# ZPP-Robotics/OSQP-Solver

Hardware: AMD Instinct MI355X
Metric: QPs/sec on a 1024-QP batch of box-QPs (n=512, m=1024), OSQP defaults; ADMM iters/sec alongside (higher is better)
Workload: dtype f64

## Files before the change

include/mi_osqp.h:

```cpp
#ifndef MI_OSQP_H
#define MI_OSQP_H

#include <stdint.h>

#ifdef __cplusplus
extern "C" {
#endif

typedef enum {
  MI_OSQP_OK = 0,
  MI_OSQP_ERR_INVALID_DATA = 1,
  MI_OSQP_ERR_INVALID_SETTINGS = 2,
  MI_OSQP_ERR_PATTERN_CHANGED = 3,
  MI_OSQP_ERR_NONCONVEX = 4,
  MI_OSQP_ERR_DEVICE = 5,
  MI_OSQP_ERR_NULL = 6,
  MI_OSQP_ERR_ALLOC = 7
} mi_osqp_error;

typedef enum {
  MI_OSQP_EXIT_OPTIMAL = 0,
  MI_OSQP_EXIT_PRIMAL_INFEASIBLE = 1,
  MI_OSQP_EXIT_DUAL_INFEASIBLE = 2,
  MI_OSQP_EXIT_OPTIMAL_INACCURATE = 3,
// ... 132 lines not shown
int mi_osqp_batch_update_A_bounds_some(mi_osqp_batch *h, int64_t n_ids, const int64_t *ids,
                                       const double *A_val, const double *l, const double *u);
int mi_osqp_batch_warm_start_x_some(mi_osqp_batch *h, int64_t n_ids, const int64_t *ids, const double *x );
int mi_osqp_batch_update_q_some(mi_osqp_batch *h, int64_t n_ids, const int64_t *ids, const double *q );
int mi_osqp_batch_warm_start_y_some(mi_osqp_batch *h, int64_t n_ids, const int64_t *ids, const double *y );
int mi_osqp_batch_solve_begin_some(mi_osqp_batch *h, int64_t n_ids, const int64_t *ids);
int mi_osqp_batch_advance(mi_osqp_batch *h, int64_t n_segments);
int mi_osqp_batch_poll(mi_osqp_batch *h, int64_t wait, int64_t *n_finished, int64_t *ids_out, int64_t capacity);
int mi_osqp_batch_get_primal_some(mi_osqp_batch *h, int64_t n_ids, const int64_t *ids, double *x_out );
int mi_osqp_batch_get_dual_some(mi_osqp_batch *h, int64_t n_ids, const int64_t *ids, double *y_out );
int mi_osqp_batch_get_info_some(mi_osqp_batch *h, int64_t n_ids, const int64_t *ids, mi_osqp_info *info );
int64_t mi_osqp_batch_running(mi_osqp_batch *h);

typedef enum {
  MI_GOMP_MODEL_UR5E_FLANGE = 1,
  MI_GOMP_MODEL_UR5E_WRIST3 = 2,
  MI_GOMP_MODEL_UR5E_ELBOW = 3,
  MI_GOMP_MODEL_YAW_2LINK = 4,
  MI_GOMP_MODEL_TABLE = 5
} mi_gomp_model;
typedef struct { int32_t model; int32_t is_gripper; double radius; double param[12]; } mi_gomp_ball;
typedef struct { double dir[2]; double point[3]; int32_t below; int32_t reserved; } mi_gomp_line;
typedef struct mi_gomp_scene mi_gomp_scene;
int mi_gomp_scene_create(mi_gomp_scene **out, mi_osqp_batch *h, int64_t dims, int64_t waypoints,
                         int64_t n_balls, const mi_gomp_ball *balls, int64_t n_lines, const mi_gomp_line *lines,
                         const double *con_lo, const double *con_hi);
void mi_gomp_scene_free(mi_gomp_scene *sc);
int mi_gomp_scene_set_rows(mi_gomp_scene *sc, int64_t n_ids, const int64_t *ids, const double *A_val, const double *l, const double *u);
int mi_gomp_scene_get_rows(mi_gomp_scene *sc, int64_t id, double *A_val, double *l, double *u);
int mi_gomp_assemble_some(mi_gomp_scene *sc, int64_t n_ids, const int64_t *ids, const double *x, int32_t *ok_out);
int mi_gomp_relinearise_some(mi_gomp_scene *sc, int64_t n_ids, const int64_t *ids, const double *x, int32_t *ok_out);

typedef struct mi_osqp_multi mi_osqp_multi;
int mi_osqp_multi_batch_setup(mi_osqp_multi **out, int64_t n_devices, const int64_t *devices,
                              int64_t B, int64_t n, int64_t m,
                              const int64_t *P_colptr, const int64_t *P_rowidx, const double *P_val,
                              const double *q,
                              const int64_t *A_colptr, const int64_t *A_rowidx, const double *A_val,
                              const double *l, const double *u, const mi_osqp_settings *settings);
int mi_osqp_multi_batch_update_A(mi_osqp_multi *h, const int64_t *A_colptr, const int64_t *A_rowidx, const double *A_val);
int mi_osqp_multi_batch_update_bounds(mi_osqp_multi *h, const double *l, const double *u);
int mi_osqp_multi_batch_update_A_bounds(mi_osqp_multi *h, const int64_t *A_colptr, const int64_t *A_rowidx, const double *A_val,
                                        const double *l, const double *u);
int mi_osqp_multi_batch_warm_start_x(mi_osqp_multi *h, const double *x);
int mi_osqp_multi_batch_update_q(mi_osqp_multi *h, const double *q);
int mi_osqp_multi_batch_update_P(mi_osqp_multi *h, const int64_t *P_colptr, const int64_t *P_rowidx, const double *P_val);
int mi_osqp_multi_batch_update_P_A(mi_osqp_multi *h, const int64_t *P_colptr, const int64_t *P_rowidx, const double *P_val,
                                   const int64_t *A_colptr, const int64_t *A_rowidx, const double *A_val);
int mi_osqp_multi_batch_warm_start_y(mi_osqp_multi *h, const double *y);
int mi_osqp_multi_batch_solve(mi_osqp_multi *h);
int mi_osqp_multi_batch_solve_async(mi_osqp_multi *h);
int mi_osqp_multi_batch_wait(mi_osqp_multi *h);
int mi_osqp_multi_batch_get_primal(mi_osqp_multi *h, double *x_out );
int mi_osqp_multi_batch_get_dual(mi_osqp_multi *h, double *y_out );
int mi_osqp_multi_batch_get_info(mi_osqp_multi *h, mi_osqp_info *info );
int64_t mi_osqp_multi_batch_shards(mi_osqp_multi *h);
int mi_osqp_multi_batch_shard(mi_osqp_multi *h, int64_t k, int64_t *device, int64_t *begin, int64_t *end, mi_osqp_batch **handle);
void mi_osqp_multi_batch_free(mi_osqp_multi *h);

int mi_osqp_batch_spmv(mi_osqp_batch *h, const double *d_x, const double *d_y,
                       double *d_Px, double *d_Aty, double *d_Ax, void *stream);
int mi_osqp_batch_kkt_solve(mi_osqp_batch *h, const double *d_rhs, double *d_sol, void *stream);
int mi_osqp_batch_refactor_device(mi_osqp_batch *h);
int mi_osqp_batch_kernel_time(mi_osqp_batch *h, double *avg_ms, int64_t *launches);
int mi_osqp_batch_refactor_time(mi_osqp_batch *h, double *factor_ms, double *tail_ms, int64_t *launches, int64_t *qps);
int mi_osqp_batch_refactor_peak(mi_osqp_batch *h, int64_t *qps, double *factor_ms, double *tail_ms);

int mi_osqp_batch_get_scaling(mi_osqp_batch *h, double *D , double *E , double *c );

int mi_osqp_debug_host_kkt_solve(int64_t n, int64_t m,
                                 const int64_t *P_colptr, const int64_t *P_rowidx, const double *P_val,
                                 const int64_t *A_colptr, const int64_t *A_rowidx, const double *A_val,
                                 const double *l, const double *u, const mi_osqp_settings *settings,
                                 int64_t tile, const double *rhs ,
                                 double *sol_schedule , double *sol_direct ,
                                 mi_osqp_stats *st);

int mi_osqp_debug_host_block_factor(int64_t n, int64_t m,
                                    const int64_t *P_colptr, const int64_t *P_rowidx, const double *P_val,
                                    const int64_t *A_colptr, const int64_t *A_rowidx, const double *A_val,
                                    const double *l, const double *u, const mi_osqp_settings *settings,
                                    double *max_rel_diff_L, double *max_rel_diff_Dinv, int64_t *counts);

int mi_osqp_debug_refactor_chunks(int64_t n_flagged, const int64_t *flagged, int64_t n_active, const int64_t *active, int64_t tile,
                                  int64_t chunk_qps, int64_t max_chunks, int64_t *n_chunks, int64_t *work_begin, int64_t *tiles,
                                  int64_t *tile_begin);

int mi_osqp_debug_trace_kkt_solve(mi_osqp_batch *h, int32_t which, const double *d_rhs, double *d_sol,
                                  uint32_t *out, int64_t out_capacity_words, int64_t *dims);

#ifdef __cplusplus
}
#endif
#endif
```

osqp-solver_amd/__init__.py:

```python
import ctypes as C
import os

import numpy as np

try:
    import torch
except ImportError:
    torch = None

from . import build as _build

_HERE = os.path.dirname(os.path.abspath(__file__))
_LIB = None

EXIT_NAMES = ["kOptimal", "kPrimalInfeasible", "kDualInfeasible", "kOptimalInaccurate",
              "kPrimalInfeasibleInaccurate", "kDualInfeasibleInaccurate", "kMaxIterations",
              "kInterrupted", "kTimeLimitReached", "kNonConvex", "kUnknown"]
K_OPTIMAL = 0


class Settings(C.Structure):
    _fields_ = [("rho", C.c_double), ("sigma", C.c_double), ("scaling", C.c_int64),
                ("adaptive_rho", C.c_int64), ("adaptive_rho_interval", C.c_int64),
                ("adaptive_rho_tolerance", C.c_double), ("max_iter", C.c_int64),
# ... 58 lines not shown
        L.mi_osqp_last_error.restype = C.c_char_p
        L.mi_osqp_batch_setup.argtypes = [C.POINTER(vp), C.c_int64, C.c_int64, C.c_int64, ip, ip, dp, dp, ip, ip, dp,
                                          dp, dp, C.POINTER(Settings), C.c_int64]
        L.mi_osqp_batch_update_A.argtypes = [vp, ip, ip, dp]
        L.mi_osqp_batch_update_A_bounds.argtypes = [vp, ip, ip, dp, dp, dp]
        L.mi_osqp_batch_update_bounds.argtypes = [vp, dp, dp]
        L.mi_osqp_batch_warm_start_x.argtypes = [vp, dp]
        L.mi_osqp_batch_update_q.argtypes = [vp, dp]
        L.mi_osqp_batch_update_q_device.argtypes = [vp, vp, vp]
        L.mi_osqp_batch_update_P.argtypes = [vp, ip, ip, dp]
        L.mi_osqp_batch_update_P_A.argtypes = [vp, ip, ip, dp, ip, ip, dp]
        L.mi_osqp_batch_warm_start_y.argtypes = [vp, dp]
        L.mi_osqp_batch_update_q_some.argtypes = [vp, C.c_int64, ip, dp]
        L.mi_osqp_batch_warm_start_y_some.argtypes = [vp, C.c_int64, ip, dp]
        L.mi_osqp_batch_solve.argtypes = [vp]
        L.mi_osqp_batch_get_primal.argtypes = [vp, dp]
        L.mi_osqp_batch_get_dual.argtypes = [vp, dp]
        L.mi_osqp_batch_get_info.argtypes = [vp, C.POINTER(Info)]
        L.mi_osqp_batch_get_stats.argtypes = [vp, C.POINTER(Stats)]
        L.mi_osqp_batch_get_ordering.argtypes = [vp, ip]
        L.mi_osqp_batch_free.argtypes = [vp]; L.mi_osqp_batch_free.restype = None
        L.mi_osqp_batch_update_bounds_device.argtypes = [vp, vp, vp, vp]
        L.mi_osqp_batch_update_A_bounds_device.argtypes = [vp, vp, vp, vp, vp]
        L.mi_osqp_batch_solve_device.argtypes = [vp, vp, vp, vp, vp]
        L.mi_osqp_batch_reset.argtypes = [vp]
        L.mi_osqp_batch_refactor_device.argtypes = [vp]
        L.mi_osqp_batch_last_solve_stats.argtypes = [vp, ip, ip, dp, dp, ip, dp]
        L.mi_osqp_batch_last_polish_stats.argtypes = [vp, ip, ip, dp]
        L.mi_osqp_batch_get_polish_active.argtypes = [vp, C.POINTER(C.c_int8)]
        L.mi_osqp_batch_get_scaling.argtypes = [vp, dp, dp, dp]
        L.mi_osqp_batch_spmv.argtypes = [vp, vp, vp, vp, vp, vp, vp]
        L.mi_osqp_batch_kkt_solve.argtypes = [vp, vp, vp, vp]
        L.mi_osqp_batch_kernel_time.argtypes = [vp, dp, ip]
        L.mi_osqp_batch_refactor_time.argtypes = [vp, dp, dp, ip, ip]
        L.mi_osqp_batch_refactor_peak.argtypes = [vp, ip, dp, dp]
        L.mi_osqp_batch_reinit_some.argtypes = [vp, C.c_int64, ip, dp, dp, dp]
        L.mi_osqp_batch_update_A_bounds_some.argtypes = [vp, C.c_int64, ip, dp, dp, dp]
        L.mi_osqp_batch_warm_start_x_some.argtypes = [vp, C.c_int64, ip, dp]
        L.mi_osqp_batch_solve_begin_some.argtypes = [vp, C.c_int64, ip]
        L.mi_osqp_batch_advance.argtypes = [vp, C.c_int64]
        L.mi_osqp_batch_poll.argtypes = [vp, C.c_int64, ip, ip, C.c_int64]
        L.mi_osqp_batch_get_primal_some.argtypes = [vp, C.c_int64, ip, dp]
        L.mi_osqp_batch_get_dual_some.argtypes = [vp, C.c_int64, ip, dp]
        L.mi_osqp_batch_get_info_some.argtypes = [vp, C.c_int64, ip, C.POINTER(Info)]
        L.mi_osqp_batch_running.argtypes = [vp]; L.mi_osqp_batch_running.restype = C.c_int64
        L.mi_osqp_setup.argtypes = [C.POINTER(vp), C.c_int64, C.c_int64, ip, ip, dp, dp, ip, ip, dp, dp, dp, C.POINTER(Settings)]
        L.mi_osqp_update_A.argtypes = [vp, ip, ip, dp]
        L.mi_osqp_update_bounds.argtypes = [vp, dp, dp]
        L.mi_osqp_warm_start_x.argtypes = [vp, dp]
        L.mi_osqp_update_q.argtypes = [vp, dp]
        L.mi_osqp_update_P.argtypes = [vp, ip, ip, dp]
        L.mi_osqp_update_P_A.argtypes = [vp, ip, ip, dp, ip, ip, dp]
        L.mi_osqp_warm_start_y.argtypes = [vp, dp]
        L.mi_osqp_solve.argtypes = [vp, C.POINTER(Info)]
        L.mi_osqp_get_primal.argtypes = [vp, dp]
        L.mi_osqp_get_dual.argtypes = [vp, dp]
        L.mi_osqp_get_stats.argtypes = [vp, C.POINTER(Stats)]
        L.mi_osqp_free.argtypes = [vp]; L.mi_osqp_free.restype = None
        L.mi_osqp_multi_batch_setup.argtypes = [C.POINTER(vp), C.c_int64, ip, C.c_int64, C.c_int64, C.c_int64, ip, ip, dp, dp,
                                                ip, ip, dp, dp, dp, C.POINTER(Settings)]
        L.mi_osqp_multi_batch_update_A.argtypes = [vp, ip, ip, dp]
        L.mi_osqp_multi_batch_update_bounds.argtypes = [vp, dp, dp]
        L.mi_osqp_multi_batch_update_A_bounds.argtypes = [vp, ip, ip, dp, dp, dp]
        L.mi_osqp_multi_batch_warm_start_x.argtypes = [vp, dp]
        L.mi_osqp_multi_batch_update_q.argtypes = [vp, dp]
        L.mi_osqp_multi_batch_update_P.argtypes = [vp, ip, ip, dp]
        L.mi_osqp_multi_batch_update_P_A.argtypes = [vp, ip, ip, dp, ip, ip, dp]
        L.mi_osqp_multi_batch_warm_start_y.argtypes = [vp, dp]
        L.mi_osqp_multi_batch_solve.argtypes = [vp]
        L.mi_osqp_multi_batch_solve_async.argtypes = [vp]
        L.mi_osqp_multi_batch_wait.argtypes = [vp]
        L.mi_osqp_multi_batch_get_primal.argtypes = [vp, dp]
        L.mi_osqp_multi_batch_get_dual.argtypes = [vp, dp]
        L.mi_osqp_multi_batch_get_info.argtypes = [vp, C.POINTER(Info)]
        L.mi_osqp_multi_batch_shards.argtypes = [vp]; L.mi_osqp_multi_batch_shards.restype = C.c_int64
        L.mi_osqp_multi_batch_shard.argtypes = [vp, C.c_int64, ip, ip, ip, C.POINTER(vp)]
        L.mi_osqp_multi_batch_free.argtypes = [vp]; L.mi_osqp_multi_batch_free.restype = None
        L.mi_osqp_debug_host_kkt_solve.argtypes = [C.c_int64, C.c_int64, ip, ip, dp, ip, ip, dp, dp, dp,
                                                   C.POINTER(Settings), C.c_int64, dp, dp, dp, C.POINTER(Stats)]
        L.mi_osqp_debug_refactor_chunks.argtypes = [C.c_int64, ip, C.c_int64, ip, C.c_int64, C.c_int64, C.c_int64, ip, ip, ip, ip]
        L.mi_osqp_prefetch_analysis.argtypes = [C.c_int64, C.c_int64, C.c_int64, ip, ip, ip, ip, C.c_int64]
        L.mi_osqp_debug_host_block_factor.argtypes = [C.c_int64, C.c_int64, ip, ip, dp, ip, ip, dp, dp, dp,
                                                      C.POINTER(Settings), dp, dp, ip]
        _LIB = L
    return _LIB


def host_cores():
    try:
        n = len(os.sched_getaffinity(0))
    except Exception:
        n = os.cpu_count() or 1
    for path in ("/sys/fs/cgroup/cpu.max",):
        try:
            quota, period = open(path).read().split()[:2]
            if quota != "max":
                n = min(n, max(1, int(round(int(quota) / int(period)))))
        except Exception:
            pass
    try:
        q = int(open("/sys/fs/cgroup/cpu/cpu.cfs_quota_us").read())
        p = int(open("/sys/fs/cgroup/cpu/cpu.cfs_period_us").read())
        if q > 0:
            n = min(n, max(1, int(round(q / p))))
    except Exception:
        pass
    return n


def default_settings(**kw):
    s = Settings()
    lib().mi_osqp_default_settings(C.byref(s))
    for k, v in kw.items():
        if not hasattr(s, k):
            raise KeyError(k)
        setattr(s, k, v)
    return s


def _i64(a):
    return np.ascontiguousarray(a, dtype=np.int64)


def _f64(a):
    return np.ascontiguousarray(a, dtype=np.float64)


def _ip(a):
    return a.ctypes.data_as(C.POINTER(C.c_int64))


def _dp(a):
    return None if a is None else a.ctypes.data_as(C.POINTER(C.c_double))


def _chk(rc, where):
    if rc != 0:
        raise MiOsqpError(rc, where)


def _csc(M):
    import scipy.sparse as sp
    M = sp.csc_matrix(M)
    M.sort_indices()
    return M


class BatchSolver:

    def __init__(self, P_pattern, Px, q, A_pattern, Ax, l, u, device=-1, **settings):
        L = lib()
        P, A = _csc(P_pattern), _csc(A_pattern)
        self.n, self.m = A.shape[1], A.shape[0]
        Px, Ax, l, u = _f64(Px), _f64(Ax), _f64(l), _f64(u)
        if Ax.ndim == 1:
            Px, Ax, l, u = Px[None], Ax[None], l[None], u[None]
            q = None if q is None else _f64(q)[None]
        self.B = Ax.shape[0]
        q = None if q is None else _f64(q)
        self._Pp, self._Pi = _i64(P.indptr), _i64(P.indices)
        self._Ap, self._Ai = _i64(A.indptr), _i64(A.indices)
        self.settings = default_settings(**settings)
        self._h = C.c_void_p()
        rc = L.mi_osqp_batch_setup(C.byref(self._h), self.B, self.n, self.m, _ip(self._Pp), _ip(self._Pi), _dp(Px),
                                   _dp(q), _ip(self._Ap), _ip(self._Ai), _dp(Ax), _dp(l), _dp(u),
                                   C.byref(self.settings), device)
# ... 330 lines not shown
    def __init__(self, constraints, P, q=None, **settings):
        l, A, u = constraints
        self._b = BatchSolver(P, _csc(P).data, q, A, _csc(A).data, l, u, **settings)

    def update(self, constraints):
        l, A, u = constraints
        A = _csc(A)
        try:
            self._b.update_A(A.data, A_pattern=A)
            self._b.update_bounds(l, u)
        except MiOsqpError as e:
            raise ValueError(str(e)) from e

    def setWarmStart(self, x):
        self._b.warm_start_x(x)

    def solve(self):
        info = self._b.solve()[0]
        return int(info.exit_code), self._b.primal()[0]

    def info(self):
        return self._b.info()[0]

    def dual(self):
        return self._b.dual()[0]

    def stats(self):
        return self._b.stats()


def debug_host_kkt_solve(P, A, l, u, rhs, tri_waves=0, **settings):
    L = lib()
    P, A = _csc(P), _csc(A)
    n, m = A.shape[1], A.shape[0]
    s = default_settings(**settings)
    rhs = _f64(rhs)
    sol_s, sol_d = np.empty(n + m), np.empty(n + m)
    st = Stats()
    Pp, Pi, Px = _i64(P.indptr), _i64(P.indices), _f64(P.data)
    Ap, Ai, Ax = _i64(A.indptr), _i64(A.indices), _f64(A.data)
    l, u = _f64(l), _f64(u)
    rc = L.mi_osqp_debug_host_kkt_solve(n, m, _ip(Pp), _ip(Pi), _dp(Px), _ip(Ap), _ip(Ai), _dp(Ax), _dp(l), _dp(u),
                                        C.byref(s), 1 + int(tri_waves), _dp(rhs), _dp(sol_s), _dp(sol_d), C.byref(st))
    _chk(rc, "debug_host_kkt_solve")
    return sol_s, sol_d, st.as_dict()


def prefetch_analysis(P, A, B=1, device=-1, check=True):
    L = lib()
    P, A = _csc(P), _csc(A)
    n, m = A.shape[1], A.shape[0]
    Pp, Pi, Ap, Ai = _i64(P.indptr), _i64(P.indices), _i64(A.indptr), _i64(A.indices)
    rc = L.mi_osqp_prefetch_analysis(B, n, m, _ip(Pp), _ip(Pi), _ip(Ap), _ip(Ai), device)
    if check:
        _chk(rc, "prefetch_analysis")
    return rc


def debug_refactor_chunks(flagged, active, tile, chunk_qps, max_chunks=8):
    f, a = _i64(flagged), _i64(active)
    nch = C.c_int64()
    wb = np.zeros(max_chunks + 2, dtype=np.int64); tb = np.zeros(max_chunks + 2, dtype=np.int64)
    tl = np.zeros(max(1, len(a)), dtype=np.int64)
    _chk(lib().mi_osqp_debug_refactor_chunks(len(f), _ip(f), len(a), _ip(a), tile, chunk_qps, max_chunks, C.byref(nch), _ip(wb), _ip(tl),
                                             _ip(tb)), "debug_refactor_chunks")
    k = int(nch.value)
    return ([f[wb[c]:wb[c + 1]].tolist() for c in range(k)], [tl[tb[c]:tb[c + 1]].tolist() for c in range(k)])


def debug_host_block_factor(P, A, l, u, **settings):
    L = lib()
    P, A = _csc(P), _csc(A)
    n, m = A.shape[1], A.shape[0]
    s = default_settings(**settings)
    Pp, Pi, Px = _i64(P.indptr), _i64(P.indices), _f64(P.data)
    Ap, Ai, Ax = _i64(A.indptr), _i64(A.indices), _f64(A.data)
    l, u = _f64(l), _f64(u)
    dL, dD = C.c_double(), C.c_double()
    cnt = (C.c_int64 * 4)()
    rc = L.mi_osqp_debug_host_block_factor(n, m, _ip(Pp), _ip(Pi), _dp(Px), _ip(Ap), _ip(Ai), _dp(Ax), _dp(l), _dp(u),
                                           C.byref(s), C.byref(dL), C.byref(dD), cnt)
    _chk(rc, "debug_host_block_factor")
    return dL.value, dD.value, dict(blocks=cnt[0], triples=cnt[1], storage=cnt[2], levels=cnt[3])
```

osqp-solver_amd/csrc/device_types.h:

```cpp
#pragma once
#include <hip/hip_runtime.h>
#include <stdint.h>

namespace miosqp {

#define MI_CHUNK 16

struct SchedDev {
  const uint32_t *step, *idxw;
  const uint64_t *idxw64;
  const uint32_t *lvl_pos, *tail_bar;
  int n_phases, nw, n_levels;
  uint32_t n_steps, n_slots;
};

struct DenseTailDev {
  int s, k, n_phases;
  uint32_t n_steps;
  const uint32_t *task;
  const uint32_t *wave_task, *wave_step, *tail_bar;
};

enum { DS_C = 0, DS_CINV, DS_RHO, DS_RHO_EST, DS_PRI_RES, DS_DUA_RES, DS_OBJ, DS_COUNT };
enum { IS_STATUS = 0, IS_ITER, IS_RHO_UPDATES, IS_DONE, IS_NEED_REFACTOR, IS_CUR, IS_PENDING, IS_EPOCH, IS_COUNT };

struct KernelArgs {
  int n, m, N, B;
  SchedDev fwd, bwd, chk;
  const uint32_t *pinv;
  const uint32_t *xloc;
  const double *fwd_val, *bwd_val, *chk_val, *dinv;
  DenseTailDev dt;
  const double *dt_val;
  const double *fwd_val0, *bwd_val0, *dt_val0;
  const int *use_work;
  double *x, *z, *y;
  const double *q, *l, *u, *rho_vec, *rho_inv, *Dsc, *Dsc_inv, *Esc, *Esc_inv;
  double *dx, *dy, *out1, *out2, *dscal;
  int *iscal;
  double *x_out, *y_out;
  double *xs_global;
  int xs_len;
  int rs_off;
  int rf_off;
  int wide;
  double sigma, alpha, eps_abs, eps_rel, eps_prim_inf, eps_dual_inf, rho_tolerance;
  int check_termination, rho_interval, max_iter, scaled_termination, scaling, adaptive_rho;
  int iter_begin, iter_end;
  int op_out_lds;
  int info_at_end;
  int mw_groups;
  unsigned *mw_bar;
  double *mw_scratch;
  int df;
  unsigned df_shadow;
  const unsigned char *rflag;
  const int *sel;
  const int *tiles;
};

struct FactorArgs {
  int n, m, N, B, nnzP, nnzK, pa_len, n_levels, force_all;
  int debug_skip;
  uint32_t storage;
  SchedDev fwd, bwd;
  const uint32_t *blk, *lvl, *utask, *tri4, *dtask, *ttask, *asm_dst, *asm_src;
  const uint32_t *ubig;
  int *use_work;
  const int32_t *fwd_srcblk, *bwd_srcblk;
  const double *pa_val, *l, *u, *dscal;
  double *rho_vec, *rho_inv, *Lblk, *Dl, *dinv_scratch, *fwd_val, *bwd_val, *dinv;
  int *iscal, *npos;
  int home_bt;
  const int *work;
  double sigma;
  int dt_k;
  int mw_groups;
  unsigned *mw_bar;
  const signed char *pmask;
  const int32_t *arow;
  int *pstat;
  double pdelta;
};

struct TailArgs {
  int n, N, s, k, kbt, home_bt;
  uint32_t storage, n_slots;
  int n_lt, n_ltcol;
  uint32_t n_quads;
  int nh;
  uint32_t cs_doubles;
  const int *work;
  const uint32_t *lt_pos, *ltcol_col, *tile_tab, *wave_tiles, *diag_tile;
  const uint64_t *asm_q64;
  const int32_t *src_tile;
  const uint32_t *dt_task, *dt_task_step;
  uint32_t n_tasks;
  const double *Lblk, *Dl;
  double *Sd, *dt_val, *dinv;
  int *npos, *iscal;
  unsigned long long *trace;
  int *pstat;
};
hipError_t launch_tail(const TailArgs &a, int nwork, size_t lds_asm, size_t lds, hipStream_t st);

struct PolishArgs {
  int *stat;
  signed char *act;
  double *sol;
  int refine_iter;
};
hipError_t launch_polish_active(const KernelArgs &a, const PolishArgs &p, int BT, hipStream_t st);
hipError_t launch_polish(const KernelArgs &a, const PolishArgs &p, int BT, int tiles, int threads, size_t lds, int n_cus, hipStream_t st);
hipError_t launch_factor(const FactorArgs &a, int BT, int tiles, int threads, hipStream_t st);
size_t factor_lds_bytes(int BT, int threads);
bool factor_fits_lds(const FactorArgs &a, int threads);

int max_coresident_groups(int threads, size_t lds, int n_cus);
int max_coresident_factor_groups(int threads, int n_cus);
hipError_t launch_iterate(const KernelArgs &a, int BT, int tiles, int threads, size_t lds, hipStream_t st);
int rf_head_steps();
int rf_lds_steps();
hipError_t launch_check(const KernelArgs &a, int BT, int tiles, int threads, size_t lds, hipStream_t st);
hipError_t launch_advance(const KernelArgs &a, int BT, int tiles, int threads, size_t lds, hipStream_t st, int max_segments, int seg_len,
                          int *host_is, double *host_ds, unsigned *stop, unsigned seq, unsigned *counter, unsigned *host_done);
hipError_t launch_spmv(const KernelArgs &a, int BT, int tiles, int threads, size_t lds, hipStream_t st,
                       const double *x, const double *y, double *Px, double *Aty, double *Ax);
struct SpmvFused {
  const uint32_t *ptr, *ent;
  const double *pa_val;
  int pa_len;
  const uint32_t *ell, *rowid;
  int n_pass;
  uint32_t ell_off[4], ell_k[4];
};
hipError_t launch_spmv_fused(const KernelArgs &a, const SpmvFused &t, int BT, int tiles, int n_cus, hipStream_t st,
                             const double *x, const double *y, double *Px, double *Aty, double *Ax);
size_t spmv_fused_lds_bytes(int n, int m, int pa_len, int BT);
hipError_t launch_kkt_solve(const KernelArgs &a, int BT, int tiles, int threads, size_t lds, hipStream_t st,
                            const double *rhs, double *sol);
hipError_t launch_kkt_trace(const KernelArgs &a, int BT, int tiles, int threads, size_t lds, hipStream_t st,
                            const double *rhs, double *sol, uint32_t *trace, uint32_t words);
hipError_t launch_warm_start(const KernelArgs &a, int BT, int tiles, int threads, size_t lds, hipStream_t st,
                             const double *x0);
hipError_t launch_interleave(const double *src, double *dst, const int *ids, int nq, int len, int BT, hipStream_t st);
hipError_t launch_scatter(const double *src, double *dst, const int *map, const int *ids, int nq, int srclen,
                          const SchedDev &sd, int BT, hipStream_t st);
hipError_t launch_deinterleave(const double *src, double *dst, int nq, int len, int BT, hipStream_t st);
struct RuizArgs {
  int n, m, nnzP, nnzA, B, BT, iters;
  const int *ids;
  int raw_by_qp;
  int fresh;
  const double *rawP, *rawq;
  const int32_t *Prow, *Pcol, *Arow, *Acol;
  const double *rawPnew;
  const double *rawA;
  const double *rawl, *rawu;
  double *pa_val, *q, *Dsc, *Dsc_inv, *Esc, *Esc_inv, *l, *u, *dscal;
  double *dn, *en;
  double *pa_out;
};
hipError_t launch_ruiz(const RuizArgs &a, hipStream_t st);
hipError_t launch_lin_cost(const double *gq, const int *ids, double *q, double *rawq, const double *Dsc, const double *dscal,
                           int nq, int n, int BT, int scaling, hipStream_t st);
hipError_t launch_warm_start_y(const KernelArgs &a, int nslots, int BT, hipStream_t st, const double *y0);
hipError_t launch_start_slots(const KernelArgs &a, const int *slots, const int *clear, int nslots, int BT, int cold, hipStream_t st);
hipError_t launch_fresh_slots(const KernelArgs &a, const int *slots, int nslots, int BT, double rho0, hipStream_t st);
hipError_t launch_worklist(const int *iscal, int *work, int nslots, int BT, hipStream_t st);
hipError_t launch_resume_flagged(const KernelArgs &a, int nslots, int BT, hipStream_t st);
hipError_t launch_copy_slot_streams(double *dst, const double *src, const int *slots, int nslots, size_t per, hipStream_t st);
hipError_t launch_keep_rows(double *dst, const double *src, const int *ids, int n_ids, int len, hipStream_t st);
hipError_t launch_copy_flagged_streams(double *dst, const double *src, const int *flags, int want, int nslots, size_t per, hipStream_t st);
hipError_t launch_copy_slot_rows(double *dst, const double *src, const int *slots, int nslots, int len, int BT, hipStream_t st);
enum { MI_GM_UR5E_FLANGE = 1, MI_GM_UR5E_WRIST3 = 2, MI_GM_UR5E_ELBOW = 3, MI_GM_YAW_2LINK = 4, MI_GM_TABLE = 5 };
struct GompBallDev { int model, is_gripper; double radius; double param[12]; };
struct GompLineDev { double D[3], A[3]; int below, pad; };
struct GompArgs {
  int dims, W, n_balls, n_lines, n, m, nnzA, n_ids, row0, write_rows;
  const int *ids;
  const GompBallDev *balls;
  const GompLineDev *lines;
  double con_lo[3], con_hi[3];
  const int *aidx;
  const double *traj;
// ... 12 lines not shown
```

osqp-solver_amd/csrc/host_core.cpp:

```cpp
#include "host_core.hpp"
#include "sched_format.h"

#include <algorithm>
#include <cmath>
#include <cstdio>
#include <cstdlib>
#include <cstring>
#include <numeric>
#include <set>
#include <chrono>
#include <thread>

#include "../../include/mi_osqp.h"

namespace miosqp {

int validate_settings(const Settings &s) {
  if (s.scaling < 0 || s.max_iter <= 0 || s.check_termination < 0) return 1;
  if (s.adaptive_rho != 0 && s.adaptive_rho != 1) return 1;
  if (s.adaptive_rho_interval < 0 || s.adaptive_rho_tolerance < 1.0) return 1;
  if (!(s.rho > 0.0) || !(s.sigma > 0.0)) return 1;
  if (s.eps_abs < 0.0 || s.eps_rel < 0.0 || (s.eps_abs == 0.0 && s.eps_rel == 0.0)) return 1;
  if (!(s.eps_prim_inf > 0.0) || !(s.eps_dual_inf > 0.0)) return 1;
  if (!(s.alpha > 0.0) || !(s.alpha < 2.0)) return 1;
// ... 726 lines not shown
          ut_of_level[lev1].push_back({id, tb, te, te});
        }
        if (n1 < tl.size()) {
          uint32_t tb = (uint32_t)(bf.tri.size() / 2);
          for (size_t q = n1; q < tl.size(); q++) bf.tri.insert(bf.tri.end(), {tl[q].first, tl[q].second});
          uint32_t te = (uint32_t)(bf.tri.size() / 2);
          ut_of_level[L].push_back({id, tb, tb, te});
        }
      }
    }
  for (int L = 0; L < nlev; L++) {
    uint32_t u0 = (uint32_t)(bf.utask.size() / 4), d0 = (uint32_t)bf.dtask.size(), t0 = (uint32_t)(bf.ttask.size() / 2);
    auto &uts = ut_of_level[L];
    std::stable_sort(uts.begin(), uts.end(), [](const UT &a, const UT &b) { return a.te - a.tb > b.te - b.tb; });
    {
      auto small = [&](const UT &u) { return u.te - u.tb <= 16u && (bf.blk[4 * u.id + 3] & 255u) <= 8u; };
      std::stable_partition(uts.begin(), uts.end(), [&](const UT &u) { return !small(u); });
      uint32_t nbig = 0;
      while (nbig < uts.size() && !small(uts[nbig])) nbig++;
      bf.ubig.push_back(u0 + nbig);
    }
    for (const UT &u : uts) bf.utask.insert(bf.utask.end(), {u.id, u.tb, u.tm, u.te});
    if (getenv("MI_OSQP_DEBUG_ORDER") && !uts.empty()) {
      std::vector<double> wv(16, 0.0);
      size_t r1 = 0, gen = 0;
      for (size_t k = 0; k < uts.size(); k++) { wv[k % 16] += (uts[k].tm - uts[k].tb + 7) / 8 * 1.0 + (uts[k].te - uts[k].tm) * 1.5; r1 += uts[k].tm - uts[k].tb; gen += uts[k].te - uts[k].tm; }
      fprintf(stderr, "[mi_osqp] factor level %d: %zu update tasks, rank-1 triples %zu, general %zu, biggest task %u, modelled path %.0f units (ideal %.0f)\n",
              L, uts.size(), r1, gen, uts[0].te - uts[0].tb, *std::max_element(wv.begin(), wv.end()), (r1 / 8.0 + gen * 1.5) / 16);
    }
    for (int pass = 0; pass < 2; pass++) {
      for (int J : cols_of_level[L]) {
        if (J >= ct0 || (cw(J) > 4) != (pass == 0)) continue;
        for (const auto &[I, id] : colblk[J]) {
          if (I == J) bf.dtask.push_back(id);
          else bf.ttask.insert(bf.ttask.end(), {id, colblk[J][0].second});
        }
      }
      if (pass == 0) { bf.ubig.push_back((uint32_t)bf.dtask.size()); bf.ubig.push_back((uint32_t)(bf.ttask.size() / 2)); }
    }
    bf.lvl.insert(bf.lvl.end(), {u0, (uint32_t)(bf.utask.size() / 4), d0, (uint32_t)bf.dtask.size(), t0, (uint32_t)(bf.ttask.size() / 2)});
  }
  if (getenv("MI_OSQP_DEBUG_ORDER")) {
    size_t cnt[5] = {0, 0, 0, 0, 0}, small = 0;
    for (size_t t = 0; t < bf.utask.size() / 4; t++) {
      const uint32_t w = bf.blk[4 * bf.utask[4 * t] + 3] & 255u, sz = bf.utask[4 * t + 3] - bf.utask[4 * t + 1];
      cnt[w <= 1 ? 0 : w <= 2 ? 1 : w <= 4 ? 2 : w <= 8 ? 3 : 4]++;
      small += sz <= 16;
    }
    fprintf(stderr, "[mi_osqp] update tasks by target width: 1: %zu, 2: %zu, 3-4: %zu, 5-8: %zu, 9-16: %zu; %zu of %zu with <= 16 triples\n", cnt[0], cnt[1], cnt[2], cnt[3], cnt[4], small, bf.utask.size() / 4);
  }
  bf.utask4.resize(bf.utask.size());
  for (size_t t = 0; t < bf.utask.size() / 4; t++) {
    const uint32_t id = bf.utask[4 * t], tb = bf.utask[4 * t + 1], tm = bf.utask[4 * t + 2], te = bf.utask[4 * t + 3];
    const uint32_t hw = bf.blk[4 * id + 3];
    if (tm - tb >= (1u << 22)) bf.overflow = true;
    bf.utask4[4 * t] = bf.blk[4 * id]; bf.utask4[4 * t + 1] = tb; bf.utask4[4 * t + 2] = ((hw >> 8) << 27) | ((hw & 255u) << 22) | ((tm - tb) & 0x3FFFFFu); bf.utask4[4 * t + 3] = te - tm;
  }
  bf.dtask4.resize(4 * bf.dtask.size());
  for (size_t t = 0; t < bf.dtask.size(); t++) for (int k = 0; k < 4; k++) bf.dtask4[4 * t + k] = bf.blk[4 * bf.dtask[t] + k];
  bf.ttask4.resize(2 * bf.ttask.size());
  for (size_t t = 0; t < bf.ttask.size() / 2; t++) {
    const uint32_t id = bf.ttask[2 * t], dg = bf.ttask[2 * t + 1];
    bf.ttask4[4 * t] = bf.blk[4 * id]; bf.ttask4[4 * t + 1] = bf.blk[4 * id + 2]; bf.ttask4[4 * t + 2] = bf.blk[4 * id + 3]; bf.ttask4[4 * t + 3] = bf.blk[4 * dg];
  }
  bf.tri4.resize(2 * bf.tri.size());
  for (size_t q = 0; q < bf.tri.size() / 2; q++) {
    const uint32_t ia = bf.tri[2 * q], ib = bf.tri[2 * q + 1];
    const uint32_t ahw = bf.blk[4 * ia + 3], bh = bf.blk[4 * ib + 3] >> 8;
    bf.tri4[4 * q] = bf.blk[4 * ia]; bf.tri4[4 * q + 1] = bf.blk[4 * ib]; bf.tri4[4 * q + 2] = bf.blk[4 * ia + 2];
    bf.tri4[4 * q + 3] = ((ahw >> 8) << 16) | ((ahw & 255u) << 8) | bh;
  }
  const int n = an.n, m = an.m, nnzK = an.nnzK();
  bf.asm_dst.assign(nnzK, 0); bf.asm_src.assign(nnzK, 0);
  std::vector<int> colOfK(nnzK);
  for (int j = 0; j < N; j++) for (int k = an.Kp[j]; k < an.Kp[j + 1]; k++) colOfK[k] = j;
  for (int e = 0; e < nnzK; e++) {
    int a = an.pinv[an.Ki[e]], b = an.pinv[colOfK[e]];
    bf.asm_dst[e] = pos_of(std::max(a, b), std::min(a, b));
  }
  for (int k = 0; k < an.Pp[n]; k++) bf.asm_src[an.PtoK[k]] = ((uint32_t)(an.PisDiag[k] ? ASM_P_SIGMA : ASM_P) << 29) | (uint32_t)k;
  for (int pos : an.sigmaOnlyK) bf.asm_src[pos] = (uint32_t)ASM_SIGMA << 29;
  for (int k = 0; k < an.Ap[n]; k++) bf.asm_src[an.AtoK[k]] = ((uint32_t)ASM_A << 29) | (uint32_t)k;
  for (int r = 0; r < m; r++) bf.asm_src[an.rhotoK[r]] = ((uint32_t)ASM_NEG_RHOINV << 29) | (uint32_t)r;
  bf.lpos.assign(an.nnzLx(), 0);
  for (int j = 0; j < N; j++) for (int p = an.Lp[j]; p < an.Lp[j + 1]; p++) bf.lpos[p] = (int32_t)pos_of(an.Li[p], j);
  for (int c = 0; c < nch; c++) {
    const int c0 = an.chunk_start[c], r = cw(c);
    if (an.inv_off[c] < 0) continue;
    const uint32_t id = find_blk(c, c), off = bf.blk[4 * id];
    for (int k = 0; k < r; k++) for (int i = k + 1; i < r; i++) bf.lpos[an.inv_index(c, i, k)] = (int32_t)(off + (uint32_t)i * r + (uint32_t)k);
    (void)c0;
  }
  auto compose = [&](const Schedule &s, std::vector<int32_t> &out) {
    out.resize(s.src.size());
    for (size_t k = 0; k < s.src.size(); k++) out[k] = s.src[k] >= 0 ? bf.lpos[s.src[k]] : s.src[k];
  };
  compose(an.fwd, an.fwd_srcblk);
  compose(an.bwd, an.bwd_srcblk);
  if (an.dt.k) {
    const int k = an.dt.k;
    an.dt.sblk.assign((size_t)k * k, 0u);
    for (int j = 0; j < k; j++) for (int i = j; i < k; i++) an.dt.sblk[(size_t)j * k + i] = pos_of(ts + i, ts + j);
    DenseTail &dt = an.dt;
    const int nt = k / 16;
    dt.lt_pos.clear(); dt.ltcol_col.clear();
    std::vector<std::vector<std::pair<int, std::vector<uint16_t>>>> frag(nt);
    for (int c = 0; c < ts; c++) {
      int ci = -1;
      for (int p = an.Lp[c]; p < an.Lp[c + 1]; p++) {
        const int i = an.Li[p];
        if (i < ts) continue;
        if (ci < 0) { ci = (int)dt.ltcol_col.size(); dt.ltcol_col.push_back((uint32_t)c); }
        const int I = (i - ts) / 16;
        if (frag[I].empty() || frag[I].back().first != ci) frag[I].push_back({ci, std::vector<uint16_t>(16, 0xFFFFu)});
        frag[I].back().second[(i - ts) % 16] = (uint16_t)dt.lt_pos.size();
        dt.lt_pos.push_back((uint32_t)bf.lpos[p]);
      }
    }
    dt.n_lt = (int)dt.lt_pos.size(); dt.n_ltcol = (int)dt.ltcol_col.size();
    const uint16_t zero_slot = (uint16_t)dt.n_lt;
    for (auto &fr : frag) for (auto &f : fr) for (uint16_t &v : f.second) if (v == 0xFFFFu) v = zero_slot;
    struct TileRec { int I, J; std::vector<std::pair<int, int>> src; };
    std::vector<TileRec> tiles;
    for (int I = 0; I < nt; I++)
      for (int J = 0; J <= I; J++) {
        TileRec t{I, J, {}};
        size_t a = 0, b = 0;
        while (a < frag[I].size() && b < frag[J].size()) {
          if (frag[I][a].first < frag[J][b].first) a++;
          else if (frag[I][a].first > frag[J][b].first) b++;
          else { t.src.push_back({(int)a, (int)b}); a++; b++; }
        }
        tiles.push_back(std::move(t));
      }
    const int nw = 16;
    std::vector<int> order(tiles.size());
    std::iota(order.begin(), order.end(), 0);
    std::stable_sort(order.begin(), order.end(), [&](int x, int y) { return tiles[x].src.size() > tiles[y].src.size(); });
    std::vector<std::vector<int>> mine(nw);
    for (size_t d = 0; d < order.size(); d++) { const size_t round = d / nw, pos = d % nw; mine[(round & 1) ? nw - 1 - pos : pos].push_back(order[d]); }
    dt.tile_tab.clear(); dt.wave_tiles.assign(nw + 1, 0u); dt.asm_q.clear(); dt.asm_qcol.clear();
    for (int w = 0; w < nw; w++) {
      dt.wave_tiles[w] = (uint32_t)(dt.tile_tab.size() / 4);
      for (int ti : mine[w]) {
        const TileRec &t = tiles[ti];
        const uint32_t q0 = (uint32_t)(dt.asm_q.size() / 64);
        const size_t padded = (t.src.size() + 31) / 32 * 32;
        for (size_t s0 = 0; s0 < padded; s0 += 4) {
          for (int g = 0; g < 4; g++) {
            const bool real = s0 + g < t.src.size();
            const auto *fa = real ? &frag[t.I][t.src[s0 + g].first] : nullptr;
            const auto *fb = real ? &frag[t.J][t.src[s0 + g].second] : nullptr;
            dt.asm_qcol.push_back(real ? (uint16_t)fa->first : (uint16_t)0);
            for (int e = 0; e < 16; e++) dt.asm_q.push_back(real ? ((uint32_t)fa->second[e] | ((uint32_t)fb->second[e] << 16)) : ((uint32_t)zero_slot | ((uint32_t)zero_slot << 16)));
          }
        }
        const uint32_t blk_id = find_blk(ct0 + t.I, ct0 + t.J);
        dt.tile_tab.insert(dt.tile_tab.end(), {((uint32_t)t.I << 16) | (uint32_t)t.J, bf.blk[4 * blk_id], q0, (uint32_t)(dt.asm_q.size() / 64)});
      }
    }
    dt.wave_tiles[nw] = (uint32_t)(dt.tile_tab.size() / 4);
    dt.asm_q64.resize(dt.asm_q.size());
    for (size_t e = 0; e < dt.asm_q.size(); e++) {
      const uint64_t w = dt.asm_q[e], ci = dt.asm_qcol[e / 16];
      dt.asm_q64[e] = ((w & 0xFFFFu) * 8u) | ((((w >> 16) * 8u) | ((ci * 8u) << 17)) << 32);
    }
    dt.src_tile.resize(dt.src.size());
    for (size_t e = 0; e < dt.src.size(); e++) {
      const int32_t sc = dt.src[e];
      dt.src_tile[e] = sc < 0 ? sc : (int32_t)dt_tile_offset(sc % k, sc / k);
    }
    dt.diag_tile.resize(k);
    for (int i = 0; i < k; i++) dt.diag_tile[i] = dt_tile_offset(i, i);
    dt.task_step.clear();
    { uint32_t pos = 0; for (size_t t = 0; t < dt.task.size() / 4; t++) { dt.task_step.push_back(pos); pos += dt.task[4 * t + 3]; } }
  }
}


Tuning tuning_from_env() {
  Tuning t;
  if (const char *e = getenv("MI_OSQP_TILE")) { const int v = atoi(e); if (v == 1 || v == 2 || v == 4) t.tile = v; }
  if (const char *e = getenv("MI_OSQP_THREADS")) t.threads = std::max(64, std::min(1024, atoi(e) / 64 * 64));
  t.global_xs = getenv("MI_OSQP_GLOBAL_XS") != nullptr;
  if (const char *e = getenv("MI_OSQP_GROUPS")) t.groups = std::max(0, std::min(256, atoi(e)));
  if (const char *e = getenv("MI_OSQP_GROUP_THREADS")) t.group_threads = std::max(64, std::min(512, atoi(e) / 64 * 64));
  if (const char *e = getenv("MI_OSQP_ASSUME_CUS")) t.assume_cus = std::max(0, atoi(e));
  if (const char *e = getenv("MI_OSQP_FACTOR_THREADS")) t.factor_threads = std::max(64, std::min(1024, atoi(e) / 64 * 64));
  if (const char *e = getenv("MI_OSQP_FACTOR_GROUPS")) t.factor_groups = std::max(1, std::min(256, atoi(e)));
  t.ruiz = getenv("MI_OSQP_HOST_RUIZ") ? 1 : getenv("MI_OSQP_DEVICE_RUIZ") ? -1 : 0;
  if (const char *e = getenv("MI_OSQP_CONT_RING_KB")) t.cont_ring_kb = std::max(0L, atol(e));
  if (const char *e = getenv("MI_OSQP_ANALYSIS_CACHE")) t.analysis_cache = atoi(e) != 0;
  t.stream_state = getenv("MI_OSQP_STREAM_STATE") != nullptr;
  t.stream_factor = getenv("MI_OSQP_STREAM_FACTOR") != nullptr;
  if (const char *e = getenv("MI_OSQP_REFACTOR_PIPELINE")) t.refactor_pipeline = atoi(e) != 0;
  if (const char *e = getenv("MI_OSQP_REFACTOR_PIPELINE_MIN")) t.pipeline_min = std::max(0, atoi(e));
  if (const char *e = getenv("MI_OSQP_REFACTOR_CHUNKS")) t.pipeline_chunks = std::max(0, std::min(8, atoi(e)));
  if (const char *e = getenv("MI_OSQP_REFACTOR_CHUNK_QPS")) t.pipeline_chunk_qps = std::max(0, atoi(e));
  AnalysisTuning &a = t.analysis;
  if (const char *e = getenv("MI_OSQP_DENSE_TAIL")) a.dense_tail = atoi(e);
  if (const char *e = getenv("MI_OSQP_ORDERING")) a.ordering = e[0];
  if (const char *e = getenv("MI_OSQP_ND_LEAF")) a.nd_leaf = atoi(e);
  if (const char *e = getenv("MI_OSQP_RELAX")) a.relax = atoi(e);
  a.serial = getenv("MI_OSQP_SERIAL_ANALYSIS") != nullptr;
  return t;
}

RefactorChunks refactor_chunks(const std::vector<int> &flagged, const std::vector<int> &active, int bt, int chunk_qps, int max_chunks) {
  RefactorChunks rc;
  const int nq = (int)flagged.size();
  max_chunks = std::max(1, max_chunks);
  chunk_qps = std::max(1, chunk_qps);
  if ((nq + chunk_qps - 1) / chunk_qps > max_chunks) chunk_qps = (nq + max_chunks - 1) / max_chunks;
  const int n_ref = (nq + chunk_qps - 1) / chunk_qps;
  rc.n_chunks = 1 + n_ref;
  rc.work_begin.assign(1, 0);
  for (int c = 0; c <= n_ref; c++) rc.work_begin.push_back(std::min(nq, c * chunk_qps));
  std::vector<std::pair<int, int>> tc;
  size_t f = 0;
  for (size_t i = 0; i < active.size(); i++) {
    const int tile = active[i] / bt;
    if (i && active[i - 1] / bt == tile) continue;
    int chunk = 0;
    while (f < flagged.size() && flagged[f] / bt < tile) f++;
    for (size_t g = f; g < flagged.size() && flagged[g] / bt == tile; g++) chunk = 1 + (int)g / chunk_qps;
    tc.emplace_back(chunk, tile);
  }
  std::stable_sort(tc.begin(), tc.end(), [](const std::pair<int, int> &x, const std::pair<int, int> &y) { return x.first < y.first; });
  rc.tile_begin.assign((size_t)rc.n_chunks + 1, 0);
  for (const auto &p : tc) { rc.tiles.push_back(p.second); rc.tile_begin[(size_t)p.first + 1]++; }
  for (int c = 0; c < rc.n_chunks; c++) rc.tile_begin[(size_t)c + 1] += rc.tile_begin[c];
  return rc;
}


int analyze(int64_t n64, int64_t m64, const int64_t *Pp, const int64_t *Pi, const int64_t *Ap,
            const int64_t *Ai, const AnalysisTuning &tune, Analysis &an, int nwaves, int bt, int max_extra_rows, int dense_tail_max, int tri_waves, int n_tiles) {
  if (nwaves < 1 || nwaves > 16 || (bt != 1 && bt != 2 && bt != 4) || tri_waves < 0 || tri_waves > 2048) return MI_OSQP_ERR_INVALID_SETTINGS;
  if (n64 <= 0 || m64 < 0 || !Pp || !Ap || n64 + m64 > (int64_t)1 << 30) return MI_OSQP_ERR_INVALID_DATA;
  int n = (int)n64, m = (int)m64, N = n + m;
  an = Analysis();
// ... 551 lines not shown
      const uint32_t st = pos[w], d = s.step[st];
      if (MI_D_NBAR(d)) return false;
      if (MI_D_TYPE(d) == MI_D_TYPE_ROW) {
        bool ready = true;
        for (uint32_t ln = 0; ln < 64 && ready; ln++) {
          const uint32_t slot = st * 64 + ln;
          if (s.src[slot] != MI_SRC_ZERO && wait[s.idx[slot]]) ready = false;
          if (s.src[slot] == MI_SRC_ZERO && s.idx[slot] != s.pad) ok = false;
        }
        if (!ready) continue;
        const uint32_t lt = MI_D_LT(d), T = 1u << lt;
        for (uint32_t ln = 0; ln < 64; ln++) {
          const uint32_t slot = st * 64 + ln;
          if (s.src[slot] != MI_SRC_ZERO) acc[w][ln] += (s.src[slot] == MI_SRC_ONE ? 1.0 : canon[s.src[slot]]) * xs[s.idx[slot]];
        }
        if (d & MI_D_FLUSH) {
          for (uint32_t g = 0; g < 64 / T; g++) {
            double sum = 0.0;
            for (uint32_t ln = g * T; ln < (g + 1) * T; ln++) sum += acc[w][ln];
            const uint32_t row = s.outA[s.step_ob[st] + g];
            if (row == kNoRow) continue;
            const bool sub = !(d & MI_D_STORE);
            const uint32_t dst = sub ? row + s.shadow : row;
            if (dst >= xs_len || written[dst] || !pending[dst] || (sub && (pending[row] || written[row]))) { ok = false; continue; }
            xs[dst] = sub ? xs[row] - sum : sum;
            written[dst] = 1; wait[dst] = 0;
          }
          std::fill(acc[w].begin(), acc[w].end(), 0.0);
        }
      }
      pos[w]++; progress = true;
    }
    if (done) break;
    if (!progress) return false;
  }
  for (size_t e = 0; e < xs_len; e++) if (pending[e] && !written[e]) ok = false;
  return ok;
}

static bool replay_kkt_solve_df(const Analysis &an, const QPNumeric &qp, const double *rhs, double *sol) {
  const int N = an.N, SH = an.Next;
  std::vector<double> xs(an.xs_total, 0.0);
  std::vector<char> pend(an.xs_total, 0);
  for (int k = 0; k < N; k++) {
    xs[k] = rhs[an.perm[k]];
    if (an.rflag[k] & 1) pend[k + SH] = 1;
    if (an.rflag[k] & 4) pend[an.xloc[k]] = 1;
  }
  bool ok = replay_dataflow(an.fwd, qp.Lx.data(), xs.data(), xs.size(), pend);
  std::fill(pend.begin(), pend.end(), 0);
  for (int k = 0; k < N; k++) {
    const double v = xs[an.df_floc(k)] * qp.Dlinv[k];
    xs[an.xloc[k]] = v;
    if (an.rflag[k] & 2) pend[an.xloc[k] + SH] = 1;
    if (an.rflag[k] & 4) pend[k] = 1;
  }
  ok = replay_dataflow(an.bwd, qp.Lx.data(), xs.data(), xs.size(), pend) && ok;
  for (int k = 0; k < N; k++) sol[an.perm[k]] = xs[an.df_bloc(k)];
  return ok;
}

bool replay_kkt_solve(const Analysis &an, const QPNumeric &qp, const double *rhs, double *sol) {
  if (an.df) return replay_kkt_solve_df(an, qp, rhs, sol);
  int N = an.N;
  std::vector<double> xs(an.Next, 0.0);
  for (int k = 0; k < N; k++) xs[k] = rhs[an.perm[k]];
  bool ok = replay(an.fwd, qp.Lx.data(), xs.data(), xs.size(), true, nullptr);
  const int ts = an.dt.k ? an.dt.s : N;
  for (int k = 0; k < ts; k++) xs[an.xloc[k]] *= qp.Dlinv[k];
  if (an.dt.k) {
    std::vector<double> md(an.dt.k);
    for (int i = 0; i < an.dt.k; i++) md[i] = qp.Minv[(size_t)i * an.dt.k + i];
    ok = replay_dense_tail(an.dt, qp.Minv.data(), md.data(), xs.data() + ts) && ok;
  }
  ok = replay(an.bwd, qp.Lx.data(), xs.data(), xs.size(), true, nullptr) && ok;
  for (int k = 0; k < N; k++) sol[an.perm[k]] = xs[k];
  return ok;
}

int replay_block_factor(const Analysis &an, const Settings &st, const QPNumeric &qp, QPNumeric &out) {
  const BlockFactor &bf = an.bf;
  const int n = an.n, N = an.N;
  std::vector<double> S(bf.storage, 0.0), D(N, 0.0);
  for (int e = 0; e < an.nnzK(); e++) {
    uint32_t kind = bf.asm_src[e] >> 29, idx = bf.asm_src[e] & 0x1FFFFFFFu;
    double v = 0.0;
    switch (kind) {
      case ASM_P: v = qp.Pv[idx]; break;
      case ASM_P_SIGMA: v = qp.Pv[idx] + st.sigma; break;
      case ASM_SIGMA: v = st.sigma; break;
      case ASM_A: v = qp.Av[idx]; break;
      default: v = -qp.rho_inv[idx]; break;
    }
    S[bf.asm_dst[e]] = v;
  }
  auto B = [&](uint32_t id, uint32_t &off, uint32_t &r0, uint32_t &c0, uint32_t &h, uint32_t &w) {
    off = bf.blk[4 * id]; r0 = bf.blk[4 * id + 1]; c0 = bf.blk[4 * id + 2]; h = bf.blk[4 * id + 3] >> 8; w = bf.blk[4 * id + 3] & 255u;
  };
  int positive = 0;
  for (int L = 0; L < bf.n_levels; L++) {
    const uint32_t *lv = &bf.lvl[6 * L];
    for (uint32_t t = lv[0]; t < lv[1]; t++) {
      uint32_t off, r0, c0, h, w; B(bf.utask[4 * t], off, r0, c0, h, w);
      for (uint32_t q = bf.utask[4 * t + 1]; q < bf.utask[4 * t + 3]; q++) {
        uint32_t ao, ar, ac, ah, aw, bo, br, bc, bh, bw;
        B(bf.tri[2 * q], ao, ar, ac, ah, aw); B(bf.tri[2 * q + 1], bo, br, bc, bh, bw);
        for (uint32_t j = 0; j < w; j++) for (uint32_t i = 0; i < h; i++) {
          double acc = 0.0;
          for (uint32_t k = 0; k < aw; k++) acc += S[ao + k * ah + i] * D[ac + k] * S[bo + k * bh + j];
          S[off + j * h + i] -= acc;
        }
      }
    }
    for (uint32_t t = lv[2]; t < lv[3]; t++) {
      uint32_t off, r0, c0, h, w; B(bf.dtask[t], off, r0, c0, h, w);
      for (uint32_t j = 0; j < w; j++) {
        double d = S[off + j * h + j];
        if (d == 0.0) return MI_OSQP_ERR_NONCONVEX;
        if (d > 0.0) positive++;
        D[c0 + j] = d;
        for (uint32_t i = j + 1; i < h; i++) S[off + j * h + i] /= d;
        for (uint32_t k = j + 1; k < w; k++) for (uint32_t i = k; i < h; i++) S[off + k * h + i] -= S[off + j * h + i] * d * S[off + j * h + k];
      }
    }
    for (uint32_t t = lv[4]; t < lv[5]; t++) {
      uint32_t off, r0, c0, h, w, doff, dr, dc, dh, dw;
      B(bf.ttask[2 * t], off, r0, c0, h, w); B(bf.ttask[2 * t + 1], doff, dr, dc, dh, dw);
      for (uint32_t i = 0; i < h; i++)
        for (uint32_t j = 0; j < w; j++) {
          double v = S[off + j * h + i];
          for (uint32_t k = 0; k < j; k++) v -= S[off + k * h + i] * D[c0 + k] * S[doff + k * dh + j];
          S[off + j * h + i] = v / D[c0 + j];
        }
    }
  }
  for (uint32_t t = 0; t < bf.dtask.size(); t++) {
    uint32_t off, r0, c0, h, w; B(bf.dtask[t], off, r0, c0, h, w);
    for (int j = (int)w - 2; j >= 0; j--)
      for (uint32_t i = (uint32_t)j + 1; i < w; i++) {
        double x = -S[off + (uint32_t)j * h + i];
        for (uint32_t p2 = (uint32_t)j + 1; p2 < i; p2++) x = std::fma(-S[off + i * h + p2], S[off + (uint32_t)j * h + p2], x);
        S[off + i * h + (uint32_t)j] = x;
      }
  }
  out.Lx.resize(an.nnzLx()); out.Dl = D; out.Dlinv.resize(N);
  for (int p = 0; p < an.nnzLx(); p++) out.Lx[p] = S[bf.lpos[p]];
  for (int j = 0; j < N; j++) out.Dlinv[j] = 1.0 / D[j];
  out.Minv.clear();
  if (an.dt.k) {
    const int k = an.dt.k;
    const DenseTail &dt = an.dt;
    std::vector<double> A((size_t)k * k);
    {
      std::vector<double> La((size_t)dt.n_lt + 1, 0.0), Dc(dt.n_ltcol);
      for (int e = 0; e < dt.n_lt; e++) La[e] = S[dt.lt_pos[e]];
      for (int ci = 0; ci < dt.n_ltcol; ci++) Dc[ci] = D[dt.ltcol_col[ci]];
      for (size_t t = 0; t < dt.tile_tab.size() / 4; t++) {
        const uint32_t I = dt.tile_tab[4 * t] >> 16, J = dt.tile_tab[4 * t] & 0xFFFFu, boff = dt.tile_tab[4 * t + 1];
        double tile[16][16];
        for (int r = 0; r < 16; r++) for (int c = 0; c < 16; c++) {
          const int rr = (I == J && r < c) ? c : r, cc = (I == J && r < c) ? r : c;
          tile[r][c] = S[boff + (uint32_t)cc * 16 + (uint32_t)rr];
        }
        for (uint32_t q = dt.tile_tab[4 * t + 2]; q < dt.tile_tab[4 * t + 3]; q++)
          for (int r = 0; r < 16; r++) for (int c = 0; c < 16; c++) {
            double acc = tile[r][c];
            for (int g = 0; g < 4; g++) {
              const double av = -La[dt.asm_q[(size_t)q * 64 + g * 16 + r] & 0xFFFFu];
              const double bv = La[dt.asm_q[(size_t)q * 64 + g * 16 + c] >> 16] * Dc[dt.asm_qcol[(size_t)q * 4 + g]];
              acc = std::fma(av, bv, acc);
            }
            tile[r][c] = acc;
          }
        for (int r = 0; r < 16; r++) for (int c = 0; c < 16; c++) {
          const size_t i = (size_t)I * 16 + r, j = (size_t)J * 16 + c;
          if (I != J || r >= c) A[j * k + i] = A[i * k + j] = tile[r][c];
        }
      }
    }
    std::vector<double> G((size_t)k * 16), C((size_t)k * 16);
    for (int p0 = 0; p0 < k; p0 += 16) {
      double T[16][16];
      for (int a = 0; a < 16; a++) for (int b = 0; b < 16; b++) T[a][b] = A[(size_t)(p0 + b) * k + p0 + a];
      for (int kk = 0; kk < 16; kk++) {
        const double d = T[kk][kk];
        if (d == 0.0) return MI_OSQP_ERR_NONCONVEX;
        if (d > 0.0) positive++;
        const double di = 1.0 / d;
        for (int a = 0; a < 16; a++) for (int b = 0; b < 16; b++) if (a != kk && b != kk) T[a][b] -= T[a][kk] * di * T[kk][b];
        for (int a = 0; a < 16; a++) if (a != kk) { T[a][kk] *= di; T[kk][a] = T[a][kk]; }
        T[kk][kk] = -di;
      }
      for (int r = 0; r < k; r++)
        for (int c = 0; c < 16; c++) {
          const bool piv = r >= p0 && r < p0 + 16;
          C[(size_t)c * k + r] = piv ? 0.0 : A[(size_t)(p0 + c) * k + r];
        }
      for (int r = 0; r < k; r++)
        for (int c = 0; c < 16; c++) {
          double g = 0.0;
          for (int q = 0; q < 16; q++) g = std::fma(C[(size_t)q * k + r], -T[q][c], g);
          G[(size_t)c * k + r] = g;
        }
      for (int j = 0; j < k; j++) for (int i = 0; i < k; i++) {
        double acc = A[(size_t)j * k + i];
        for (int q = 0; q < 16; q++) acc = std::fma(-G[(size_t)q * k + i], C[(size_t)q * k + j], acc);
        A[(size_t)j * k + i] = acc;
      }
      for (int r = 0; r < k; r++) {
        if (r >= p0 && r < p0 + 16) continue;
        for (int c = 0; c < 16; c++) A[(size_t)(p0 + c) * k + r] = A[(size_t)r * k + p0 + c] = G[(size_t)c * k + r];
      }
      for (int a = 0; a < 16; a++) for (int b = 0; b < 16; b++) A[(size_t)(p0 + b) * k + p0 + a] = T[a][b];
    }
    out.Minv.resize((size_t)k * k);
    for (size_t e = 0; e < A.size(); e++) out.Minv[e] = -A[e];
  }
  return positive == n ? MI_OSQP_OK : MI_OSQP_ERR_NONCONVEX;
}

void replay_spmv(const Analysis &an, const QPNumeric &qp, const double *x, const double *y,
                 double *Px, double *Aty, double *Ax) {
  int n = an.n, m = an.m;
  std::vector<double> xs(n + m), out(2 * n + m, 0.0), pa(qp.Pv.size() + qp.Av.size());
  std::copy(x, x + n, xs.begin()); std::copy(y, y + m, xs.begin() + n);
  std::copy(qp.Pv.begin(), qp.Pv.end(), pa.begin());
  std::copy(qp.Av.begin(), qp.Av.end(), pa.begin() + qp.Pv.size());
  replay(an.chk, pa.data(), xs.data(), xs.size(), false, out.data());
  std::copy(out.begin(), out.begin() + n, Px);
  std::copy(out.begin() + n, out.begin() + 2 * n, Aty);
  std::copy(out.begin() + 2 * n, out.end(), Ax);
}

}
```

osqp-solver_amd/csrc/host_core.hpp:

```cpp
#pragma once

#include <cstdint>
#include <string>
#include <vector>

namespace miosqp {

constexpr double kInfty = 1e30;
constexpr double kRhoMin = 1e-6, kRhoMax = 1e6, kRhoEqOverIneq = 1e3, kRhoTol = 1e-4;
constexpr double kMinScaling = 1e-4, kMaxScaling = 1e4;
constexpr double kDivisionTol = 1.0 / kInfty;
constexpr int kChunk = 16;
constexpr uint32_t kNoRow = 0xFFFFFFFFu;

struct Settings {
  double rho = 0.1, sigma = 1e-6;
  int64_t scaling = 10, adaptive_rho = 1, adaptive_rho_interval = 0;
  double adaptive_rho_tolerance = 5.0;
  int64_t max_iter = 4000;
  double eps_abs = 1e-3, eps_rel = 1e-3, eps_prim_inf = 1e-4, eps_dual_inf = 1e-4, alpha = 1.6;
  int64_t scaled_termination = 0, check_termination = 25, warm_start = 1, verbose = 0;
  int64_t polish = 0, polish_refine_iter = 3;
  double delta = 1e-6;
};
int validate_settings(const Settings &s);

struct AnalysisTuning {
  int dense_tail = -1;
  char ordering = 0;
  int nd_leaf = 0;
  int relax = -1;
  bool serial = false;
  bool operator==(const AnalysisTuning &o) const {
    return dense_tail == o.dense_tail && ordering == o.ordering && nd_leaf == o.nd_leaf && relax == o.relax && serial == o.serial;
  }
};
struct Tuning {
  int tile = 0;
  int threads = 0;
  bool global_xs = false;
  int groups = -1;
  int group_threads = 0;
  int assume_cus = 0;
  int factor_threads = 1024;
  int factor_groups = 0;
  int ruiz = 0;
  long cont_ring_kb = -1;
  bool analysis_cache = true;
  bool stream_state = false;
  bool stream_factor = false;
  bool refactor_pipeline = true;
  int pipeline_min = 0;
  int pipeline_chunks = 0;
  int pipeline_chunk_qps = 0;
  AnalysisTuning analysis;
};
Tuning tuning_from_env();

struct RefactorChunks {
  int n_chunks = 1;
  std::vector<int> work_begin;
  std::vector<int> tiles;
  std::vector<int> tile_begin;
};
RefactorChunks refactor_chunks(const std::vector<int> &flagged, const std::vector<int> &active, int bt, int chunk_qps, int max_chunks);

struct Schedule {
  int n_phases = 0, nw = 0, bt = 1;
  bool barriers = true;
  std::vector<uint32_t> phase;
  std::vector<int> level_first_phase;
  std::vector<uint32_t> step;
  std::vector<uint32_t> step_ob;
  std::vector<uint32_t> outA;
  std::vector<uint32_t> idx;
  std::vector<uint32_t> idxw;
  std::vector<uint64_t> idxw64;
  std::vector<int32_t> src;
  uint32_t n_slots = 0;
  uint32_t n_steps = 0;
  std::vector<uint32_t> wave_range;
  std::vector<uint32_t> lvl_pos;
  std::vector<uint32_t> tail_bar;
  bool dataflow = false;
  uint32_t shadow = 0, pad = 0;
  uint32_t phys_steps() const { return n_steps; }
  size_t phase_stride() const { return 4 * (size_t)nw + 1; }
  int n_levels = 0;
};

struct BlockFactor {
  uint32_t storage = 0;
  std::vector<uint32_t> blk;
  std::vector<uint32_t> lvl;
  std::vector<uint32_t> utask;
  std::vector<uint32_t> tri;
  std::vector<uint32_t> tri4;
  std::vector<uint32_t> utask4;
  bool overflow = false;
  std::vector<uint32_t> ubig;
  std::vector<uint32_t> dtask4;
  std::vector<uint32_t> ttask4;
  std::vector<uint32_t> dtask;
  std::vector<uint32_t> ttask;
  std::vector<uint32_t> asm_dst;
  std::vector<uint32_t> asm_src;
  std::vector<int32_t> lpos;
  int n_levels = 0;
  size_t n_blocks() const { return blk.size() / 4; }
};
enum { ASM_P = 0, ASM_P_SIGMA = 1, ASM_SIGMA = 2, ASM_A = 3, ASM_NEG_RHOINV = 4 };

struct DenseTail {
  int s = 0, k = 0, nb = 0;
  int nw = 0, n_phases = 0;
  uint32_t n_steps = 0;
  std::vector<uint32_t> task;
  std::vector<uint32_t> wave_task;
  std::vector<uint32_t> wave_step;
  std::vector<uint32_t> tail_bar;
  std::vector<int32_t> src;
  std::vector<uint32_t> sblk;
  int n_lt = 0, n_ltcol = 0;
  std::vector<uint32_t> lt_pos;
  std::vector<uint32_t> ltcol_col;
  std::vector<uint32_t> tile_tab;
  std::vector<uint32_t> wave_tiles;
  std::vector<uint32_t> asm_q;
  std::vector<uint16_t> asm_qcol;
  std::vector<uint64_t> asm_q64;
  std::vector<int32_t> src_tile;
  std::vector<uint32_t> diag_tile;
  std::vector<uint32_t> task_step;
  size_t asm_lds_bytes() const { return ((size_t)n_lt + 1 + (size_t)n_ltcol) * sizeof(double); }
};
inline uint32_t dt_tile_offset(int i, int j) {
  const int I = i / 16, J = j / 16, r = i % 16, c = j % 16;
  return (uint32_t)((I * (I + 1) / 2 + J) * 256 + ((r % 4) * 16 + c) * 4 + r / 4);
}
enum { DT_DIAG = 1, DT_SWAP = 2 };

struct Analysis {
  int n = 0, m = 0, N = 0;
  bool wide = false;
  std::vector<int> Pp, Pi, Psrc;
  std::vector<int> Ap, Ai;
  std::vector<int> Kp, Ki, PtoK, AtoK, rhotoK, sigmaOnlyK;
  std::vector<char> PisDiag;
  std::vector<int> perm, pinv;
  int ordering = 0;
  int relaxed_zeros = 0;
  std::vector<int> Klp, Kli, KtoKl;
  std::vector<int> Lp, Li, Rp, Rj, Rpos, etree;
  std::vector<int> sn_start;
  std::vector<int> chunk_start;
  std::vector<int> chunk_lev;
  std::vector<int> inv_off;
  int n_inv = 0;
  std::vector<int> xloc;
  int Next = 0;
  bool df = false;
  int tri_waves = 0;
  int xs_total = 0;
  std::vector<uint8_t> rflag;
  int df_floc(int e) const { return (rflag[e] & 4) ? xloc[e] : ((rflag[e] & 1) ? e + Next : e); }
  int df_bloc(int e) const { return (rflag[e] & 4) ? e : ((rflag[e] & 2) ? e + Next : e); }
  Schedule fwd, bwd, chk;
  BlockFactor bf;
  DenseTail dt;
  std::vector<int32_t> fwd_srcblk, bwd_srcblk;
  int nnzL() const { return Lp.empty() ? 0 : Lp.back(); }
  int nnzLx() const { return nnzL() + n_inv; }
  int inv_index(int c, int i, int k) const {
    const int r = chunk_start[c + 1] - chunk_start[c];
    return nnzL() + inv_off[c] + k * (2 * r - k - 1) / 2 + (i - k - 1);
  }
  int nnzK() const { return Kp.empty() ? 0 : Kp.back(); }
};

int analyze(int64_t n, int64_t m, const int64_t *Pp, const int64_t *Pi, const int64_t *Ap,
            const int64_t *Ai, const AnalysisTuning &tune, Analysis &an, int nwaves = 8, int bt = 1, int max_extra_rows = -1,
            int dense_tail_max = 512, int tri_waves = 0, int n_tiles = 1);
size_t phys_index(const Schedule &s, uint32_t slot, int b);

struct QPNumeric {
  std::vector<double> Pv, Av, q, l, u;
  std::vector<double> D, Dinv, E, Einv;
  double c = 1.0, cinv = 1.0;
  double rho = 0.1;
  std::vector<double> rho_vec, rho_inv;
  std::vector<int8_t> ctype;
  std::vector<double> Lx, Dl, Dlinv;
  std::vector<double> Minv;
};

void load_qp(const Analysis &an, const Settings &st, const double *Pval, const double *q,
             const double *Aval, const double *l, const double *u, QPNumeric &qp);
void scale_qp(const Analysis &an, const Settings &st, QPNumeric &qp);
void scale_like(const Analysis &an, const QPNumeric &rep, QPNumeric &qp);
void unscale_qp(const Analysis &an, QPNumeric &qp);
void set_rho_vec(const Analysis &an, const Settings &st, QPNumeric &qp);
int refresh_rho_types(const Analysis &an, QPNumeric &qp);
void apply_rho(const Analysis &an, QPNumeric &qp, double rho_new);
int factor_qp(const Analysis &an, const Settings &st, QPNumeric &qp, std::vector<double> &work);
void direct_kkt_solve(const Analysis &an, const QPNumeric &qp, const double *rhs, double *sol);
bool replay_dense_tail(const DenseTail &dt, const double *M, const double *mdiag, double *xt);
bool replay_kkt_solve(const Analysis &an, const QPNumeric &qp, const double *rhs, double *sol);
int replay_block_factor(const Analysis &an, const Settings &st, const QPNumeric &qp, QPNumeric &out);
void replay_spmv(const Analysis &an, const QPNumeric &qp, const double *x, const double *y,
// ... 4 lines not shown
```

osqp-solver_amd/csrc/kernels.hip:

```cpp
#include <hip/hip_runtime.h>
#include <stdint.h>
#include <stdlib.h>
#include <string.h>

#include <algorithm>
#include <map>
#include <mutex>

#include "device_types.h"
#include "sched_format.h"

namespace miosqp {

static hipError_t ensure_dynamic_lds(const void *kern, size_t lds);

#define MI_INFTY 1e30
#define MI_MIN_SCALING 1e-4
#define MI_DIV_TOL 1e-30
#define MI_RHO_MIN 1e-6
#define MI_RHO_MAX 1e6
#define MI_NOROW 0xFFFFFFFFu
#ifdef MI_OSQP_DEBUG_BUILD
#define MI_DBG_SKIP(a) ((a).debug_skip)
static bool debug_drop_group(const char *which) {
// ... 1882 lines not shown
    wave_sync();
    if (on && i > j) {
      const double ld = lij * d;
      for (int k = j + 1; k <= i; k++) MI_QS(k, i) -= ld * MI_QS(j, k);
    }
    wave_sync();
  }
  if (ok) { for (int k = 0; k < i; k++) Lb[((size_t)off + k * w + i) * BT + b] = MI_QS(k, i); }
#pragma unroll
  for (int j = 2; j >= 0; j--) {
    const bool on = ok && (uint32_t)(j + 2) <= w && i > j;
    double x = 0.0;
    if (on) {
      x = -MI_QS(j, i);
      for (int p2 = j + 1; p2 < i; p2++) x = fma(-MI_QS(p2, i), MI_QS(j, p2), x);
    }
    wave_sync();
    if (on) MI_QS(j, i) = x;
    wave_sync();
  }
  if (ok && w >= 2) { for (int k = 0; k < i; k++) Lb[((size_t)off + (size_t)i * w + k) * BT + b] = MI_QS(k, i); }
}
template <int BT>
__device__ __forceinline__ void fct_trsm_quad(double *Lb, const double *dinv, double *Ss, const uint4 td, const bool valid, int lane) {
  const int g = lane / (MI_CHUNK * BT), i = (lane / BT) % MI_CHUNK, b = lane % BT;
  const uint32_t off = td.x, h = td.z >> 8, w = td.z & 255u, c0 = td.y, db_off = td.w;
#pragma unroll
  for (int k = 0; k < 4; k++) MI_QS(k, i) = (valid && (uint32_t)k < w && (uint32_t)i < w && i > k) ? Lb[((size_t)db_off + k * w + i) * BT + b] : 0.0;
  wave_sync();
  if (valid && (uint32_t)i < h) {
    double ld[4];
#pragma unroll
    for (int j = 0; j < 4; j++) {
      if ((uint32_t)j < w) {
        double v = Lb[((size_t)off + j * h + i) * BT + b];
#pragma unroll
        for (int k = 0; k < j; k++) v = fma(-ld[k], MI_QS(k, j), v);
        ld[j] = v;
        Lb[((size_t)off + j * h + i) * BT + b] = v * dinv[((size_t)c0 + j) * BT + b];
      }
    }
  }
  wave_sync();
#undef MI_QS
}

template <int BT, bool LBL = false>
__global__ __launch_bounds__(1024) void factor_kernel(FactorArgs a) {
  extern __shared__ double smem[];
  bool multi = false;
  if constexpr (BT == 1) multi = a.mw_groups > 1;
  const unsigned G = multi ? (unsigned)a.mw_groups : 1u;
  const int tile = (int)(blockIdx.x / G), gidx = (int)(blockIdx.x % G);
  const Mw mw{a.mw_bar + 4 * (size_t)tile, G};
  const int tid = gidx * (int)blockDim.x + (int)threadIdx.x, nthr = (int)(blockDim.x * G);
  const int lane = tid & 63, wave = __builtin_amdgcn_readfirstlane(tid >> 6), nw = nthr >> 6, b = tid % BT;
  auto sync = [&]() { if constexpr (BT == 1) wg_or_grid_barrier(mw); else __syncthreads(); };
  const int m = a.m, N = a.N;
  const int slot = a.work ? a.work[tile * BT + b] : tile * BT + b;
  const size_t hbt = (size_t)a.home_bt;
  const size_t home = slot >= 0 ? (size_t)slot / hbt : 0, hb = slot >= 0 ? (size_t)slot % hbt : 0;
  auto H = [&](size_t len, size_t i) { return (home * len + i) * hbt + hb; };
  int flag = 0;
  if (slot >= 0) flag = a.work ? 1 : (a.force_all ? (slot < a.B) : a.iscal[H(IS_COUNT, IS_NEED_REFACTOR)]);
  if (!__syncthreads_or(flag)) return;
  double *Ss = smem + (size_t)(threadIdx.x >> 6) * MI_CHUNK * MI_CHUNK * BT;
  double *lds_rest = smem + (size_t)(blockDim.x >> 6) * MI_CHUNK * MI_CHUNK * BT;
  double *Lb, *Dl;
  if constexpr (LBL) { Lb = lds_rest; Dl = lds_rest + (size_t)a.storage * BT; }
  else { Lb = a.Lblk + (size_t)tile * a.storage * BT; Dl = a.Dl + (size_t)tile * N * BT; }
  const double rho = a.dscal[H(DS_COUNT, DS_RHO)];
  if (flag && !a.force_all && !a.pmask) {
    for (int e = tid; e < m * BT; e += nthr) {
      const size_t k = H(m, e / BT);
      const double l = a.l[k], u = a.u[k];
      double rv;
      if (l < -MI_INFTY * MI_MIN_SCALING && u > MI_INFTY * MI_MIN_SCALING) rv = MI_RHO_MIN;
      else if (u - l < 1e-4) rv = 1e3 * rho;
      else rv = rho;
      a.rho_vec[k] = rv; a.rho_inv[k] = 1.0 / rv;
    }
  }
  {
    const size_t tot = (size_t)a.storage * BT, pairs = tot / 2;
    double2 *L2p = reinterpret_cast<double2 *>(Lb);
    for (size_t e = tid; e < pairs; e += nthr) L2p[e] = make_double2(0.0, 0.0);
    if (tid == 0 && (tot & 1)) Lb[tot - 1] = 0.0;
    if (multi && tid == 0 && slot >= 0) a.npos[slot] = 0;
  }
  sync();
  {
    constexpr int UA = 2;
    const int tot = a.nnzK * BT;
    for (int e0 = tid; e0 < tot; e0 += nthr * UA) {
      uint32_t src[UA], dst[UA];
      double v[UA];
#pragma unroll
      for (int u = 0; u < UA; u++) {
        const int e = e0 + u * nthr;
        const int k = e < tot ? e / BT : 0;
        src[u] = a.asm_src[k]; dst[u] = a.asm_dst[k];
      }
#pragma unroll
      for (int u = 0; u < UA; u++) {
        const uint32_t kind = src[u] >> 29, idx = src[u] & 0x1FFFFFFFu;
        if (kind == 0) v[u] = a.pa_val[H(a.pa_len, idx)];
        else if (kind == 1) v[u] = a.pa_val[H(a.pa_len, idx)] + a.sigma;
        else if (kind == 2) v[u] = a.sigma;
        else if (kind == 3) {
          const bool off = a.pmask && (slot < 0 || a.pmask[(size_t)slot * m + a.arow[idx]] == 0);
          v[u] = off ? 0.0 : a.pa_val[H(a.pa_len, (size_t)a.nnzP + idx)];
        }
        else v[u] = a.pmask ? -a.pdelta : -a.rho_inv[H(m, idx)];
      }
#pragma unroll
      for (int u = 0; u < UA; u++) if (e0 + u * nthr < tot) Lb[(size_t)dst[u] * BT + b] = v[u];
    }
  }
  sync();
  int npos = 0, bad_inertia = 0;
  double *dnew;
  if constexpr (LBL) dnew = lds_rest + ((size_t)a.storage + (size_t)N) * BT;
  else dnew = a.dinv_scratch + (size_t)tile * N * BT;
  for (int L = 0; L < a.n_levels; L++) {
    const uint32_t *lv = a.lvl + 6 * L;
    const uint4 *ut4 = reinterpret_cast<const uint4 *>(a.utask), *dt4 = reinterpret_cast<const uint4 *>(a.dtask), *tt4 = reinterpret_cast<const uint4 *>(a.ttask);
    if (lv[1] > lv[0]) {
      uint32_t ub = lv[1];
      if constexpr (BT <= 2) { if (!(MI_DBG_SKIP(a) & 32)) ub = a.ubig[3 * L]; }
      uint32_t t = lv[0] + wave;
      uint4 nxt = t < ub ? ut4[t] : make_uint4(0, 0, 0, 0);
      for (; t < ub; t += nw) {
        const uint4 cur = nxt;
        if (t + nw < ub) nxt = ut4[t + nw];
        fct_update<BT>(a, Lb, Dl, Ss, cur, lane);
      }
      if constexpr (BT <= 2) {
        constexpr uint32_t NG = 64 / (MI_CHUNK * BT);
        const uint32_t g = (uint32_t)lane / (MI_CHUNK * BT);
        uint32_t tq = ub + NG * (uint32_t)wave;
        uint4 nq = tq + g < lv[1] ? ut4[tq + g] : make_uint4(0, 0, 0, 0);
        for (; tq < lv[1]; tq += NG * (uint32_t)nw) {
          const uint4 cur = nq;
          const bool valid = tq + g < lv[1];
          const uint32_t tn = tq + NG * (uint32_t)nw + g;
          if (tn < lv[1]) nq = ut4[tn];
          fct_update_quad<BT>(a, Lb, Dl, Ss, cur, valid, lane);
        }
      }
      sync();
    }
    if (!(MI_DBG_SKIP(a) & 4)) {
      uint32_t db = lv[3];
      if constexpr (BT <= 2) { if (!(MI_DBG_SKIP(a) & 32)) db = a.ubig[3 * L + 1]; }
      uint32_t t = lv[2] + wave;
      uint4 nxt = t < db ? dt4[t] : make_uint4(0, 0, 0, 0);
      for (; t < db; t += nw) {
        const uint4 cur = nxt;
        if (t + nw < db) nxt = dt4[t + nw];
        fct_diag<BT>(a, Lb, Dl, dnew, Ss, cur, lane, npos);
      }
      if constexpr (BT <= 2) {
        constexpr uint32_t NG = 64 / (MI_CHUNK * BT);
        const uint32_t g = (uint32_t)lane / (MI_CHUNK * BT);
        uint32_t tq = db + NG * (uint32_t)wave;
        uint4 nq = tq + g < lv[3] ? dt4[tq + g] : make_uint4(0, 0, 0, 0);
        for (; tq < lv[3]; tq += NG * (uint32_t)nw) {
// ... 46 lines not shown
    } else if (tid < BT && slot >= 0) a.npos[slot] = s_npos[b];
    if (tid < BT && flag && s_npos[b] != a.n && !MI_DBG_SKIP(a) && !a.dt_k) bad_inertia = 1;
  }
  if (flag && !(MI_DBG_SKIP(a) & 16)) {
    double *fv = a.fwd_val + (size_t)slot * a.fwd.n_steps * 64, *bv = a.bwd_val + (size_t)slot * a.bwd.n_steps * 64;
    auto scatter = [&](double *dst, const int32_t *map, uint32_t n_slots) {
      constexpr int US = 4;
      const uint32_t tot = n_slots * (uint32_t)BT;
      for (uint32_t e0 = tid; e0 < tot; e0 += (uint32_t)nthr * US) {
        int32_t mp[US];
        double v[US];
#pragma unroll
        for (int u = 0; u < US; u++) { const uint32_t e = e0 + (uint32_t)(u * nthr); mp[u] = e < tot ? map[e / BT] : MI_SRC_ZERO; }
#pragma unroll
        for (int u = 0; u < US; u++) v[u] = slot_value(mp[u], Lb, BT, b);
#pragma unroll
        for (int u = 0; u < US; u++) { const uint32_t e = e0 + (uint32_t)(u * nthr); if (e < tot) dst[e / BT] = v[u]; }
      }
    };
    scatter(fv, a.fwd_srcblk, a.fwd.n_slots);
    scatter(bv, a.bwd_srcblk, a.bwd.n_slots);
    for (int e = tid; e < N * BT; e += nthr) a.dinv[H(N, e / BT)] = dnew[e];
  }
  if (tid < BT && slot >= 0 && flag && a.use_work) a.use_work[slot] = 1;
  sync();
  __threadfence();
  if (a.pmask) { if (tid < BT && slot >= 0 && bad_inertia) a.pstat[slot] = -1; }
  else if (tid < BT && slot >= 0) a.iscal[H(IS_COUNT, IS_NEED_REFACTOR)] = bad_inertia ? -1 : 0;
}

template <int BT, bool LBL = false>
static hipError_t launch_factor_t(const FactorArgs &a, int tiles, int threads, hipStream_t st) {
  size_t lds = factor_lds_bytes(BT, threads);
  if (LBL) lds += ((size_t)a.storage + 2 * (size_t)a.N) * BT * sizeof(double);
  if (a.mw_groups > 1) { if (BT != 1 || !a.mw_bar || LBL) return hipErrorInvalidValue; tiles *= a.mw_groups; }
#ifdef MI_OSQP_DEBUG_BUILD
  if (a.mw_groups > 1 && debug_drop_group("factor")) tiles--;
#endif
  hipError_t e = ensure_dynamic_lds(reinterpret_cast<const void *>(&factor_kernel<BT, LBL>), lds);
  if (e != hipSuccess) return e;
  hipLaunchKernelGGL((factor_kernel<BT, LBL>), dim3(tiles), dim3(threads), lds, st, a);
  return hipGetLastError();
}
size_t factor_lds_bytes(int BT, int threads) { return (size_t)(threads / 64) * MI_CHUNK * MI_CHUNK * BT * sizeof(double); }
bool factor_fits_lds(const FactorArgs &a, int threads) {
  return !a.dt_k && factor_lds_bytes(1, threads) + ((size_t)a.storage + 2 * (size_t)a.N) * sizeof(double) <= 160 * 1024 - 1024;
}
hipError_t launch_factor(const FactorArgs &a, int BT, int tiles, int threads, hipStream_t st) {
  if (BT == 1 && a.mw_groups <= 1 && factor_fits_lds(a, threads)) return launch_factor_t<1, true>(a, tiles, threads, st);
  switch (BT) {
    case 1: return launch_factor_t<1>(a, tiles, threads, st);
    case 2: return launch_factor_t<2>(a, tiles, threads, st);
    default: return launch_factor_t<4>(a, tiles, threads, st);
  }
}


typedef double mi_v4d __attribute__((ext_vector_type(4)));
__device__ __forceinline__ mi_v4d mfma_f64(double a, double b, mi_v4d c) { return __builtin_amdgcn_mfma_f64_16x16x4f64(a, b, c, 0, 0, 0); }
__device__ __forceinline__ mi_v4d ld_tile(const double *A, uint32_t tix, int lane) {
  const double2 *p = reinterpret_cast<const double2 *>(A + (size_t)tix * 256 + (size_t)lane * 4);
  const double2 v0 = p[0], v1 = p[1];
  return mi_v4d{v0.x, v0.y, v1.x, v1.y};
}
__device__ __forceinline__ void st_tile(double *A, uint32_t tix, int lane, mi_v4d v) {
  double2 *p = reinterpret_cast<double2 *>(A + (size_t)tix * 256 + (size_t)lane * 4);
  p[0] = make_double2(v[0], v[1]); p[1] = make_double2(v[2], v[3]);
}
__device__ __forceinline__ uint32_t tile_ix(int I, int J) { return (uint32_t)(I * (I + 1) / 2 + J); }

#define MI_TAIL_NW 8
#define MI_TAIL_TS 65

__global__ __launch_bounds__(1024) void tail_assemble_kernel(TailArgs a) {
  extern __shared__ double smem[];
  const int g = blockIdx.x, tid = threadIdx.x, nthr = blockDim.x;
  const int lane = tid & 63, wave = __builtin_amdgcn_readfirstlane(tid >> 6);
  const int slot = a.work[g];
  if (slot < 0) return;
  const int k = a.k, kbt = a.kbt, wt = g / kbt, wb = g % kbt;
  double *A = a.Sd + (size_t)g * k * k;
  const double *Lb = a.Lblk + (size_t)wt * a.storage * kbt + wb;
  const double *Dl = a.Dl + (size_t)wt * a.N * kbt + wb;
  const int l15 = lane & 15, l4 = lane >> 4;
  {
    double *La = smem, *Dc = smem + a.n_lt + 1;
    for (int e = tid; e < a.n_lt; e += nthr) La[e] = Lb[(size_t)a.lt_pos[e] * kbt];
    if (tid == 0) La[a.n_lt] = 0.0;
    for (int c = tid; c < a.n_ltcol; c += nthr) Dc[c] = -Dl[(size_t)a.ltcol_col[c] * kbt];
    __syncthreads();
    constexpr int QB = 8;
    const uint32_t t_begin = a.wave_tiles[wave], t_end = a.wave_tiles[wave + 1];
    if (t_begin < t_end) {
      const uint4 *ttab = reinterpret_cast<const uint4 *>(a.tile_tab);
      auto load_init = [&](const uint4 &tt) {
        const int I = (int)(tt.x >> 16), J = (int)(tt.x & 0xFFFFu);
        mi_v4d v;
#pragma unroll
        for (int r = 0; r < 4; r++) {
          int row = l4 + 4 * r, col = l15;
          if (I == J && row < col) { const int t = row; row = col; col = t; }
          v[r] = Lb[((size_t)tt.y + (size_t)col * 16 + row) * kbt];
        }
        return v;
      };
      const mi_rsrc tab = make_rsrc(a.asm_q64, a.n_quads * 512u);
      const uint32_t q_last = a.n_quads ? a.n_quads - 1 : 0u;
      mi_u32x2 nxt[QB];
      auto fetch = [&](uint32_t qb) {
#pragma unroll
        for (int u = 0; u < QB; u++) {
          const uint32_t q = qb + u < q_last ? qb + u : q_last;
          nxt[u] = __builtin_amdgcn_raw_buffer_load_b64(tab, (uint32_t)lane * 8u, q * 512u, 0);
        }
      };
#pragma unroll
      for (int u = 0; u < QB; u++) nxt[u] = mi_u32x2{0u, 0u};
      uint32_t qnext = ttab[t_begin].z;
      if (a.n_quads) { fetch(qnext); qnext += QB; }
      const char *lds = reinterpret_cast<const char *>(smem);
      const uint32_t dc_off = (uint32_t)(a.n_lt + 1) * 8u;
      mi_v4d acc_next = load_init(ttab[t_begin]);
      for (uint32_t ti = t_begin; ti < t_end; ti++) {
        const uint4 tt = ttab[ti];
        mi_v4d acc = acc_next;
        acc_next = load_init(ttab[ti + 1 < t_end ? ti + 1 : ti]);
        for (uint32_t q = tt.z; q < tt.w; q += QB) {
          mi_u32x2 cur[QB];
#pragma unroll
          for (int u = 0; u < QB; u++) cur[u] = nxt[u];
          fetch(qnext); qnext += QB;
          double av[QB], bv[QB];
#pragma unroll
          for (int u = 0; u < QB; u++) {
            av[u] = *reinterpret_cast<const double *>(lds + cur[u].x);
            bv[u] = *reinterpret_cast<const double *>(lds + (cur[u].y & 0x1FFFFu)) * *reinterpret_cast<const double *>(lds + dc_off + (cur[u].y >> 17));
          }
#pragma unroll
          for (int u = 0; u < QB; u++) acc = mfma_f64(av[u], bv[u], acc);
        }
        st_tile(A, tile_ix((int)(tt.x >> 16), (int)(tt.x & 0xFFFFu)), lane, acc);
      }
    }
  }
}

template <int MI_TAIL_MAXSLOT, int PFT>
__global__ __launch_bounds__(512) void tail_kernel(TailArgs a) {
  extern __shared__ double smem[];
  const int g = blockIdx.x, tid = threadIdx.x, nthr = blockDim.x;
  const int lane = tid & 63, wave = __builtin_amdgcn_readfirstlane(tid >> 6);
  const int slot = a.work[g];
  if (slot < 0) return;
  const int k = a.k, kbt = a.kbt, wt = g / kbt, wb = g % kbt, nt = k / 16;
  const size_t hbt = (size_t)a.home_bt, home = (size_t)slot / hbt, hb = (size_t)slot % hbt;
  auto H = [&](size_t len, size_t i) { return (home * len + i) * hbt + hb; };
  double *A = a.Sd + (size_t)g * k * k;
  (void)wt; (void)wb;
  const int l15 = lane & 15, l4 = lane >> 4;
  unsigned long long tr_t = a.trace ? __builtin_amdgcn_s_memtime() : 0ull, tr_acc[8] = {0ull, 0ull, 0ull, 0ull, 0ull, 0ull, 0ull, 0ull};
  auto stamp = [&](int which) {
    if (a.trace && wave == 0) { const unsigned long long t = __builtin_amdgcn_s_memtime(); tr_acc[which] += t - tr_t; tr_t = t; }
  };
  stamp(0);
  const int nrt = nt - 4;
  const int nh = a.nh;
  double *Cs = smem;
  double *Ps = smem + (size_t)a.cs_doubles;
  double *Ts = Cs;
  int npos = 0;
  for (int p = 0; p < k / 64; p++) {
    const int P0 = 4 * p;
    auto nonp = [&](int x) { return x < P0 ? x : x + 4; };
    for (int t = wave; t < 10; t += MI_TAIL_NW) {
      int ta = 0, tb = t;
      while (tb > ta) { tb -= ta + 1; ta++; }
      const mi_v4d v = ld_tile(A, tile_ix(P0 + ta, P0 + tb), lane);
#pragma unroll
      for (int r = 0; r < 4; r++) {
        const int row = 16 * ta + l4 + 4 * r, col = 16 * tb + l15;
        if (ta != tb || row >= col) {
          Ts[row * MI_TAIL_TS + col] = v[r];
          Ts[col * MI_TAIL_TS + row] = v[r];
        }
      }
    }
    __syncthreads();
    for (int q = 0; q < 4; q++) {
      if (wave == 0) {
        double *U = Ts + (16 * q) * MI_TAIL_TS + 16 * q;
        double *rowbuf = Ps;
        const int r = l15, c0 = l4 * 4;
        double u[4];
#pragma unroll
        for (int cc = 0; cc < 4; cc++) u[cc] = U[r * MI_TAIL_TS + c0 + cc];
        for (int kk = 0; kk < 16; kk++) {
          if (r == kk) {
#pragma unroll
            for (int cc = 0; cc < 4; cc++) rowbuf[c0 + cc] = u[cc];
          }
          wave_sync();
          const double d = rowbuf[kk], ta = rowbuf[r];
          double tb[4];
#pragma unroll
          for (int cc = 0; cc < 4; cc++) tb[cc] = rowbuf[c0 + cc];
          wave_sync();
          if (lane == 0 && d > 0.0) npos++;
          double di = __builtin_amdgcn_rcp(d);
          di = fma(fma(-d, di, 1.0), di, di);
// ... 1081 lines not shown
```

osqp-solver_amd/csrc/solver.hip:

```cpp
#include <hip/hip_runtime.h>
#include <time.h>

#include <algorithm>
#include <atomic>
#include <chrono>
#include <cmath>
#include <condition_variable>
#include <functional>
#include <cstdio>
#include <cstdlib>
#include <cstring>
#include <string>
#include <thread>
#include <map>
#include <memory>
#include <mutex>
#include <vector>

#include "../../include/mi_osqp.h"
#include "device_types.h"
#include "host_core.hpp"

using namespace miosqp;

// ... 170 lines not shown
}
}

template <class T>
struct DevBuf {
  T *p = nullptr; size_t n = 0;
  size_t cap = 0;
  int dev = 0;
  int alloc(size_t count) {
    free();
    n = count;
    if (!count) return 0;
    const size_t bytes = (count * sizeof(T) + 255) & ~(size_t)255;
    if (hipGetDevice(&dev) != hipSuccess) dev = 0;
    if (void *q = devpool::take(dev, bytes, cap)) { p = (T *)q; return 0; }
    hipError_t e = hipMalloc((void **)&p, bytes);
    if (e != hipSuccess) {
      devpool::release_all();
      e = hipMalloc((void **)&p, bytes);
    }
    if (e != hipSuccess) { p = nullptr; g_last_error = std::string("hipMalloc: ") + hipGetErrorString(e); return MI_OSQP_ERR_ALLOC; }
    cap = bytes;
    return 0;
  }
  int zero(hipStream_t s) { if (n && hipMemsetAsync(p, 0, n * sizeof(T), s) != hipSuccess) return MI_OSQP_ERR_DEVICE; return 0; }
  int upload(const std::vector<T> &v) {
    int rc = alloc(v.size());
    if (rc) return rc;
    if (v.size() && hipMemcpy(p, v.data(), v.size() * sizeof(T), hipMemcpyHostToDevice) != hipSuccess) return MI_OSQP_ERR_DEVICE;
    return 0;
  }
  void free() { if (p && !devpool::give(dev, p, cap)) (void)hipFree(p); p = nullptr; n = 0; cap = 0; }
  ~DevBuf() { free(); }
};

struct SchedBufs {
  DevBuf<uint32_t> step, idxw, lvl_pos, tail_bar;
  DevBuf<uint64_t> idxw64;
  DevBuf<int32_t> src;
  int upload(const Schedule &s) {
    int rc;
    if ((rc = step.upload(s.step)) || (rc = idxw.upload(s.idxw)) || (rc = idxw64.upload(s.idxw64)) || (rc = src.upload(s.src)) ||
        (rc = lvl_pos.upload(s.lvl_pos)) || (rc = tail_bar.upload(s.tail_bar))) return rc;
    return 0;
  }
  SchedDev view(const Schedule &s) const {
    SchedDev d; d.step = step.p; d.idxw = idxw.p; d.idxw64 = idxw64.p; d.lvl_pos = lvl_pos.p; d.tail_bar = tail_bar.p;
    d.n_phases = s.n_phases; d.nw = s.nw; d.n_levels = s.n_levels;
    d.n_steps = s.n_steps; d.n_slots = s.n_slots;
    return d;
  }
};

struct mi_osqp_batch {
  Settings st;
  Tuning tune;
  std::shared_ptr<const Analysis> anp;
  int B = 0, BT = 1, ntiles = 0, threads = 512, device = 0, n_cus = 256;
  size_t lds = 0;
  size_t lds_iter = 0;
  int rs_off = 0;
  size_t lds_factor = 0;
  int rf_off = 0, rf_steps = 0;
  std::vector<QPNumeric> qp;
  bool host_bounds_stale = false;
  hipStream_t stream = nullptr;
  SchedBufs fwd, bwd, chk;
  DevBuf<uint32_t> pinv, xloc;
  DevBuf<double> fwd_val, bwd_val, chk_val, dinv, x, z, y, q, l, u, rho_vec, rho_inv, Dsc, Dsc_inv, Esc, Esc_inv;
  DevBuf<double> dx, dy, out1, out2, dscal, x_out, y_out, xs_global;
  bool global_xs = false;
  int mw_groups = 0, mw_threads = 0;
  DevBuf<uint32_t> mw_bar;
  DevBuf<unsigned char> rflag;
  DevBuf<double> mw_scratch;
  DevBuf<double> fwd_val0, bwd_val0, dinv0, rho_vec0, rho_inv0, dscal0;
  DevBuf<int> use_work;
  DevBuf<int> iscal, flag, npos;
  DevBuf<uint32_t> bf_blk, bf_lvl, bf_utask, bf_tri, bf_dtask, bf_ttask, bf_asm_dst, bf_asm_src, bf_ubig;
  DevBuf<int32_t> fwd_srcblk, bwd_srcblk;
  DevBuf<double> pa_val, Lblk, Dl, dinv_scratch;
  DevBuf<uint32_t> dt_task, dt_wave_task, dt_wave_step, dt_tail_bar;
  DevBuf<uint32_t> dt_lt_pos, dt_ltcol_col, dt_tile_tab, dt_wave_tiles, dt_diag_tile, dt_task_step;
  DevBuf<uint64_t> dt_asm_q64;
  DevBuf<int32_t> dt_src_tile;
  int dt_nh = 0; uint32_t dt_cs_doubles = 0; size_t dt_lds = 0, dt_lds_asm = 0;
  DevBuf<int32_t> dt_src;
  DevBuf<double> dt_val, dt_val0, dt_Sd;
  DevBuf<uint32_t> sp_ptr, sp_ent;
  DevBuf<uint32_t> sp_ell, sp_rowid;
  int sp_npass = 0;
  uint32_t sp_ell_off[4] = {0, 0, 0, 0}, sp_ell_k[4] = {0, 0, 0, 0};
  bool host_rho_stale = false;
  bool host_scaling_stale = false;
  DevBuf<int32_t> rz_prow, rz_pcol, rz_arow, rz_acol;
  bool clear_rho_updates = true;
  int *h_npos = nullptr;
  DevBuf<double> stage; DevBuf<int> ids, work;
  int *h_iscal = nullptr;
  double *h_dscal = nullptr;
  size_t h_iscal_cap = 0, h_dscal_cap = 0, h_npos_cap = 0, pin_cap = 0;
  double *pin = nullptr;
  size_t pin_n = 0;
  hipEvent_t ev0 = nullptr, ev1 = nullptr, evf0 = nullptr, evf1 = nullptr, evf2 = nullptr;
  hipStream_t pipe_r = nullptr, pipe_i = nullptr;
  hipEvent_t pipe_ev[streampool::kPipeEvents] = {};
  DevBuf<int> tile_list;
  int64_t pipelined_refactors = 0;
  double factor_ms_sum = 0.0, dense_ms_sum = 0.0;
  int64_t refactor_launches = 0, refactor_qps = 0, peak_qps = 0;
  double peak_factor_ms = 0.0, peak_tail_ms = 0.0;
  mi_osqp_stats stats{};
  int64_t last_total_iters = 0, last_launches = 0, last_refactors = 0;
  double last_device_s = 0.0, last_refactor_s = 0.0, kernel_ms_sum = 0.0;
  int64_t kernel_launches = 0, kernel_qp_iters = 0;
  bool solved_once = false;
  std::vector<char> failed;
  DevBuf<int> fail_list;
  DevBuf<double> rawP, rawq;
  DevBuf<double> pol_fwd, pol_bwd, pol_dinv, pol_dt, pol_sol;
  DevBuf<signed char> pol_act;
  DevBuf<int> pol_stat;
  std::vector<int> pol_status;
  int64_t pol_count = 0, pol_accepted = 0;
  double pol_seconds = 0.0;
  hipEvent_t evp0 = nullptr, evp1 = nullptr;
  struct Cont {
    bool on = false;
    int L = 25;
    unsigned launch_seq = 0;
    DevBuf<unsigned> stop;
    int64_t adv_seq = 0, polled_seq = 0;
    std::vector<char> running, clear_rho;
    std::vector<mi_osqp_info> info;
    int n_running = 0;
    int *h_is[2] = {nullptr, nullptr}; double *h_ds[2] = {nullptr, nullptr}; size_t h_is_cap[2] = {0, 0}, h_ds_cap[2] = {0, 0};
    hipEvent_t ev[2] = {nullptr, nullptr}; int64_t seq_of[2] = {0, 0};
    double *xh = nullptr, *yh = nullptr; size_t xh_cap = 0, yh_cap = 0;
    char *ring_h = nullptr; size_t ring_cap = 0, ring_h_cap = 0, ring_head = 0;
    DevBuf<char> ring_d;
    DevBuf<int> work;
    hipEvent_t ev_adv = nullptr;
    std::vector<int> epoch;
    DevBuf<double> rz_scratch;
    double *keepA = nullptr, *keepl = nullptr, *keepu = nullptr;
    DevBuf<unsigned> counter;
    unsigned *h_done = nullptr; size_t h_done_cap = 0;
  } cont;
  ~mi_osqp_batch() {
    DevGuard guard(device);
    if (stream) (void)hipStreamSynchronize(stream);
    for (int k = 0; k < 2; k++) { hostpool::give(cont.h_is[k], cont.h_is_cap[k]); hostpool::give(cont.h_ds[k], cont.h_ds_cap[k]); if (cont.ev[k]) (void)hipEventDestroy(cont.ev[k]); }
    hostpool::give(cont.xh, cont.xh_cap); hostpool::give(cont.yh, cont.yh_cap); hostpool::give(cont.ring_h, cont.ring_h_cap);
    if (cont.ev_adv) (void)hipEventDestroy(cont.ev_adv);
    if (evp0) (void)hipEventDestroy(evp0);
    if (evp1) (void)hipEventDestroy(evp1);
    hostpool::give(cont.h_done, cont.h_done_cap);
    hostpool::give(h_iscal, h_iscal_cap); hostpool::give(h_dscal, h_dscal_cap); hostpool::give(pin, pin_cap); hostpool::give(h_npos, h_npos_cap);
    if (pipe_r) (void)hipStreamSynchronize(pipe_r);
    if (pipe_i) (void)hipStreamSynchronize(pipe_i);
    streampool::Bundle sb{device, stream, {ev0, ev1, evf0, evf1, evf2}, pipe_r, pipe_i, {}};
    for (int k = 0; k < streampool::kPipeEvents; k++) sb.pipe_ev[k] = pipe_ev[k];
    if (stream && ev0 && ev1 && evf0 && evf1 && evf2) streampool::give(sb);
    else streampool::destroy(sb);
  }
};

struct mi_osqp_solver { mi_osqp_batch *b = nullptr; };


static Settings to_settings(const mi_osqp_settings *s) {
  Settings t;
  if (!s) return t;
  t.rho = s->rho; t.sigma = s->sigma; t.scaling = s->scaling; t.adaptive_rho = s->adaptive_rho;
  t.adaptive_rho_interval = s->adaptive_rho_interval; t.adaptive_rho_tolerance = s->adaptive_rho_tolerance;
  t.max_iter = s->max_iter; t.eps_abs = s->eps_abs; t.eps_rel = s->eps_rel; t.eps_prim_inf = s->eps_prim_inf;
  t.eps_dual_inf = s->eps_dual_inf; t.alpha = s->alpha; t.scaled_termination = s->scaled_termination;
  t.check_termination = s->check_termination; t.warm_start = s->warm_start; t.verbose = s->verbose;
  t.polish = s->polish; t.polish_refine_iter = s->polish_refine_iter; t.delta = s->delta;
  return t;
}

static void dense_tail_deal_stats(const DenseTail &dt, mi_osqp_stats &s) {
  s.dense_tail_tasks = s.dense_tail_waves_used = s.dense_tail_wave_tasks_max = 0;
  if (!dt.k) return;
  s.dense_tail_tasks = (int64_t)dt.task.size() / 4;
  for (int w = 0; w < dt.nw; w++) {
    const int64_t c = (int64_t)dt.wave_task[w + 1] - (int64_t)dt.wave_task[w];
    s.dense_tail_waves_used += c > 0; s.dense_tail_wave_tasks_max = std::max(s.dense_tail_wave_tasks_max, c);
  }
}

static size_t lds_bytes(int N, int BT, int threads) {
  int nw = threads / 64;
  return ((size_t)N * BT + (size_t)nw * 14 * BT + 14 * BT) * sizeof(double);
}

static KernelArgs make_args(mi_osqp_batch *h) {
  KernelArgs a{};
  a.n = (*h->anp).n; a.m = (*h->anp).m; a.N = (*h->anp).N; a.B = h->B;
  a.fwd = h->fwd.view((*h->anp).fwd); a.bwd = h->bwd.view((*h->anp).bwd); a.chk = h->chk.view((*h->anp).chk);
  a.pinv = h->pinv.p; a.xloc = h->xloc.p;
  a.fwd_val = h->fwd_val.p; a.bwd_val = h->bwd_val.p; a.chk_val = h->chk_val.p; a.dinv = h->dinv.p;
  a.fwd_val0 = h->fwd_val0.p; a.bwd_val0 = h->bwd_val0.p; a.dt_val0 = h->dt_val0.p;
  a.use_work = (h->fwd_val0.p && h->bwd_val0.p && (!(*h->anp).dt.k || h->dt_val0.p)) ? h->use_work.p : nullptr;
  a.x = h->x.p; a.z = h->z.p; a.y = h->y.p; a.q = h->q.p; a.l = h->l.p; a.u = h->u.p;
  a.rho_vec = h->rho_vec.p; a.rho_inv = h->rho_inv.p; a.Dsc = h->Dsc.p; a.Dsc_inv = h->Dsc_inv.p;
  a.Esc = h->Esc.p; a.Esc_inv = h->Esc_inv.p; a.dx = h->dx.p; a.dy = h->dy.p; a.out1 = h->out1.p; a.out2 = h->out2.p;
  a.dscal = h->dscal.p; a.iscal = h->iscal.p;
  a.x_out = h->x_out.p; a.y_out = h->y_out.p;
  a.xs_global = h->global_xs ? h->xs_global.p : nullptr; a.xs_len = (*h->anp).xs_total; a.wide = (*h->anp).wide ? 1 : 0;
  a.rs_off = h->rs_off; a.rf_off = h->rf_off;
  a.mw_groups = h->mw_groups; a.mw_bar = h->mw_bar.p; a.mw_scratch = h->mw_scratch.p;
  a.df = (*h->anp).df ? 1 : 0; a.df_shadow = (unsigned)(*h->anp).Next; a.rflag = h->rflag.p;
  {
    const DenseTail &dt = (*h->anp).dt;
    a.dt.s = dt.s; a.dt.k = dt.k; a.dt.n_phases = dt.n_phases; a.dt.n_steps = dt.n_steps;
    a.dt.task = h->dt_task.p; a.dt.wave_task = h->dt_wave_task.p; a.dt.wave_step = h->dt_wave_step.p; a.dt.tail_bar = h->dt_tail_bar.p;
    a.dt_val = h->dt_val.p;
  }
  const Settings &s = h->st;
  a.sigma = s.sigma; a.alpha = s.alpha; a.eps_abs = s.eps_abs; a.eps_rel = s.eps_rel;
  a.eps_prim_inf = s.eps_prim_inf; a.eps_dual_inf = s.eps_dual_inf; a.rho_tolerance = s.adaptive_rho_tolerance;
  a.check_termination = (int)s.check_termination; a.rho_interval = (int)s.adaptive_rho_interval;
  a.max_iter = (int)s.max_iter; a.scaled_termination = (int)s.scaled_termination; a.scaling = s.scaling ? 1 : 0;
  a.adaptive_rho = (int)s.adaptive_rho; a.iter_begin = 0; a.iter_end = 0; a.info_at_end = 1;
  return a;
}

static FactorArgs make_factor_args(mi_osqp_batch *h, int force_all) {
  FactorArgs a{};
  const Analysis &an = (*h->anp);
  a.n = an.n; a.m = an.m; a.N = an.N; a.B = h->B; a.nnzP = an.Pp[an.n]; a.nnzK = an.nnzK();
  a.pa_len = an.Pp[an.n] + an.Ap[an.n]; a.n_levels = an.bf.n_levels; a.force_all = force_all;
  a.storage = an.bf.storage; a.fwd = h->fwd.view(an.fwd); a.bwd = h->bwd.view(an.bwd);
  a.blk = h->bf_blk.p; a.lvl = h->bf_lvl.p; a.utask = h->bf_utask.p; a.tri4 = h->bf_tri.p; a.dtask = h->bf_dtask.p; a.ubig = h->bf_ubig.p;
  a.ttask = h->bf_ttask.p; a.asm_dst = h->bf_asm_dst.p; a.asm_src = h->bf_asm_src.p;
  a.fwd_srcblk = h->fwd_srcblk.p; a.bwd_srcblk = h->bwd_srcblk.p;
  a.pa_val = h->pa_val.p; a.l = h->l.p; a.u = h->u.p; a.dscal = h->dscal.p;
  a.rho_vec = h->rho_vec.p; a.rho_inv = h->rho_inv.p; a.Lblk = h->Lblk.p; a.Dl = h->Dl.p; a.dinv_scratch = h->dinv_scratch.p;
  a.fwd_val = h->fwd_val.p; a.bwd_val = h->bwd_val.p; a.dinv = h->dinv.p; a.iscal = h->iscal.p; a.npos = h->npos.p; a.use_work = h->use_work.p;
  a.sigma = h->st.sigma; a.home_bt = h->BT; a.dt_k = an.dt.k;
  a.mw_groups = 0; a.mw_bar = h->mw_bar.p;
#ifdef MI_OSQP_DEBUG_BUILD
  { const char *e = getenv("MI_OSQP_FACTOR_SKIP"); a.debug_skip = e ? atoi(e) : 0; }
#endif
  return a;
}

static int ensure_stage(mi_osqp_batch *h, size_t doubles, size_t ints) {
  int rc;
  if (h->stage.n < doubles && (rc = h->stage.alloc(doubles))) return rc;
  if (h->ids.n < ints && (rc = h->ids.alloc(ints))) return rc;
  return 0;
}

static int ensure_pin(mi_osqp_batch *h, size_t doubles) {
  if (h->pin_n >= doubles) return 0;
  if (h->pin) { hostpool::give(h->pin, h->pin_cap); h->pin = nullptr; h->pin_n = 0; }
  HIPCHK(hostpool::alloc((void **)&h->pin, doubles * sizeof(double), &h->pin_cap));
  h->pin_n = h->pin_cap / sizeof(double);
  return 0;
}
static void par_copy(double *dst, const double *src, size_t n) {
  const size_t chunk = (size_t)1 << 17;
  const int parts = (int)((n + chunk - 1) / chunk);
  if (parts <= 2) { memcpy(dst, src, n * sizeof(double)); return; }
  parallel_for(parts, [&](int i, int) { const size_t b = (size_t)i * chunk; memcpy(dst + b, src + b, std::min(chunk, n - b) * sizeof(double)); });
}

static int upload_rows(mi_osqp_batch *h, const std::vector<double> &rows, const std::vector<int> *ids, int nq,
                       int len, double *dst) {
  if (!nq || !len) return 0;
  int rc = ensure_stage(h, rows.size(), ids ? ids->size() : 0);
  if (rc) return rc;
  HIPCHK(hipMemcpyAsync(h->stage.p, rows.data(), rows.size() * sizeof(double), hipMemcpyHostToDevice, h->stream));
  if (ids) HIPCHK(hipMemcpyAsync(h->ids.p, ids->data(), ids->size() * sizeof(int), hipMemcpyHostToDevice, h->stream));
  HIPCHK(launch_interleave(h->stage.p, dst, ids ? h->ids.p : nullptr, nq, len, h->BT, h->stream));
  HIPCHK(hipStreamSynchronize(h->stream));
  return 0;
}

template <class G>
static std::vector<double> gather_rows(const std::vector<int> &ids, int len, G &&get) {
  std::vector<double> rows((size_t)ids.size() * len);
  for (size_t j = 0; j < ids.size(); j++) { const std::vector<double> &v = get(ids[j]); std::copy(v.begin(), v.begin() + len, rows.begin() + j * len); }
  return rows;
}

static int upload_rho(mi_osqp_batch *h, const std::vector<int> &ids) {
  int m = (*h->anp).m, nq = (int)ids.size(), rc;
  if (!nq || !m) return 0;
  std::vector<double> r1 = gather_rows(ids, m, [&](int q) -> const std::vector<double> & { return h->qp[q].rho_vec; });
  if ((rc = upload_rows(h, r1, &ids, nq, m, h->rho_vec.p))) return rc;
  std::vector<double> r2 = gather_rows(ids, m, [&](int q) -> const std::vector<double> & { return h->qp[q].rho_inv; });
  return upload_rows(h, r2, &ids, nq, m, h->rho_inv.p);
}

static int upload_problem(mi_osqp_batch *h, const std::vector<int> &ids, bool with_matrices) {
  const Analysis &an = (*h->anp);
  int n = an.n, m = an.m, nq = (int)ids.size(), rc;
  if (!nq) return 0;
  auto up = [&](int len, double *dst, auto get) -> int {
    std::vector<double> rows = gather_rows(ids, len, get);
    return upload_rows(h, rows, &ids, nq, len, dst);
  };
  if (with_matrices) {
    int nnzP = an.Pp[n], nnzA = an.Ap[n];
    std::vector<double> pa((size_t)nq * (nnzP + nnzA));
    for (int j = 0; j < nq; j++) {
      const QPNumeric &q = h->qp[ids[j]];
      std::copy(q.Pv.begin(), q.Pv.end(), pa.begin() + (size_t)j * (nnzP + nnzA));
      std::copy(q.Av.begin(), q.Av.end(), pa.begin() + (size_t)j * (nnzP + nnzA) + nnzP);
    }
    if ((rc = ensure_stage(h, std::max<size_t>(pa.size(), 1), ids.size()))) return rc;
    HIPCHK(hipMemcpyAsync(h->ids.p, ids.data(), ids.size() * sizeof(int), hipMemcpyHostToDevice, h->stream));
    if (!pa.empty()) {
      HIPCHK(hipMemcpyAsync(h->stage.p, pa.data(), pa.size() * sizeof(double), hipMemcpyHostToDevice, h->stream));
// ... 245 lines not shown

static int batch_setup_impl(mi_osqp_batch *h, int64_t B, int64_t n, int64_t m, const int64_t *Pp, const int64_t *Pi,
                            const double *Pv, const double *q, const int64_t *Ap, const int64_t *Ai,
                            const double *Av, const double *l, const double *u, int64_t device) {
  double t0 = now_s();
  if (B <= 0 || !Pp || !Ap || (m > 0 && (!l || !u)) || (Pp[n] > 0 && !Pv) || (Ap[n] > 0 && !Av)) return MI_OSQP_ERR_INVALID_DATA;
  if (validate_settings(h->st)) return MI_OSQP_ERR_INVALID_SETTINGS;
  if (h->st.adaptive_rho && !h->st.adaptive_rho_interval)
    h->st.adaptive_rho_interval = h->st.check_termination ? 4 * h->st.check_termination : 100;
  for (int64_t k = 0; k < B * m; k++) if (l[k] > u[k]) return MI_OSQP_ERR_INVALID_DATA;
  int BT = 1, max_extra = -1;
  const size_t lds_cap = 160 * 1024 - 1024;
  h->tune = tuning_from_env();
  const double ta0 = now_s();
  int rc = shape_and_analysis(h, B, n, m, Pp, Pi, Ap, Ai, device, BT, max_extra, h->anp);
  const double t_analysis = now_s() - ta0;
  if (rc) return rc;
  const Analysis &an = (*h->anp);
  h->B = (int)B;
  h->failed.assign((size_t)B, 0);
  int ndev = 0;
  if (hipGetDeviceCount(&ndev) != hipSuccess || ndev <= 0) { g_last_error = "no HIP device visible"; return MI_OSQP_ERR_DEVICE; }
  if (device >= ndev) { g_last_error = "no such HIP device"; return MI_OSQP_ERR_DEVICE; }
  if (device >= 0) h->device = (int)device; else HIPCHK(hipGetDevice(&h->device));
  DevGuard guard(h->device);
  hipDeviceProp_t prop;
  HIPCHK(hipGetDeviceProperties(&prop, h->device));
  h->n_cus = prop.multiProcessorCount > 0 ? prop.multiProcessorCount : 256;
  if (strncmp(prop.gcnArchName, "gfx950", 6) != 0) { g_last_error = std::string("device is not gfx950: ") + prop.gcnArchName; return MI_OSQP_ERR_DEVICE; }
  {
    streampool::Bundle sb;
    if (streampool::take(h->device, sb)) {
      h->stream = sb.stream; h->ev0 = sb.ev[0]; h->ev1 = sb.ev[1]; h->evf0 = sb.ev[2]; h->evf1 = sb.ev[3]; h->evf2 = sb.ev[4];
      h->pipe_r = sb.pipe_r; h->pipe_i = sb.pipe_i;
      for (int k = 0; k < streampool::kPipeEvents; k++) h->pipe_ev[k] = sb.pipe_ev[k];
    }
    else {
      HIPCHK(hipStreamCreateWithFlags(&h->stream, hipStreamNonBlocking));
      HIPCHK(hipEventCreate(&h->ev0)); HIPCHK(hipEventCreate(&h->ev1));
      HIPCHK(hipEventCreate(&h->evf0)); HIPCHK(hipEventCreate(&h->evf1)); HIPCHK(hipEventCreate(&h->evf2));
    }
  }
  h->BT = BT; h->ntiles = (int)((B + BT - 1) / BT);
  h->lds = h->global_xs ? lds_bytes(0, BT, h->threads) : lds_bytes(an.Next + 2 * an.dt.k, BT, h->threads);
  if (h->lds > lds_cap) { g_last_error = "internal: LDS budget exceeded"; return MI_OSQP_ERR_ALLOC; }
  h->lds_iter = h->lds; h->rs_off = 0;
  {
    const size_t state = sizeof(double) * (size_t)BT * (2 * (size_t)n + 6 * (size_t)m + (size_t)an.N);
    if (!h->tune.stream_state && !h->global_xs && h->mw_groups <= 0 && h->threads == 1024 && h->lds + state <= lds_cap) {
      h->rs_off = (int)(h->lds / sizeof(double)); h->lds_iter = h->lds + state;
    }
  }
  h->lds_factor = 0; h->rf_off = 0; h->rf_steps = 0;
  if (h->rs_off && BT == 1 && an.dt.k > 0 && !h->tune.stream_factor) {
    const size_t part = (size_t)(h->threads / 64) * rf_lds_steps() * 64 * sizeof(double);
    if (h->lds_iter + part <= lds_cap) {
      h->rf_off = (int)(h->lds_iter / sizeof(double)); h->lds_factor = part; h->rf_steps = rf_head_steps();
    }
  }
  size_t T = (size_t)h->ntiles * BT;
  if ((rc = h->fwd.upload(an.fwd)) || (rc = h->bwd.upload(an.bwd)) || (rc = h->chk.upload(an.chk))) return rc;
  { std::vector<uint32_t> pv(an.pinv.begin(), an.pinv.end()); if ((rc = h->pinv.upload(pv))) return rc; }
  { std::vector<uint32_t> xv(an.xloc.begin(), an.xloc.end()); if ((rc = h->xloc.upload(xv))) return rc; }
  {
    std::vector<int32_t> pr(an.Pi.begin(), an.Pi.begin() + an.Pp[n]), pc(an.Pp[n]), ar(an.Ai.begin(), an.Ai.begin() + an.Ap[n]), ac(an.Ap[n]);
    for (int j = 0; j < n; j++) { for (int k = an.Pp[j]; k < an.Pp[j + 1]; k++) pc[k] = j; for (int k = an.Ap[j]; k < an.Ap[j + 1]; k++) ac[k] = j; }
    if ((rc = h->rz_prow.upload(pr)) || (rc = h->rz_pcol.upload(pc)) || (rc = h->rz_arow.upload(ar)) || (rc = h->rz_acol.upload(ac))) return rc;
  }
  if ((rc = h->use_work.alloc(T)) || (rc = h->use_work.zero(h->stream))) return rc;
#define ALLOC(buf, len) if ((rc = h->buf.alloc((size_t)(len) * T)) || (rc = h->buf.zero(h->stream))) return rc
  ALLOC(fwd_val, (size_t)an.fwd.phys_steps() * 64); ALLOC(bwd_val, (size_t)an.bwd.phys_steps() * 64); ALLOC(chk_val, (size_t)an.chk.phys_steps() * 64); ALLOC(dinv, an.N);
  ALLOC(x, n); ALLOC(z, m); ALLOC(y, m); ALLOC(q, n); ALLOC(l, m); ALLOC(u, m); ALLOC(rho_vec, m); ALLOC(rho_inv, m);
  ALLOC(Dsc, n); ALLOC(Dsc_inv, n); ALLOC(Esc, m); ALLOC(Esc_inv, m); ALLOC(dx, n); ALLOC(dy, m);
  ALLOC(out1, 2 * n + m); ALLOC(out2, 2 * n + m); ALLOC(dscal, DS_COUNT);
  if (h->global_xs) { ALLOC(xs_global, an.xs_total); }
  if ((rc = h->mw_bar.alloc(4 * (size_t)std::max(h->n_cus, 1))) || (rc = h->mw_bar.zero(h->stream))) return rc;
  if (an.df && ((rc = h->rflag.upload(an.rflag)) || (rc = h->mw_scratch.alloc((size_t)8 * 256 * 16)) || (rc = h->mw_scratch.zero(h->stream)))) return rc;
  if (an.dt.k) {
    const DenseTail &dt = an.dt;
    ALLOC(dt_val, (size_t)dt.n_steps * 64);
    if ((rc = h->dt_task.upload(dt.task)) || (rc = h->dt_wave_task.upload(dt.wave_task)) || (rc = h->dt_wave_step.upload(dt.wave_step)) ||
        (rc = h->dt_tail_bar.upload(dt.tail_bar)) || (rc = h->dt_src.upload(dt.src)) ||
        (rc = h->dt_lt_pos.upload(dt.lt_pos)) || (rc = h->dt_ltcol_col.upload(dt.ltcol_col)) || (rc = h->dt_tile_tab.upload(dt.tile_tab)) ||
        (rc = h->dt_wave_tiles.upload(dt.wave_tiles)) || (rc = h->dt_asm_q64.upload(dt.asm_q64)) ||
        (rc = h->dt_src_tile.upload(dt.src_tile)) || (rc = h->dt_diag_tile.upload(dt.diag_tile)) || (rc = h->dt_task_step.upload(dt.task_step)) ||
        (rc = h->dt_Sd.alloc((size_t)dt.k * dt.k * (T + 4)))) return rc;
    const int nrt = dt.k / 16 - 4;
    h->dt_nh = nrt <= 14 ? std::max(nrt, 1) : (nrt + 1) / 2;
    h->dt_cs_doubles = (uint32_t)std::max(h->dt_nh * 1024, 64 * 65 + 63) / 64 * 64;
    h->dt_lds = std::max<size_t>((size_t)h->dt_cs_doubles + 4096, 2 * 64 * 65) * sizeof(double);
    h->dt_lds_asm = (dt.asm_lds_bytes() + 255) & ~(size_t)255;
    if (h->dt_lds > lds_cap || h->dt_lds_asm > lds_cap) { g_last_error = "internal: LDS budget of tail_kernel exceeded"; return MI_OSQP_ERR_ALLOC; }
  }
#undef ALLOC
  if ((rc = h->iscal.alloc((size_t)IS_COUNT * T)) || (rc = h->flag.alloc(4))) return rc;
  {
    const BlockFactor &bf = an.bf;
    if ((rc = h->bf_blk.upload(bf.blk)) || (rc = h->bf_lvl.upload(bf.lvl)) || (rc = h->bf_ubig.upload(bf.ubig)) || (rc = h->bf_utask.upload(bf.utask4)) ||
        (rc = h->bf_tri.upload(bf.tri4)) || (rc = h->bf_dtask.upload(bf.dtask4)) || (rc = h->bf_ttask.upload(bf.ttask4)) ||
        (rc = h->bf_asm_dst.upload(bf.asm_dst)) || (rc = h->bf_asm_src.upload(bf.asm_src)) ||
        (rc = h->fwd_srcblk.upload(an.fwd_srcblk)) || (rc = h->bwd_srcblk.upload(an.bwd_srcblk))) return rc;
    if ((rc = h->pa_val.alloc((size_t)(an.Pp[n] + an.Ap[n]) * T)) || (rc = h->pa_val.zero(h->stream)) ||
        (rc = h->Lblk.alloc((size_t)bf.storage * (T + 4))) || (rc = h->Dl.alloc((size_t)an.N * (T + 4))) || (rc = h->Dl.zero(h->stream)) ||
        (rc = h->dinv_scratch.alloc((size_t)an.N * (T + 4))) || (rc = h->npos.alloc(T))) return rc;
    HIPCHK(hostpool::alloc((void **)&h->h_npos, T * sizeof(int), &h->h_npos_cap));
  }
  if (!h->global_xs && an.Pp[n] + an.Ap[n] < 65536 && n + m < 65536 &&
      spmv_fused_lds_bytes((int)n, (int)m, an.Pp[n] + an.Ap[n], BT) <= 150 * 1024) {
    const int nnzP = an.Pp[n];
    std::vector<std::vector<uint32_t>> rows((size_t)2 * n + m);
    for (int c = 0; c < (int)n; c++)
      for (int k = an.Pp[c]; k < an.Pp[c + 1]; k++) {
        const int r = an.Pi[k];
        rows[r].push_back((uint32_t)k | ((uint32_t)c << 16));
        if (r != c) rows[c].push_back((uint32_t)k | ((uint32_t)r << 16));
      }
    for (int c = 0; c < (int)n; c++)
      for (int k = an.Ap[c]; k < an.Ap[c + 1]; k++) {
        const int r = an.Ai[k];
        rows[(size_t)n + c].push_back((uint32_t)(nnzP + k) | ((uint32_t)(n + r) << 16));
        rows[(size_t)2 * n + r].push_back((uint32_t)(nnzP + k) | ((uint32_t)c << 16));
      }
    std::vector<uint32_t> ptr{0u}, ent;
    for (auto &rw : rows) { ent.insert(ent.end(), rw.begin(), rw.end()); ptr.push_back((uint32_t)ent.size()); }
    if ((rc = h->sp_ptr.upload(ptr)) || (rc = h->sp_ent.upload(ent))) return rc;
    const size_t nrows = rows.size();
    size_t maxlen = 0;
    for (auto &rw : rows) maxlen = std::max(maxlen, rw.size());
    if (nrows <= 4 * 512 && maxlen <= 24) {
      std::vector<uint32_t> order(nrows);
      for (size_t r = 0; r < nrows; r++) order[r] = (uint32_t)r;
      std::stable_sort(order.begin(), order.end(), [&](uint32_t x, uint32_t y) { return rows[x].size() > rows[y].size(); });
      const int npass = (int)((nrows + 511) / 512);
      std::vector<uint32_t> ell, rowid((size_t)npass * 512, 0xFFFFFFFFu);
      const uint32_t pad = (uint32_t)(an.Pp[n] + an.Ap[n]) | ((uint32_t)(n + m) << 16);
      for (int p = 0; p < npass; p++) {
        const size_t r0 = (size_t)p * 512, r1 = std::min(nrows, r0 + 512);
        const uint32_t K = (uint32_t)rows[order[r0]].size();
        h->sp_ell_off[p] = (uint32_t)ell.size(); h->sp_ell_k[p] = K;
        ell.resize(ell.size() + (size_t)K * 512, pad);
        for (size_t r = r0; r < r1; r++) {
          rowid[r] = order[r];
          const auto &rw = rows[order[r]];
          for (size_t k = 0; k < rw.size(); k++) ell[h->sp_ell_off[p] + k * 512 + (r - r0)] = rw[k];
        }
      }
      h->sp_npass = npass;
      if ((rc = h->sp_ell.upload(ell)) || (rc = h->sp_rowid.upload(rowid))) return rc;
    }
  }
  if ((rc = h->x_out.alloc((size_t)B * n)) || (rc = h->y_out.alloc((size_t)B * std::max<int64_t>(m, 1)))) return rc;
  if ((rc = h->rawP.alloc((size_t)B * std::max(an.Pp[n], 1))) || (rc = h->rawq.alloc((size_t)B * n))) return rc;
  if ((rc = h->x_out.zero(h->stream)) || (rc = h->y_out.zero(h->stream))) return rc;
  HIPCHK(hostpool::alloc((void **)&h->h_iscal, (size_t)IS_COUNT * T * sizeof(int), &h->h_iscal_cap));
  HIPCHK(hostpool::alloc((void **)&h->h_dscal, (size_t)DS_COUNT * T * sizeof(double), &h->h_dscal_cap));
  if ((rc = ensure_pin(h, std::max((size_t)2 * B * m, (size_t)B * n)))) return rc;
  HIPCHK(hipStreamSynchronize(h->stream));
  double t1 = now_s();
  h->qp.resize(B);
  int nnzPin = (int)Pp[n], nnzA = (int)Ap[n];
  const int CH = 128;
  double t_factor = 0.0, t_upload = 0.0;
  const bool dev_ruiz = !host_ruiz(h);
  for (int c0 = 0; c0 < B; c0 += CH) {
    int c1 = (int)std::min<int64_t>(B, c0 + CH);
    double ta = now_s();
    std::vector<char> dup(c1 - c0, 0);
// ... 37 lines not shown
    for (int i = 0; i < B; i++) all[i] = i;
    size_t cnt = (size_t)DS_COUNT * T;
    for (size_t k = 0; k < cnt; k++) h->h_dscal[k] = 0.0;
    HIPCHK(hipMemcpy(h->dscal.p, h->h_dscal, cnt * sizeof(double), hipMemcpyHostToDevice));
    if ((rc = sync_scalars_to_device(h, all, !dev_ruiz))) return rc;
  }
  if (dev_ruiz) {
    double tb = now_s();
    const size_t cA = (size_t)B * nnzA, cb = (size_t)B * m, cpa = (size_t)B * (an.Pp[n] + nnzA);
    if ((rc = ensure_pin(h, cA + 2 * cb + 1)) || (rc = ensure_stage(h, cA + 2 * cb + cpa + 1, (size_t)B))) return rc;
    par_copy(h->pin, Av, cA);
    if (m) { par_copy(h->pin + cA, l, cb); par_copy(h->pin + cA + cb, u, cb); }
    HIPCHK(hipMemcpyAsync(h->stage.p, h->pin, (cA + 2 * cb) * sizeof(double), hipMemcpyHostToDevice, h->stream));
    RuizArgs r{};
    r.n = (int)n; r.m = (int)m; r.nnzP = an.Pp[n]; r.nnzA = nnzA; r.B = (int)B; r.BT = BT; r.iters = (int)h->st.scaling;
    r.ids = nullptr; r.fresh = 1; r.rawP = h->rawP.p; r.rawq = h->rawq.p;
    r.Prow = h->rz_prow.p; r.Pcol = h->rz_pcol.p; r.Arow = h->rz_arow.p; r.Acol = h->rz_acol.p;
    r.rawA = h->stage.p; r.rawl = h->stage.p + cA; r.rawu = h->stage.p + cA + cb;
    r.pa_val = h->pa_val.p; r.q = h->q.p; r.Dsc = h->Dsc.p; r.Dsc_inv = h->Dsc_inv.p; r.Esc = h->Esc.p; r.Esc_inv = h->Esc_inv.p;
    r.l = h->l.p; r.u = h->u.p; r.dscal = h->dscal.p;
    r.dn = h->out1.p; r.en = h->out1.p + (size_t)B * n;
    r.pa_out = h->stage.p + cA + 2 * cb;
    HIPCHK(launch_ruiz(r, h->stream));
    std::vector<int> ids(B);
    for (int i = 0; i < (int)B; i++) ids[i] = i;
    HIPCHK(hipMemcpyAsync(h->ids.p, ids.data(), ids.size() * sizeof(int), hipMemcpyHostToDevice, h->stream));
    HIPCHK(launch_scatter(r.pa_out, h->chk_val.p, h->chk.src.p, h->ids.p, (int)B, an.Pp[n] + nnzA, h->chk.view(an.chk), BT, h->stream));
    HIPCHK(hipStreamSynchronize(h->stream));
    h->host_scaling_stale = true; h->host_bounds_stale = true; h->host_rho_stale = true;
    t_factor += now_s() - tb;
  }
  {
    double tb = now_s();
    std::vector<int> all(B);
    for (int i = 0; i < (int)B; i++) all[i] = i;
    if ((rc = refactor_qps(h, std::move(all)))) return rc;
    t_factor += now_s() - tb;
  }
  if ((rc = reset_solve_state(h, true))) return rc;
  if ((rc = snapshot(h))) return rc;
  HIPCHK(hipStreamSynchronize(h->stream));
  mi_osqp_stats &s = h->stats;
  s.n = n; s.m = m; s.N = an.N; s.batch = B; s.tile = BT; s.n_tiles = h->ntiles;
  s.nnz_P_triu = an.Pp[n]; s.nnz_A = nnzA; s.nnz_KKT = an.nnzK(); s.nnz_L = an.nnzL();
  s.n_supernodes = (int64_t)an.sn_start.size() - 1; s.n_blocks = (int64_t)an.chunk_start.size() - 1;
  s.fwd_levels = an.fwd.n_phases; s.bwd_levels = an.bwd.n_phases;
  s.fwd_slots = (int64_t)an.fwd.phys_steps() * 64; s.bwd_slots = (int64_t)an.bwd.phys_steps() * 64; s.chk_slots = (int64_t)an.chk.phys_steps() * 64;
  s.lds_bytes = (int64_t)h->lds; s.threads_per_block = h->threads;
  s.dense_tail_rows = an.dt.k; s.dense_tail_slots = (int64_t)an.dt.n_steps * 64;
  s.setup_seconds_host = t1 - t0; s.setup_seconds_factor = t_factor; s.setup_seconds_upload = t_upload;
  s.nnz_L_before_tail = an.dt.k ? an.Lp[an.dt.s] : an.nnzL();
  s.solve_groups = h->mw_groups; s.solve_group_threads = h->mw_groups > 0 ? h->mw_threads : 0;
  s.resident_state = h->rs_off ? 1 : 0; s.lds_bytes_iterate = (int64_t)h->lds_iter;
  s.resident_factor_steps = h->rf_steps; s.lds_bytes_factor = (int64_t)h->lds_factor;
  dense_tail_deal_stats(an.dt, s);
  if (getenv("MI_OSQP_DEBUG_TIMING"))
    fprintf(stderr, "[mi_osqp] setup B=%d N=%d: analysis+alloc %.1f ms (analysis %.1f), numeric %.1f ms, upload %.1f ms, rest %.1f ms\n", (int)B, an.N,
            1e3 * (t1 - t0), 1e3 * t_analysis, 1e3 * t_factor, 1e3 * t_upload, 1e3 * (now_s() - t1 - t_factor - t_upload));
  return MI_OSQP_OK;
}


static int fail_slots(mi_osqp_batch *h, const KernelArgs &a, const std::vector<int> &bad, int iter) {
  if (bad.empty()) return 0;
  int rc;
  if (h->fail_list.n < bad.size() && (rc = h->fail_list.alloc(std::max<size_t>(bad.size(), (size_t)h->ntiles * h->BT)))) return rc;
  HIPCHK(hipMemcpyAsync(h->fail_list.p, bad.data(), bad.size() * sizeof(int), hipMemcpyHostToDevice, h->stream));
  HIPCHK(launch_fail_slots(a, h->fail_list.p, (int)bad.size(), h->BT, iter, h->stream));
  HIPCHK(hipStreamSynchronize(h->stream));
  for (int q : bad) if (q >= 0 && q < h->B) h->failed[q] = 1;
  return 0;
}

static TailArgs make_tail_args(mi_osqp_batch *h, int kbt, const int *work) {
  const DenseTail &dt = (*h->anp).dt;
  TailArgs da{};
  da.n = (*h->anp).n; da.N = (*h->anp).N; da.s = dt.s; da.k = dt.k; da.kbt = kbt; da.home_bt = h->BT;
  da.storage = (*h->anp).bf.storage; da.n_slots = dt.n_steps * 64u; da.n_lt = dt.n_lt; da.n_ltcol = dt.n_ltcol; da.n_quads = (uint32_t)(dt.asm_q64.size() / 64);
  da.nh = h->dt_nh; da.cs_doubles = h->dt_cs_doubles; da.work = work;
  da.lt_pos = h->dt_lt_pos.p; da.ltcol_col = h->dt_ltcol_col.p; da.tile_tab = h->dt_tile_tab.p; da.wave_tiles = h->dt_wave_tiles.p;
  da.dt_task = h->dt_task.p; da.dt_task_step = h->dt_task_step.p; da.n_tasks = (uint32_t)(dt.task.size() / 4);
  da.asm_q64 = h->dt_asm_q64.p; da.diag_tile = h->dt_diag_tile.p; da.src_tile = h->dt_src_tile.p;
  da.Lblk = h->Lblk.p; da.Dl = h->Dl.p; da.Sd = h->dt_Sd.p; da.dt_val = h->dt_val.p; da.dinv = h->dinv.p; da.npos = h->npos.p; da.iscal = h->iscal.p;
  return da;
}

static int device_refactor_slots(mi_osqp_batch *h, std::vector<int> work, std::vector<int> *bad, const PolishArgs *pol = nullptr) {
  if (work.empty()) return 0;
  const int BT = h->BT;
  int rc;
  FactorArgs fa = make_factor_args(h, 0);
  if (pol) {
    fa.pmask = pol->act; fa.arow = h->rz_arow.p; fa.pstat = pol->stat; fa.pdelta = h->st.delta; fa.sigma = h->st.delta;
    fa.fwd_val = h->pol_fwd.p; fa.bwd_val = h->pol_bwd.p; fa.dinv = h->pol_dinv.p; fa.use_work = nullptr;
  }
  const int nq = (int)work.size();
  const int kbt = nq <= h->n_cus ? 1 : BT;
  const int wtiles = (nq + kbt - 1) / kbt;
  work.resize((size_t)wtiles * kbt, -1);
  if (h->work.n < work.size() && (rc = h->work.alloc((size_t)h->ntiles * BT + 4))) return rc;
  HIPCHK(hipMemcpyAsync(h->work.p, work.data(), work.size() * sizeof(int), hipMemcpyHostToDevice, h->stream));
  fa.work = h->work.p;
  if (kbt == 1 && h->mw_bar.p && (*h->anp).N >= 1000) {
    const int cap = h->B == 1 ? std::max(4, std::min(64, (*h->anp).N / 600)) : 8;
    int G = h->tune.factor_groups ? h->tune.factor_groups : cap;
    G = std::min(G, std::max(1, h->n_cus / wtiles));
    static const int resident = max_coresident_factor_groups(h->tune.factor_threads, 1);
    if (resident > 0) G = std::min(G, std::max(1, resident * h->n_cus / wtiles));
    fa.mw_groups = G > 1 ? G : 0;
  }
  std::unique_lock<std::mutex> spin_lock(spin_mutex(h->device), std::defer_lock);
  if (fa.mw_groups > 1) spin_lock.lock();
  HIPCHK(hipEventRecord(h->evf0, h->stream));
  if (fa.mw_groups > 1) HIPCHK(hipMemsetAsync(h->mw_bar.p, 0, 4 * sizeof(uint32_t) * (size_t)wtiles, h->stream));
  HIPCHK(launch_factor(fa, kbt, wtiles, h->tune.factor_threads, h->stream));
  HIPCHK(hipEventRecord(h->evf1, h->stream));
  if ((*h->anp).dt.k) {
    TailArgs da = make_tail_args(h, kbt, h->work.p);
    if (pol) { da.dt_val = h->pol_dt.p; da.dinv = h->pol_dinv.p; da.pstat = pol->stat; }
    unsigned long long *d_trace = nullptr;
    const bool tracing = getenv("MI_OSQP_TAIL_TRACE") != nullptr;
    if (tracing) { HIPCHK(hipMalloc((void **)&d_trace, (size_t)wtiles * kbt * 8 * sizeof(unsigned long long))); HIPCHK(hipMemsetAsync(d_trace, 0, (size_t)wtiles * kbt * 64, h->stream)); }
    da.trace = d_trace;
    HIPCHK(launch_tail(da, wtiles * kbt, h->dt_lds_asm, h->dt_lds, h->stream));
    if (tracing) {
      std::vector<unsigned long long> tr((size_t)wtiles * kbt * 8);
      HIPCHK(hipStreamSynchronize(h->stream));
      HIPCHK(hipMemcpy(tr.data(), d_trace, tr.size() * sizeof(unsigned long long), hipMemcpyDeviceToHost));
      (void)hipFree(d_trace);
      double sum[8] = {0, 0, 0, 0, 0, 0, 0, 0};
      for (size_t i = 0; i < tr.size(); i++) sum[i % 8] += (double)tr[i] / (wtiles * kbt);
      fprintf(stderr, "[mi_osqp] tail_kernel, %d QPs, mean shader clocks of wave 0 per QP: assembly %.0f, pivot blocks %.0f, panel stores %.0f, stream write %.0f; "
              "staging %.0f, Gn %.0f, trailing %.0f, barrier waits of the panel phase %.0f\n", wtiles * kbt, sum[0], sum[1], sum[2], sum[3], sum[4], sum[5], sum[6], sum[7]);
    }
  }
  HIPCHK(hipEventRecord(h->evf2, h->stream));
  HIPCHK(hipMemcpyAsync(h->h_iscal, h->iscal.p, (size_t)h->ntiles * IS_COUNT * BT * sizeof(int), hipMemcpyDeviceToHost, h->stream));
  HIPCHK(hipStreamSynchronize(h->stream));
  if (spin_lock.owns_lock()) spin_lock.unlock();
  if (fa.mw_groups > 1) {
    std::vector<uint32_t> w(4 * (size_t)wtiles, 0u);
    HIPCHK(hipMemcpy(w.data(), h->mw_bar.p, w.size() * sizeof(uint32_t), hipMemcpyDeviceToHost));
    for (int t = 0; t < wtiles; t++)
      if (w[4 * (size_t)t + 2]) {
        if (!pol) for (int sl : work) if (sl >= 0 && sl < h->B) h->failed[(size_t)sl] = 1;
        g_last_error = "refactorisation on several workgroups: a barrier of the group timed out"; return MI_OSQP_ERR_DEVICE;
      }
  }
  if (pol) return 0;
  {
    float f = 0.f, d = 0.f;
    HIPCHK(hipEventElapsedTime(&f, h->evf0, h->evf1)); HIPCHK(hipEventElapsedTime(&d, h->evf1, h->evf2));
    h->factor_ms_sum += f; h->dense_ms_sum += (*h->anp).dt.k ? d : 0.0; h->refactor_launches++; h->refactor_qps += nq;
    if (nq >= h->peak_qps) { h->peak_qps = nq; h->peak_factor_ms = f; h->peak_tail_ms = (*h->anp).dt.k ? d : 0.0; }
  }
  for (int s : work)
    if (s >= 0 && h->h_iscal[(size_t)(s / BT) * IS_COUNT * BT + IS_NEED_REFACTOR * BT + s % BT] < 0) {
      if (getenv("MI_OSQP_DEBUG_TIMING")) {
        (void)hipMemcpy(h->h_npos, h->npos.p, (size_t)h->ntiles * BT * sizeof(int), hipMemcpyDeviceToHost);
        fprintf(stderr, "[mi_osqp] slot %d: %d positive pivots, expected %d\n", s, h->h_npos[s], (*h->anp).n);
      }
      if (bad) bad->push_back(s);
    }
  return 0;
}

static int refactor_qps(mi_osqp_batch *h, std::vector<int> qps) {
  if (qps.empty()) return 0;
  std::vector<int> bad;
  const std::vector<int> listed = qps;
  int rc = device_refactor_slots(h, std::move(qps), &bad);
  if (rc) return rc;
  for (int q : listed) h->failed[q] = 0;
  if ((rc = fail_slots(h, make_args(h), bad, 0))) return rc;
  if ((int)bad.size() == h->B) { g_last_error = "the KKT factor lost its inertia"; return MI_OSQP_ERR_NONCONVEX; }
  return 0;
}

static int polish_impl(mi_osqp_batch *h, const KernelArgs &a) {
  const Analysis &an = (*h->anp);
  const int BT = h->BT, ntl = h->ntiles;
  const size_t T = (size_t)ntl * BT;
  int rc;
  h->pol_count = h->pol_accepted = 0; h->pol_seconds = 0.0;
  h->pol_status.assign((size_t)h->B, 0);
  if (!h->pol_stat.p) {
    if ((rc = h->pol_fwd.alloc(h->fwd_val.n)) || (rc = h->pol_fwd.zero(h->stream)) || (rc = h->pol_bwd.alloc(h->bwd_val.n)) ||
        (rc = h->pol_bwd.zero(h->stream)) || (rc = h->pol_dinv.alloc(h->dinv.n)) || (rc = h->pol_dinv.zero(h->stream)) ||
        (rc = h->pol_sol.alloc(T * an.N)) || (rc = h->pol_act.alloc(std::max<size_t>(1, T * an.m))) || (rc = h->pol_act.zero(h->stream)) ||
        (rc = h->pol_stat.alloc(T)) || (rc = h->pol_stat.zero(h->stream))) return rc;
    if (an.dt.k && ((rc = h->pol_dt.alloc(h->dt_val.n)) || (rc = h->pol_dt.zero(h->stream)))) return rc;
    if (!h->evp0) HIPCHK(hipEventCreate(&h->evp0));
    if (!h->evp1) HIPCHK(hipEventCreate(&h->evp1));
  }
  std::vector<int> work;
  for (int q = 0; q < h->B; q++)
    if (h->h_iscal[(size_t)(q / BT) * IS_COUNT * BT + IS_STATUS * BT + q % BT] == 1) work.push_back(q);
  PolishArgs pa{h->pol_stat.p, h->pol_act.p, h->pol_sol.p, (int)h->st.polish_refine_iter};
  HIPCHK(hipEventRecord(h->evp0, h->stream));
  HIPCHK(launch_polish_active(a, pa, BT, h->stream));
  const int n_pol = (int)work.size();
  if (n_pol) {
// ... 1075 lines not shown
  HIPCHK(hipStreamSynchronize(h->stream));
  const size_t icnt = (size_t)h->ntiles * IS_COUNT * h->BT;
  HIPCHK(hipMemcpy(h->h_iscal, h->iscal.p, icnt * sizeof(int), hipMemcpyDeviceToHost));
  for (int q = 0; q < h->B; q++) {
    h->failed[q] = h->h_iscal[(size_t)(q / h->BT) * IS_COUNT * h->BT + IS_NEED_REFACTOR * h->BT + q % h->BT] < 0;
    if (c.clear_rho[q]) h->clear_rho_updates = true;
  }
  HIPCHK(hipMemcpy(h->x_out.p, c.xh, (size_t)h->B * (*h->anp).n * sizeof(double), hipMemcpyHostToDevice));
  if ((*h->anp).m) HIPCHK(hipMemcpy(h->y_out.p, c.yh, (size_t)h->B * (*h->anp).m * sizeof(double), hipMemcpyHostToDevice));
  c.on = false; c.n_running = 0;
  h->host_bounds_stale = h->host_rho_stale = true;
  return MI_OSQP_OK;
}

struct RingSpan { char *host; char *dev; };
static int ring_take(mi_osqp_batch *h, size_t bytes, RingSpan &out) {
  mi_osqp_batch::Cont &c = h->cont;
  bytes = (bytes + 255) & ~(size_t)255;
  if (bytes > c.ring_cap) { g_last_error = "per-QP call larger than the staging ring"; return MI_OSQP_ERR_ALLOC; }
  if (c.ring_head + bytes > c.ring_cap) { HIPCHK(hipStreamSynchronize(h->stream)); c.ring_head = 0; }
  out.host = c.ring_h + c.ring_head; out.dev = c.ring_d.p + c.ring_head;
  c.ring_head += bytes;
  return MI_OSQP_OK;
}
static int ring_reserve(mi_osqp_batch *h, size_t bytes, int spans) {
  mi_osqp_batch::Cont &c = h->cont;
  bytes += (size_t)256 * (size_t)spans;
  if (bytes > c.ring_cap) { g_last_error = "per-QP call larger than the staging ring"; return MI_OSQP_ERR_ALLOC; }
  if (c.ring_head + bytes > c.ring_cap) { HIPCHK(hipStreamSynchronize(h->stream)); c.ring_head = 0; }
  return MI_OSQP_OK;
}
static int ring_upload(mi_osqp_batch *h, const RingSpan &sp, size_t bytes) {
  if (bytes) HIPCHK(hipMemcpyAsync(sp.dev, sp.host, bytes, hipMemcpyHostToDevice, h->stream));
  return MI_OSQP_OK;
}

static int cont_check_ids(mi_osqp_batch *h, int64_t n_ids, const int64_t *ids, bool must_be_idle) {
  if (n_ids < 0 || (n_ids > 0 && !ids)) return MI_OSQP_ERR_NULL;
  if (n_ids > h->B) return MI_OSQP_ERR_INVALID_DATA;
  for (int64_t j = 0; j < n_ids; j++) {
    if (ids[j] < 0 || ids[j] >= h->B) return MI_OSQP_ERR_INVALID_DATA;
    if (must_be_idle && h->cont.running[(size_t)ids[j]]) { g_last_error = "QP " + std::to_string(ids[j]) + " is still iterating"; return MI_OSQP_ERR_INVALID_DATA; }
  }
  return MI_OSQP_OK;
}

static int cont_stage_ids(mi_osqp_batch *h, int64_t n_ids, const int64_t *ids, int **d_ids, int **d_sel) {
  const int nslots = h->ntiles * h->BT;
  RingSpan sp;
  int rc = ring_take(h, ((size_t)n_ids + (d_sel ? (size_t)nslots : 0)) * sizeof(int), sp);
  if (rc) return rc;
  int *hi = (int *)sp.host;
  for (int64_t j = 0; j < n_ids; j++) hi[j] = (int)ids[j];
  if (d_sel) {
    int *hs = hi + n_ids;
    for (int sl = 0; sl < nslots; sl++) hs[sl] = 0;
    for (int64_t j = 0; j < n_ids; j++) hs[ids[j]] = (int)j + 1;
    *d_sel = (int *)sp.dev + n_ids;
  }
  *d_ids = (int *)sp.dev;
  return ring_upload(h, sp, ((size_t)n_ids + (d_sel ? (size_t)nslots : 0)) * sizeof(int));
}

static int snapshot_some(mi_osqp_batch *h, const int *d_ids, int nq, hipStream_t st) {
  const Analysis &an = (*h->anp);
  HIPCHK(launch_copy_slot_streams(h->fwd_val0.p, h->fwd_val.p, d_ids, nq, (size_t)an.fwd.phys_steps() * 64, st));
  HIPCHK(launch_copy_slot_streams(h->bwd_val0.p, h->bwd_val.p, d_ids, nq, (size_t)an.bwd.phys_steps() * 64, st));
  if (an.dt.k) HIPCHK(launch_copy_slot_streams(h->dt_val0.p, h->dt_val.p, d_ids, nq, (size_t)an.dt.n_steps * 64, st));
  HIPCHK(launch_copy_slot_rows(h->dinv0.p, h->dinv.p, d_ids, nq, an.N, h->BT, st));
  HIPCHK(launch_copy_slot_rows(h->rho_vec0.p, h->rho_vec.p, d_ids, nq, an.m, h->BT, st));
  HIPCHK(launch_copy_slot_rows(h->rho_inv0.p, h->rho_inv.p, d_ids, nq, an.m, h->BT, st));
  HIPCHK(launch_copy_slot_rows(h->dscal0.p, h->dscal.p, d_ids, nq, DS_COUNT, h->BT, st));
  return MI_OSQP_OK;
}

static int enqueue_refactor_list(mi_osqp_batch *h, const int *d_work, int count) {
  if (count <= 0) return MI_OSQP_OK;
  const Analysis &an = (*h->anp);
  hipStream_t st = h->stream;
  FactorArgs fa = make_factor_args(h, 0);
  fa.work = d_work; fa.mw_groups = 0;
  HIPCHK(launch_factor(fa, 1, count, h->tune.factor_threads, st));
  if (an.dt.k) {
    const DenseTail &dt = an.dt;
    TailArgs da{};
    da.n = an.n; da.N = an.N; da.s = dt.s; da.k = dt.k; da.kbt = 1; da.home_bt = h->BT;
    da.storage = an.bf.storage; da.n_slots = dt.n_steps * 64u; da.n_lt = dt.n_lt; da.n_ltcol = dt.n_ltcol; da.n_quads = (uint32_t)(dt.asm_q64.size() / 64);
    da.nh = h->dt_nh; da.cs_doubles = h->dt_cs_doubles; da.work = d_work;
    da.lt_pos = h->dt_lt_pos.p; da.ltcol_col = h->dt_ltcol_col.p; da.tile_tab = h->dt_tile_tab.p; da.wave_tiles = h->dt_wave_tiles.p;
    da.dt_task = h->dt_task.p; da.dt_task_step = h->dt_task_step.p; da.n_tasks = (uint32_t)(dt.task.size() / 4);
    da.asm_q64 = h->dt_asm_q64.p; da.diag_tile = h->dt_diag_tile.p; da.src_tile = h->dt_src_tile.p;
    da.Lblk = fa.Lblk; da.Dl = fa.Dl; da.Sd = h->dt_Sd.p; da.dt_val = h->dt_val.p; da.dinv = h->dinv.p; da.npos = h->npos.p; da.iscal = h->iscal.p;
    da.trace = nullptr;
    HIPCHK(launch_tail(da, count, h->dt_lds_asm, h->dt_lds, st));
  }
  return MI_OSQP_OK;
}

static int cont_new_data(mi_osqp_batch *h, int64_t n_ids, const int64_t *ids, const double *Av, const double *l, const double *u, bool fresh,
                         const double *dA = nullptr, const double *dl = nullptr, const double *du = nullptr) {
  const Analysis &an = (*h->anp);
  const int n = an.n, m = an.m, nnzP = an.Pp[n], nnzA = an.Ap[n], pa_len = nnzP + nnzA, nq = (int)n_ids;
  int rc;
  if (!dA) for (size_t k = 0; k < (size_t)nq * m; k++) if (l[k] > u[k]) return MI_OSQP_ERR_INVALID_DATA;
  int *d_ids = nullptr;
  const size_t cA = (size_t)nq * nnzA, cb = (size_t)nq * m, cpa = (size_t)nq * pa_len;
  if ((rc = ring_reserve(h, (size_t)nq * sizeof(int) + (dA ? 0 : (cA + 2 * cb) * sizeof(double)) + std::max<size_t>(cpa, 1) * sizeof(double), 3))) return rc;
  if ((rc = cont_stage_ids(h, n_ids, ids, &d_ids, nullptr))) return rc;
  RingSpan in{nullptr, nullptr}, out;
  if (!dA && (rc = ring_take(h, (cA + 2 * cb) * sizeof(double), in))) return rc;
  if ((rc = ring_take(h, std::max<size_t>(cpa, 1) * sizeof(double), out))) return rc;
  double *hin = (double *)in.host, *din = (double *)in.dev;
  if (!dA) {
    memcpy(hin, Av, cA * sizeof(double)); memcpy(hin + cA, l, cb * sizeof(double)); memcpy(hin + cA + cb, u, cb * sizeof(double));
    if ((rc = ring_upload(h, in, (cA + 2 * cb) * sizeof(double)))) return rc;
  }
  hipStream_t us = h->stream;
  if (!dA && h->cont.keepA) {
    HIPCHK(launch_keep_rows(h->cont.keepA, din, d_ids, nq, nnzA, us));
    HIPCHK(launch_keep_rows(h->cont.keepl, din + cA, d_ids, nq, m, us));
    HIPCHK(launch_keep_rows(h->cont.keepu, din + cA + cb, d_ids, nq, m, us));
  }
  KernelArgs ka = make_args(h);
  if (fresh) HIPCHK(launch_fresh_slots(ka, d_ids, nq, h->BT, h->st.rho, us));
  RuizArgs r{};
  r.n = n; r.m = m; r.nnzP = nnzP; r.nnzA = nnzA; r.B = nq; r.BT = h->BT; r.iters = (int)h->st.scaling;
  r.ids = d_ids; r.fresh = fresh ? 1 : 0; r.rawP = h->rawP.p; r.rawq = h->rawq.p;
  r.Prow = h->rz_prow.p; r.Pcol = h->rz_pcol.p; r.Arow = h->rz_arow.p; r.Acol = h->rz_acol.p;
  if (dA) { r.rawA = dA; r.rawl = dl; r.rawu = du; r.raw_by_qp = 1; }
  else { r.rawA = din; r.rawl = din + cA; r.rawu = din + cA + cb; }
  r.pa_val = h->pa_val.p; r.q = h->q.p; r.Dsc = h->Dsc.p; r.Dsc_inv = h->Dsc_inv.p; r.Esc = h->Esc.p; r.Esc_inv = h->Esc_inv.p;
  r.l = h->l.p; r.u = h->u.p; r.dscal = h->dscal.p;
  r.dn = h->cont.rz_scratch.p; r.en = h->cont.rz_scratch.p + (size_t)h->B * n;
  r.pa_out = (double *)out.dev;
  HIPCHK(launch_ruiz(r, us));
  HIPCHK(launch_scatter(r.pa_out, h->chk_val.p, h->chk.src.p, d_ids, nq, pa_len, h->chk.view(an.chk), h->BT, us));
  if ((rc = enqueue_refactor_list(h, d_ids, nq))) return rc;
  if ((rc = snapshot_some(h, d_ids, nq, us))) return rc;
  for (int64_t j = 0; j < n_ids; j++) { h->cont.clear_rho[(size_t)ids[j]] = 1; h->failed[(size_t)ids[j]] = 0; }
  h->host_scaling_stale = true; h->host_bounds_stale = true; h->host_rho_stale = true;
  return MI_OSQP_OK;
}

extern "C" {

int mi_osqp_batch_reinit_some(mi_osqp_batch *h, int64_t n_ids, const int64_t *ids, const double *Av, const double *l, const double *u) {
  CallTimer timer_("batch_reinit_some");
  if (!h || (n_ids > 0 && (!Av || !l || !u))) return MI_OSQP_ERR_NULL;
  DevGuard guard(h->device);
  int rc;
  if ((rc = cont_enter(h)) || (rc = cont_check_ids(h, n_ids, ids, true))) return rc;
  if (!n_ids) return MI_OSQP_OK;
  return cont_new_data(h, n_ids, ids, Av, l, u, true);
}

int mi_osqp_batch_update_A_bounds_some(mi_osqp_batch *h, int64_t n_ids, const int64_t *ids, const double *Av, const double *l, const double *u) {
  CallTimer timer_("batch_update_A_bounds_some");
  if (!h || (n_ids > 0 && (!Av || !l || !u))) return MI_OSQP_ERR_NULL;
  DevGuard guard(h->device);
  int rc;
  if ((rc = cont_enter(h)) || (rc = cont_check_ids(h, n_ids, ids, true))) return rc;
  if (!n_ids) return MI_OSQP_OK;
  return cont_new_data(h, n_ids, ids, Av, l, u, false);
}

int mi_osqp_batch_warm_start_x_some(mi_osqp_batch *h, int64_t n_ids, const int64_t *ids, const double *x) {
  CallTimer timer_("batch_warm_start_x_some");
  if (!h || (n_ids > 0 && !x)) return MI_OSQP_ERR_NULL;
  DevGuard guard(h->device);
  int rc;
  if ((rc = cont_enter(h)) || (rc = cont_check_ids(h, n_ids, ids, true))) return rc;
  if (!n_ids) return MI_OSQP_OK;
  h->st.warm_start = 1;
  const size_t cnt = (size_t)n_ids * (*h->anp).n;
  int *d_ids = nullptr, *d_sel = nullptr;
// ... 563 lines not shown
  return multi_fan_out(h, [&](size_t k) { return mi_osqp_batch_update_P(h->shard[k], Pp, Pi, Pv + h->begin[k] * nnzP); });
}
int mi_osqp_multi_batch_update_P_A(mi_osqp_multi *h, const int64_t *Pp, const int64_t *Pi, const double *Pv, const int64_t *Ap,
                                   const int64_t *Ai, const double *Av) {
  if (!h || !Pp || !Pi || !Pv || !Ap || !Ai || !Av) return MI_OSQP_ERR_NULL;
  const int64_t nnzP = Pp[h->n], nnzA = Ap[h->n];
  return multi_fan_out(h, [&](size_t k) {
    return mi_osqp_batch_update_P_A(h->shard[k], Pp, Pi, Pv + h->begin[k] * nnzP, Ap, Ai, Av + h->begin[k] * nnzA);
  });
}
int mi_osqp_multi_batch_warm_start_y(mi_osqp_multi *h, const double *y) {
  if (!h || !y) return MI_OSQP_ERR_NULL;
  return multi_fan_out(h, [&](size_t k) { return mi_osqp_batch_warm_start_y(h->shard[k], y + h->begin[k] * h->m); });
}
int mi_osqp_multi_batch_solve(mi_osqp_multi *h) {
  if (!h) return MI_OSQP_ERR_NULL;
  return multi_fan_out(h, [&](size_t k) { return mi_osqp_batch_solve(h->shard[k]); });
}
int mi_osqp_multi_batch_solve_async(mi_osqp_multi *h) {
  if (!h) return MI_OSQP_ERR_NULL;
  if (h->async_pending) { const int rc0 = multi_join(h); if (rc0) return rc0; }
  const size_t ns = h->count();
  if (h->worker.size() != ns) {
    h->worker.clear();
    for (size_t k = 0; k < ns; k++) { h->worker.emplace_back(new ShardWorker()); h->worker.back()->start(); }
  }
  for (size_t k = 0; k < ns; k++) { mi_osqp_batch *b = h->shard[k]; h->worker[k]->post([b]() -> int { return mi_osqp_batch_solve(b); }); }
  h->async_pending = true;
  return MI_OSQP_OK;
}
int mi_osqp_multi_batch_wait(mi_osqp_multi *h) {
  if (!h) return MI_OSQP_ERR_NULL;
  return h->async_pending ? multi_join(h) : (int)MI_OSQP_OK;
}
int mi_osqp_multi_batch_get_primal(mi_osqp_multi *h, double *x) {
  if (!h || !x) return MI_OSQP_ERR_NULL;
  return multi_fan_out(h, [&](size_t k) { return mi_osqp_batch_get_primal(h->shard[k], x + h->begin[k] * h->n); });
}
int mi_osqp_multi_batch_get_dual(mi_osqp_multi *h, double *y) {
  if (!h || !y) return MI_OSQP_ERR_NULL;
  return multi_fan_out(h, [&](size_t k) { return mi_osqp_batch_get_dual(h->shard[k], y + h->begin[k] * h->m); });
}
int mi_osqp_multi_batch_get_info(mi_osqp_multi *h, mi_osqp_info *info) {
  if (!h || !info) return MI_OSQP_ERR_NULL;
  return multi_fan_out(h, [&](size_t k) { return mi_osqp_batch_get_info(h->shard[k], info + h->begin[k]); });
}


int mi_osqp_debug_host_kkt_solve(int64_t n, int64_t m, const int64_t *Pp, const int64_t *Pi, const double *Pv,
                                 const int64_t *Ap, const int64_t *Ai, const double *Av, const double *l,
                                 const double *u, const mi_osqp_settings *settings, int64_t tile, const double *rhs,
                                 double *sol_schedule, double *sol_direct, mi_osqp_stats *st) {
  Settings s = to_settings(settings);
  if (validate_settings(s)) return MI_OSQP_ERR_INVALID_SETTINGS;
  Analysis an;
  const Tuning tu = tuning_from_env();
  const AnalysisTuning tune = tu.analysis;
  const int nwaves = tu.threads ? tu.threads / 64 : 8;
  int rc = tile > 1 ? analyze(n, m, Pp, Pi, Ap, Ai, tune, an, 8, 1, -1, 0, (int)tile - 1) : analyze(n, m, Pp, Pi, Ap, Ai, tune, an, nwaves);
  if (rc) return rc;
  QPNumeric Q;
  load_qp(an, s, Pv, nullptr, Av, l, u, Q);
  if (s.scaling) scale_qp(an, s, Q);
  set_rho_vec(an, s, Q);
  std::vector<double> w;
  if ((rc = factor_qp(an, s, Q, w))) return rc;
  if (sol_direct) direct_kkt_solve(an, Q, rhs, sol_direct);
  if (sol_schedule && !replay_kkt_solve(an, Q, rhs, sol_schedule)) {
    g_last_error = "schedule streams are not race-free / deadlock-free"; return MI_OSQP_ERR_INVALID_DATA;
  }
  if (st) {
    memset(st, 0, sizeof(*st));
    st->n = n; st->m = m; st->N = an.N; st->batch = 1; st->tile = 1; st->n_tiles = 1;
    st->nnz_P_triu = an.Pp[n]; st->nnz_A = an.Ap[n]; st->nnz_KKT = an.nnzK(); st->nnz_L = an.nnzL();
    st->n_supernodes = (int64_t)an.sn_start.size() - 1; st->n_blocks = (int64_t)an.chunk_start.size() - 1;
    st->fwd_levels = an.fwd.n_phases; st->bwd_levels = an.bwd.n_phases;
    st->fwd_slots = (int64_t)an.fwd.phys_steps() * 64; st->bwd_slots = (int64_t)an.bwd.phys_steps() * 64; st->chk_slots = (int64_t)an.chk.phys_steps() * 64;
    st->dense_tail_rows = an.dt.k; st->dense_tail_slots = (int64_t)an.dt.n_steps * 64;
    st->nnz_L_before_tail = an.dt.k ? an.Lp[an.dt.s] : an.nnzL();
    st->threads_per_block = 64 * (tile > 1 ? 8 : nwaves);
    dense_tail_deal_stats(an.dt, *st);
  }
  return MI_OSQP_OK;
}

int mi_osqp_debug_host_block_factor(int64_t n, int64_t m, const int64_t *Pp, const int64_t *Pi, const double *Pv,
                                    const int64_t *Ap, const int64_t *Ai, const double *Av, const double *l,
                                    const double *u, const mi_osqp_settings *settings, double *dL, double *dD,
                                    int64_t *counts) {
  Settings s = to_settings(settings);
  if (validate_settings(s)) return MI_OSQP_ERR_INVALID_SETTINGS;
  Analysis an;
  int rc = analyze(n, m, Pp, Pi, Ap, Ai, tuning_from_env().analysis, an);
  if (rc) return rc;
  QPNumeric Q, R;
  load_qp(an, s, Pv, nullptr, Av, l, u, Q);
  if (s.scaling) scale_qp(an, s, Q);
  set_rho_vec(an, s, Q);
  std::vector<double> w;
  if ((rc = factor_qp(an, s, Q, w))) return rc;
  if ((rc = replay_block_factor(an, s, Q, R))) return rc;
  double mL = 0.0, sL = 1e-300, mD = 0.0;
  const int ts = an.dt.k ? an.dt.s : an.N;
  for (int k = 0; k < an.Lp[ts]; k++) { mL = std::max(mL, std::fabs(Q.Lx[k] - R.Lx[k])); sL = std::max(sL, std::fabs(Q.Lx[k])); }
  for (size_t k = (size_t)an.nnzL(); k < Q.Lx.size(); k++) { mL = std::max(mL, std::fabs(Q.Lx[k] - R.Lx[k])); sL = std::max(sL, std::fabs(Q.Lx[k])); }
  for (int k = 0; k < ts; k++) mD = std::max(mD, std::fabs(Q.Dlinv[k] - R.Dlinv[k]) / std::fabs(Q.Dlinv[k]));
  if (an.dt.k) {
    double mM = 0.0, sM = 1e-300;
    for (size_t k = 0; k < Q.Minv.size(); k++) { mM = std::max(mM, std::fabs(Q.Minv[k] - R.Minv[k])); sM = std::max(sM, std::fabs(Q.Minv[k])); }
    mL = std::max(mL, mM / sM * sL);
  }
  if (dL) *dL = mL / sL;
  if (dD) *dD = mD;
  if (counts) {
    counts[0] = (int64_t)an.bf.n_blocks(); counts[1] = (int64_t)an.bf.tri.size() / 2;
    counts[2] = an.bf.storage; counts[3] = an.bf.n_levels;
  }
  return MI_OSQP_OK;
}

}
```

Measured before the change: 38710.

## Assemble dense-tail tile initial values directly from QP data instead of block storage

Tail KKT entries are no longer scattered into the block-factor storage and zeroed there. A per-tile init table now encodes each tile element's source (P, A, or rho_inv, plus polish masks), and the tail kernel gathers the values straight from pa_val and rho_inv with software-pipelined buffer loads two tiles ahead. The factor kernel's zeroing and assembly now cover only the pre-tail prefix (zero_len), which cuts memory writes and reads for the dense tail. In exchange the tail kernel does extra indirect loads, and overflow checks are added for layouts where tail storage overlaps non-tail data.

Result: no change. 39090, median of 6 (+1.0%).

```diff
diff --git a/include/mi_osqp.h b/include/mi_osqp.h
--- a/include/mi_osqp.h
+++ b/include/mi_osqp.h
@@ -238,6 +238,11 @@
                                     const double *l, const double *u, const mi_osqp_settings *settings,
                                     double *max_rel_diff_L, double *max_rel_diff_Dinv, int64_t *counts);
 
+int mi_osqp_debug_host_tail_init(int64_t n, int64_t m, const int64_t *P_colptr, const int64_t *P_rowidx,
+                                 const int64_t *A_colptr, const int64_t *A_rowidx,
+                                 int64_t *info, int64_t *perm, int64_t *entries, int64_t capacity);
+int mi_osqp_batch_debug_tail_init(mi_osqp_batch *h, int64_t *info, int64_t *perm, int64_t *entries, int64_t capacity);
+
 int mi_osqp_debug_refactor_chunks(int64_t n_flagged, const int64_t *flagged, int64_t n_active, const int64_t *active, int64_t tile,
                                   int64_t chunk_qps, int64_t max_chunks, int64_t *n_chunks, int64_t *work_begin, int64_t *tiles,
                                   int64_t *tile_begin);
diff --git a/osqp-solver_amd/__init__.py b/osqp-solver_amd/__init__.py
--- a/osqp-solver_amd/__init__.py
+++ b/osqp-solver_amd/__init__.py
@@ -164,6 +164,8 @@
         L.mi_osqp_prefetch_analysis.argtypes = [C.c_int64, C.c_int64, C.c_int64, ip, ip, ip, ip, C.c_int64]
         L.mi_osqp_debug_host_block_factor.argtypes = [C.c_int64, C.c_int64, ip, ip, dp, ip, ip, dp, dp, dp,
                                                       C.POINTER(Settings), dp, dp, ip]
+        L.mi_osqp_debug_host_tail_init.argtypes = [C.c_int64, C.c_int64, ip, ip, ip, ip, ip, ip, ip, C.c_int64]
+        L.mi_osqp_batch_debug_tail_init.argtypes = [vp, ip, ip, ip, C.c_int64]
         _LIB = L
     return _LIB
 
@@ -660,3 +662,25 @@
                                            C.byref(s), C.byref(dL), C.byref(dD), cnt)
     _chk(rc, "debug_host_block_factor")
     return dL.value, dD.value, dict(blocks=cnt[0], triples=cnt[1], storage=cnt[2], levels=cnt[3])
+
+
+def _tail_init(call, N):
+    info, perm = np.zeros(8, dtype=np.int64), np.zeros(N, dtype=np.int64)
+    _chk(call(_ip(info), _ip(perm), None, 0), "debug_tail_init")
+    ent = np.zeros((max(int(info[3]), 1), 6), dtype=np.int64)
+    _chk(call(_ip(info), _ip(perm), _ip(ent), int(info[3])), "debug_tail_init")
+    keys = ("k", "s", "tiles", "entries", "zero_len", "storage", "asm_entries", "nnz_KKT")
+    return dict(zip(keys, (int(v) for v in info))), ent[:int(info[3])], perm
+
+
+def debug_host_tail_init(P, A):
+    L = lib()
+    P, A = _csc(P), _csc(A)
+    n, m = A.shape[1], A.shape[0]
+    Pp, Pi, Ap, Ai = _i64(P.indptr), _i64(P.indices), _i64(A.indptr), _i64(A.indices)
+    return _tail_init(lambda i, p, e, c: L.mi_osqp_debug_host_tail_init(n, m, _ip(Pp), _ip(Pi), _ip(Ap), _ip(Ai), i, p, e, c), n + m)
+
+
+def debug_batch_tail_init(solver):
+    L = lib()
+    return _tail_init(lambda i, p, e, c: L.mi_osqp_batch_debug_tail_init(solver._h, i, p, e, c), solver.n + solver.m)
diff --git a/osqp-solver_amd/csrc/device_types.h b/osqp-solver_amd/csrc/device_types.h
--- a/osqp-solver_amd/csrc/device_types.h
+++ b/osqp-solver_amd/csrc/device_types.h
@@ -63,6 +63,7 @@
   int n, m, N, B, nnzP, nnzK, pa_len, n_levels, force_all;
   int debug_skip;
   uint32_t storage;
+  uint32_t zero_len;
   SchedDev fwd, bwd;
   const uint32_t *blk, *lvl, *utask, *tri4, *dtask, *ttask, *asm_dst, *asm_src;
   const uint32_t *ubig;
@@ -101,6 +102,12 @@
   int *npos, *iscal;
   unsigned long long *trace;
   int *pstat;
+  const uint64_t *init_tab;
+  uint32_t n_init;
+  int m, pa_len;
+  const double *pa_val, *rho_inv;
+  double sigma, pdelta;
+  const signed char *pmask;
 };
 hipError_t launch_tail(const TailArgs &a, int nwork, size_t lds_asm, size_t lds, hipStream_t st);
 
diff --git a/osqp-solver_amd/csrc/host_core.cpp b/osqp-solver_amd/csrc/host_core.cpp
--- a/osqp-solver_amd/csrc/host_core.cpp
+++ b/osqp-solver_amd/csrc/host_core.cpp
@@ -832,6 +832,47 @@
   for (int pos : an.sigmaOnlyK) bf.asm_src[pos] = (uint32_t)ASM_SIGMA << 29;
   for (int k = 0; k < an.Ap[n]; k++) bf.asm_src[an.AtoK[k]] = ((uint32_t)ASM_A << 29) | (uint32_t)k;
   for (int r = 0; r < m; r++) bf.asm_src[an.rhotoK[r]] = ((uint32_t)ASM_NEG_RHOINV << 29) | (uint32_t)r;
+  bf.zero_len = bf.storage;
+  std::vector<uint32_t> tile_init;
+  if (an.dt.k) {
+    DenseTail &dt = an.dt;
+    const uint32_t tail_off = bf.blk[4 * find_blk(ct0, ct0)];
+    for (size_t id = 0; id < bf.n_blocks(); id++) {
+      const uint32_t off = bf.blk[4 * id], hw = bf.blk[4 * id + 3], len = (hw >> 8) * (hw & 255u);
+      const bool in_tail = chunk_of[bf.blk[4 * id + 2]] >= ct0;
+      if (in_tail ? off < tail_off : off + len > tail_off) bf.overflow = true;
+    }
+    for (size_t t = 0; t < bf.utask4.size() / 4; t++) if (bf.utask4[4 * t] >= tail_off) bf.overflow = true;
+    for (size_t t = 0; t < bf.dtask4.size() / 4; t++) if (bf.dtask4[4 * t] >= tail_off) bf.overflow = true;
+    for (size_t t = 0; t < bf.ttask4.size() / 4; t++) if (bf.ttask4[4 * t] >= tail_off || bf.ttask4[4 * t + 3] >= tail_off) bf.overflow = true;
+    for (size_t q = 0; q < bf.tri4.size() / 4; q++) if (bf.tri4[4 * q] >= tail_off || bf.tri4[4 * q + 1] >= tail_off) bf.overflow = true;
+    if (an.Pp[n] + an.Ap[n] >= (1 << 27) || m >= (1 << 27)) bf.overflow = true;
+    const int nt = an.dt.k / 16, nnzP = an.Pp[n];
+    tile_init.assign((size_t)nt * (nt + 1) / 2, 0u);
+    dt.init_tab.assign(256, 0xFFFFFFFFull);
+    size_t kept = 0;
+    for (int e = 0; e < nnzK; e++) {
+      const int a = an.pinv[an.Ki[e]], b = an.pinv[colOfK[e]], r = std::max(a, b), c = std::min(a, b);
+      if (c < ts) {
+        if (bf.asm_dst[e] >= tail_off) bf.overflow = true;
+        bf.asm_dst[kept] = bf.asm_dst[e]; bf.asm_src[kept] = bf.asm_src[e]; kept++;
+        continue;
+      }
+      const uint32_t kind = bf.asm_src[e] >> 29, idx = bf.asm_src[e] & 0x1FFFFFFFu;
+      uint64_t lo = 0xFFFFFFFFull, hi = (uint64_t)kind << 29;
+      if (kind == ASM_P || kind == ASM_P_SIGMA) lo = idx;
+      else if (kind == ASM_A) { lo = (uint64_t)nnzP + idx; hi |= (uint32_t)an.Ai[idx]; }
+      else if (kind == ASM_NEG_RHOINV) hi |= idx;
+      const int i = r - ts, j = c - ts, I = i / 16, J = j / 16;
+      uint32_t &blk = tile_init[(size_t)I * (I + 1) / 2 + J];
+      if (!blk) { blk = (uint32_t)(dt.init_tab.size() / 256); dt.init_tab.resize(dt.init_tab.size() + 256, 0xFFFFFFFFull); }
+      auto put = [&](int row, int col) { dt.init_tab[(size_t)blk * 256 + (size_t)(row / 4) * 64 + (size_t)(row % 4) * 16 + col] = lo | (hi << 32); };
+      put(i % 16, j % 16);
+      if (I == J && i != j) put(j % 16, i % 16);
+    }
+    bf.asm_dst.resize(kept); bf.asm_src.resize(kept);
+    bf.zero_len = tail_off;
+  }
   bf.lpos.assign(an.nnzLx(), 0);
   for (int j = 0; j < N; j++) for (int p = an.Lp[j]; p < an.Lp[j + 1]; p++) bf.lpos[p] = (int32_t)pos_of(an.Li[p], j);
   for (int c = 0; c < nch; c++) {
@@ -847,6 +888,7 @@
   };
   compose(an.fwd, an.fwd_srcblk);
   compose(an.bwd, an.bwd_srcblk);
+  for (const auto *mp : {&an.fwd_srcblk, &an.bwd_srcblk}) for (int32_t v : *mp) if (v >= 0 && (uint32_t)v >= bf.zero_len) bf.overflow = true;
   if (an.dt.k) {
     const int k = an.dt.k;
     an.dt.sblk.assign((size_t)k * k, 0u);
@@ -865,6 +907,7 @@
         if (frag[I].empty() || frag[I].back().first != ci) frag[I].push_back({ci, std::vector<uint16_t>(16, 0xFFFFu)});
         frag[I].back().second[(i - ts) % 16] = (uint16_t)dt.lt_pos.size();
         dt.lt_pos.push_back((uint32_t)bf.lpos[p]);
+        if ((uint32_t)bf.lpos[p] >= bf.zero_len) bf.overflow = true;
       }
     }
     dt.n_lt = (int)dt.lt_pos.size(); dt.n_ltcol = (int)dt.ltcol_col.size();
@@ -905,8 +948,7 @@
             for (int e = 0; e < 16; e++) dt.asm_q.push_back(real ? ((uint32_t)fa->second[e] | ((uint32_t)fb->second[e] << 16)) : ((uint32_t)zero_slot | ((uint32_t)zero_slot << 16)));
           }
         }
-        const uint32_t blk_id = find_blk(ct0 + t.I, ct0 + t.J);
-        dt.tile_tab.insert(dt.tile_tab.end(), {((uint32_t)t.I << 16) | (uint32_t)t.J, bf.blk[4 * blk_id], q0, (uint32_t)(dt.asm_q.size() / 64)});
+        dt.tile_tab.insert(dt.tile_tab.end(), {((uint32_t)t.I << 16) | (uint32_t)t.J, tile_init[(size_t)t.I * (t.I + 1) / 2 + t.J], q0, (uint32_t)(dt.asm_q.size() / 64)});
       }
     }
     dt.wave_tiles[nw] = (uint32_t)(dt.tile_tab.size() / 4);
@@ -1624,18 +1666,16 @@
   const BlockFactor &bf = an.bf;
   const int n = an.n, N = an.N;
   std::vector<double> S(bf.storage, 0.0), D(N, 0.0);
-  for (int e = 0; e < an.nnzK(); e++) {
-    uint32_t kind = bf.asm_src[e] >> 29, idx = bf.asm_src[e] & 0x1FFFFFFFu;
-    double v = 0.0;
+  auto kkt_value = [&](uint32_t kind, uint32_t idx) {
     switch (kind) {
-      case ASM_P: v = qp.Pv[idx]; break;
-      case ASM_P_SIGMA: v = qp.Pv[idx] + st.sigma; break;
-      case ASM_SIGMA: v = st.sigma; break;
-      case ASM_A: v = qp.Av[idx]; break;
-      default: v = -qp.rho_inv[idx]; break;
-    }
-    S[bf.asm_dst[e]] = v;
-  }
+      case ASM_P: return qp.Pv[idx];
+      case ASM_P_SIGMA: return qp.Pv[idx] + st.sigma;
+      case ASM_SIGMA: return st.sigma;
+      case ASM_A: return qp.Av[idx];
+      default: return -qp.rho_inv[idx];
+    }
+  };
+  for (size_t e = 0; e < bf.asm_src.size(); e++) S[bf.asm_dst[e]] = kkt_value(bf.asm_src[e] >> 29, bf.asm_src[e] & 0x1FFFFFFFu);
   auto B = [&](uint32_t id, uint32_t &off, uint32_t &r0, uint32_t &c0, uint32_t &h, uint32_t &w) {
     off = bf.blk[4 * id]; r0 = bf.blk[4 * id + 1]; c0 = bf.blk[4 * id + 2]; h = bf.blk[4 * id + 3] >> 8; w = bf.blk[4 * id + 3] & 255u;
   };
@@ -1698,11 +1738,14 @@
       for (int e = 0; e < dt.n_lt; e++) La[e] = S[dt.lt_pos[e]];
       for (int ci = 0; ci < dt.n_ltcol; ci++) Dc[ci] = D[dt.ltcol_col[ci]];
       for (size_t t = 0; t < dt.tile_tab.size() / 4; t++) {
-        const uint32_t I = dt.tile_tab[4 * t] >> 16, J = dt.tile_tab[4 * t] & 0xFFFFu, boff = dt.tile_tab[4 * t + 1];
+        const uint32_t I = dt.tile_tab[4 * t] >> 16, J = dt.tile_tab[4 * t] & 0xFFFFu;
+        const uint64_t *init = &dt.init_tab[(size_t)dt.tile_tab[4 * t + 1] * 256];
         double tile[16][16];
         for (int r = 0; r < 16; r++) for (int c = 0; c < 16; c++) {
-          const int rr = (I == J && r < c) ? c : r, cc = (I == J && r < c) ? r : c;
-          tile[r][c] = S[boff + (uint32_t)cc * 16 + (uint32_t)rr];
+          const uint64_t w = init[(r / 4) * 64 + (r % 4) * 16 + c];
+          const uint32_t lo = (uint32_t)w, hi = (uint32_t)(w >> 32), kind = hi >> 29;
+          if (lo == 0xFFFFFFFFu && hi == 0u) tile[r][c] = 0.0;
+          else tile[r][c] = kkt_value(kind, kind == ASM_A ? lo - (uint32_t)an.Pp[n] : kind == ASM_NEG_RHOINV ? (hi & 0x1FFFFFFFu) : lo);
         }
         for (uint32_t q = dt.tile_tab[4 * t + 2]; q < dt.tile_tab[4 * t + 3]; q++)
           for (int r = 0; r < 16; r++) for (int c = 0; c < 16; c++) {
diff --git a/osqp-solver_amd/csrc/host_core.hpp b/osqp-solver_amd/csrc/host_core.hpp
--- a/osqp-solver_amd/csrc/host_core.hpp
+++ b/osqp-solver_amd/csrc/host_core.hpp
@@ -91,6 +91,7 @@
 
 struct BlockFactor {
   uint32_t storage = 0;
+  uint32_t zero_len = 0;
   std::vector<uint32_t> blk;
   std::vector<uint32_t> lvl;
   std::vector<uint32_t> utask;
@@ -125,6 +126,7 @@
   std::vector<uint32_t> lt_pos;
   std::vector<uint32_t> ltcol_col;
   std::vector<uint32_t> tile_tab;
+  std::vector<uint64_t> init_tab;
   std::vector<uint32_t> wave_tiles;
   std::vector<uint32_t> asm_q;
   std::vector<uint16_t> asm_qcol;
diff --git a/osqp-solver_amd/csrc/kernels.hip b/osqp-solver_amd/csrc/kernels.hip
--- a/osqp-solver_amd/csrc/kernels.hip
+++ b/osqp-solver_amd/csrc/kernels.hip
@@ -1988,7 +1988,7 @@
     }
   }
   {
-    const size_t tot = (size_t)a.storage * BT, pairs = tot / 2;
+    const size_t tot = (size_t)a.zero_len * BT, pairs = tot / 2;
     double2 *L2p = reinterpret_cast<double2 *>(Lb);
     for (size_t e = tid; e < pairs; e += nthr) L2p[e] = make_double2(0.0, 0.0);
     if (tid == 0 && (tot & 1)) Lb[tot - 1] = 0.0;
@@ -2201,7 +2201,6 @@
   double *A = a.Sd + (size_t)g * k * k;
   const double *Lb = a.Lblk + (size_t)wt * a.storage * kbt + wb;
   const double *Dl = a.Dl + (size_t)wt * a.N * kbt + wb;
-  const int l15 = lane & 15, l4 = lane >> 4;
   {
     double *La = smem, *Dc = smem + a.n_lt + 1;
     for (int e = tid; e < a.n_lt; e += nthr) La[e] = Lb[(size_t)a.lt_pos[e] * kbt];
@@ -2212,14 +2211,43 @@
     const uint32_t t_begin = a.wave_tiles[wave], t_end = a.wave_tiles[wave + 1];
     if (t_begin < t_end) {
       const uint4 *ttab = reinterpret_cast<const uint4 *>(a.tile_tab);
-      auto load_init = [&](const uint4 &tt) {
-        const int I = (int)(tt.x >> 16), J = (int)(tt.x & 0xFFFFu);
+      const size_t hbt = (size_t)a.home_bt, home = (size_t)slot / hbt, hb = (size_t)slot % hbt;
+      const uint32_t vsh = hbt == 4 ? 5u : hbt == 2 ? 4u : 3u;
+      auto qp_rsrc = [&](const double *base, int len) {
+        return len > 0 ? make_rsrc(base + (home * (size_t)len) * hbt + hb, (uint32_t)((((size_t)len - 1) * hbt + 1) * 8)) : make_rsrc(nullptr, 0u);
+      };
+      const mi_rsrc r_pa = qp_rsrc(a.pa_val, a.pa_len), r_rho = qp_rsrc(a.rho_inv, a.m);
+      const bool polish = a.pmask != nullptr;
+      const mi_rsrc r_pm = polish ? make_rsrc(a.pmask + (size_t)slot * a.m, (uint32_t)a.m) : make_rsrc(nullptr, 0u);
+      const mi_rsrc r_init = make_rsrc(a.init_tab, a.n_init * 2048u);
+      const double sigma = a.sigma, neg_pdelta = -a.pdelta;
+      mi_u32x2 iw[4];
+      mi_u32x2 ipa[4], irho[4];
+      uint32_t ipm[4], ihi[4];
+      auto init_words = [&](uint32_t blk) {
+#pragma unroll
+        for (int r = 0; r < 4; r++) iw[r] = __builtin_amdgcn_raw_buffer_load_b64(r_init, (uint32_t)lane * 8u, (blk * 4u + (uint32_t)r) * 512u, 0);
+      };
+      auto init_loads = [&]() {
+#pragma unroll
+        for (int r = 0; r < 4; r++) {
+          const uint32_t hi = iw[r].y, kind = hi >> 29, i2 = hi & 0x1FFFFFFFu;
+          ihi[r] = hi;
+          ipa[r] = __builtin_amdgcn_raw_buffer_load_b64(r_pa, iw[r].x << vsh, 0, 0);
+          irho[r] = __builtin_amdgcn_raw_buffer_load_b64(r_rho, kind == 4u ? i2 << vsh : 0xFFFFFFF8u, 0, 0);
+          ipm[r] = __builtin_amdgcn_raw_buffer_load_b8(r_pm, kind == 3u ? i2 : 0xFFFFFFFFu, 0, 0);
+        }
+      };
+      auto init_value = [&]() {
         mi_v4d v;
 #pragma unroll
         for (int r = 0; r < 4; r++) {
-          int row = l4 + 4 * r, col = l15;
-          if (I == J && row < col) { const int t = row; row = col; col = t; }
-          v[r] = Lb[((size_t)tt.y + (size_t)col * 16 + row) * kbt];
+          const uint32_t kind = ihi[r] >> 29;
+          const double pa = __hiloint2double((int)ipa[r].y, (int)ipa[r].x), ri = __hiloint2double((int)irho[r].y, (int)irho[r].x);
+          double x = (kind == 1u || kind == 2u) ? pa + sigma : pa;
+          x = (kind == 3u && polish && ipm[r] == 0u) ? 0.0 : x;
+          x = kind == 4u ? (polish ? neg_pdelta : -ri) : x;
+          v[r] = x;
         }
         return v;
       };
@@ -2239,11 +2267,14 @@
       if (a.n_quads) { fetch(qnext); qnext += QB; }
       const char *lds = reinterpret_cast<const char *>(smem);
       const uint32_t dc_off = (uint32_t)(a.n_lt + 1) * 8u;
-      mi_v4d acc_next = load_init(ttab[t_begin]);
+      init_words(ttab[t_begin].y);
+      init_loads();
+      init_words(ttab[t_begin + 1 < t_end ? t_begin + 1 : t_begin].y);
       for (uint32_t ti = t_begin; ti < t_end; ti++) {
         const uint4 tt = ttab[ti];
-        mi_v4d acc = acc_next;
-        acc_next = load_init(ttab[ti + 1 < t_end ? ti + 1 : ti]);
+        mi_v4d acc = init_value();
+        init_loads();
+        init_words(ttab[ti + 2 < t_end ? ti + 2 : t_end - 1].y);
         for (uint32_t q = tt.z; q < tt.w; q += QB) {
           mi_u32x2 cur[QB];
 #pragma unroll
diff --git a/osqp-solver_amd/csrc/solver.hip b/osqp-solver_amd/csrc/solver.hip
--- a/osqp-solver_amd/csrc/solver.hip
+++ b/osqp-solver_amd/csrc/solver.hip
@@ -276,7 +276,7 @@
   DevBuf<double> pa_val, Lblk, Dl, dinv_scratch;
   DevBuf<uint32_t> dt_task, dt_wave_task, dt_wave_step, dt_tail_bar;
   DevBuf<uint32_t> dt_lt_pos, dt_ltcol_col, dt_tile_tab, dt_wave_tiles, dt_diag_tile, dt_task_step;
-  DevBuf<uint64_t> dt_asm_q64;
+  DevBuf<uint64_t> dt_asm_q64, dt_init_tab;
   DevBuf<int32_t> dt_src_tile;
   int dt_nh = 0; uint32_t dt_cs_doubles = 0; size_t dt_lds = 0, dt_lds_asm = 0;
   DevBuf<int32_t> dt_src;
@@ -425,9 +425,9 @@
 static FactorArgs make_factor_args(mi_osqp_batch *h, int force_all) {
   FactorArgs a{};
   const Analysis &an = (*h->anp);
-  a.n = an.n; a.m = an.m; a.N = an.N; a.B = h->B; a.nnzP = an.Pp[an.n]; a.nnzK = an.nnzK();
+  a.n = an.n; a.m = an.m; a.N = an.N; a.B = h->B; a.nnzP = an.Pp[an.n]; a.nnzK = (int)an.bf.asm_src.size();
   a.pa_len = an.Pp[an.n] + an.Ap[an.n]; a.n_levels = an.bf.n_levels; a.force_all = force_all;
-  a.storage = an.bf.storage; a.fwd = h->fwd.view(an.fwd); a.bwd = h->bwd.view(an.bwd);
+  a.storage = an.bf.storage; a.zero_len = an.bf.zero_len; a.fwd = h->fwd.view(an.fwd); a.bwd = h->bwd.view(an.bwd);
   a.blk = h->bf_blk.p; a.lvl = h->bf_lvl.p; a.utask = h->bf_utask.p; a.tri4 = h->bf_tri.p; a.dtask = h->bf_dtask.p; a.ubig = h->bf_ubig.p;
   a.ttask = h->bf_ttask.p; a.asm_dst = h->bf_asm_dst.p; a.asm_src = h->bf_asm_src.p;
   a.fwd_srcblk = h->fwd_srcblk.p; a.bwd_srcblk = h->bwd_srcblk.p;
@@ -839,7 +839,7 @@
     if ((rc = h->dt_task.upload(dt.task)) || (rc = h->dt_wave_task.upload(dt.wave_task)) || (rc = h->dt_wave_step.upload(dt.wave_step)) ||
         (rc = h->dt_tail_bar.upload(dt.tail_bar)) || (rc = h->dt_src.upload(dt.src)) ||
         (rc = h->dt_lt_pos.upload(dt.lt_pos)) || (rc = h->dt_ltcol_col.upload(dt.ltcol_col)) || (rc = h->dt_tile_tab.upload(dt.tile_tab)) ||
-        (rc = h->dt_wave_tiles.upload(dt.wave_tiles)) || (rc = h->dt_asm_q64.upload(dt.asm_q64)) ||
+        (rc = h->dt_wave_tiles.upload(dt.wave_tiles)) || (rc = h->dt_asm_q64.upload(dt.asm_q64)) || (rc = h->dt_init_tab.upload(dt.init_tab)) ||
         (rc = h->dt_src_tile.upload(dt.src_tile)) || (rc = h->dt_diag_tile.upload(dt.diag_tile)) || (rc = h->dt_task_step.upload(dt.task_step)) ||
         (rc = h->dt_Sd.alloc((size_t)dt.k * dt.k * (T + 4)))) return rc;
     const int nrt = dt.k / 16 - 4;
@@ -1043,6 +1043,9 @@
   da.dt_task = h->dt_task.p; da.dt_task_step = h->dt_task_step.p; da.n_tasks = (uint32_t)(dt.task.size() / 4);
   da.asm_q64 = h->dt_asm_q64.p; da.diag_tile = h->dt_diag_tile.p; da.src_tile = h->dt_src_tile.p;
   da.Lblk = h->Lblk.p; da.Dl = h->Dl.p; da.Sd = h->dt_Sd.p; da.dt_val = h->dt_val.p; da.dinv = h->dinv.p; da.npos = h->npos.p; da.iscal = h->iscal.p;
+  const Analysis &an = (*h->anp);
+  da.init_tab = h->dt_init_tab.p; da.n_init = (uint32_t)(dt.init_tab.size() / 256);
+  da.m = an.m; da.pa_len = an.Pp[an.n] + an.Ap[an.n]; da.pa_val = h->pa_val.p; da.rho_inv = h->rho_inv.p; da.sigma = h->st.sigma;
   return da;
 }
 
@@ -1078,7 +1081,7 @@
   HIPCHK(hipEventRecord(h->evf1, h->stream));
   if ((*h->anp).dt.k) {
     TailArgs da = make_tail_args(h, kbt, h->work.p);
-    if (pol) { da.dt_val = h->pol_dt.p; da.dinv = h->pol_dinv.p; da.pstat = pol->stat; }
+    if (pol) { da.dt_val = h->pol_dt.p; da.dinv = h->pol_dinv.p; da.pstat = pol->stat; da.pmask = fa.pmask; da.pdelta = fa.pdelta; da.sigma = fa.sigma; }
     unsigned long long *d_trace = nullptr;
     const bool tracing = getenv("MI_OSQP_TAIL_TRACE") != nullptr;
     if (tracing) { HIPCHK(hipMalloc((void **)&d_trace, (size_t)wtiles * kbt * 8 * sizeof(unsigned long long))); HIPCHK(hipMemsetAsync(d_trace, 0, (size_t)wtiles * kbt * 64, h->stream)); }
@@ -2320,15 +2323,7 @@
   fa.work = d_work; fa.mw_groups = 0;
   HIPCHK(launch_factor(fa, 1, count, h->tune.factor_threads, st));
   if (an.dt.k) {
-    const DenseTail &dt = an.dt;
-    TailArgs da{};
-    da.n = an.n; da.N = an.N; da.s = dt.s; da.k = dt.k; da.kbt = 1; da.home_bt = h->BT;
-    da.storage = an.bf.storage; da.n_slots = dt.n_steps * 64u; da.n_lt = dt.n_lt; da.n_ltcol = dt.n_ltcol; da.n_quads = (uint32_t)(dt.asm_q64.size() / 64);
-    da.nh = h->dt_nh; da.cs_doubles = h->dt_cs_doubles; da.work = d_work;
-    da.lt_pos = h->dt_lt_pos.p; da.ltcol_col = h->dt_ltcol_col.p; da.tile_tab = h->dt_tile_tab.p; da.wave_tiles = h->dt_wave_tiles.p;
-    da.dt_task = h->dt_task.p; da.dt_task_step = h->dt_task_step.p; da.n_tasks = (uint32_t)(dt.task.size() / 4);
-    da.asm_q64 = h->dt_asm_q64.p; da.diag_tile = h->dt_diag_tile.p; da.src_tile = h->dt_src_tile.p;
-    da.Lblk = fa.Lblk; da.Dl = fa.Dl; da.Sd = h->dt_Sd.p; da.dt_val = h->dt_val.p; da.dinv = h->dinv.p; da.npos = h->npos.p; da.iscal = h->iscal.p;
+    TailArgs da = make_tail_args(h, 1, d_work);
     da.trace = nullptr;
     HIPCHK(launch_tail(da, count, h->dt_lds_asm, h->dt_lds, st));
   }
@@ -3058,6 +3053,44 @@
     dense_tail_deal_stats(an.dt, *st);
   }
   return MI_OSQP_OK;
+}
+
+static int export_tail_init(const Analysis &an, int64_t *info, int64_t *perm, int64_t *entries, int64_t capacity) {
+  const DenseTail &dt = an.dt;
+  int64_t cnt = 0;
+  for (size_t t = 0; t < dt.tile_tab.size() / 4; t++) {
+    const uint64_t *blk = &dt.init_tab[(size_t)dt.tile_tab[4 * t + 1] * 256];
+    for (int p = 0; p < 256; p++) {
+      const uint32_t lo = (uint32_t)blk[p], hi = (uint32_t)(blk[p] >> 32), kind = hi >> 29;
+      if (lo == 0xFFFFFFFFu && hi == 0u) continue;
+      if (entries && cnt < capacity) {
+        int64_t idx = 0;
+        if (kind == ASM_P || kind == ASM_P_SIGMA) idx = an.Psrc[lo];
+        else if (kind == ASM_A) idx = (int64_t)lo - an.Pp[an.n];
+        else if (kind == ASM_NEG_RHOINV) idx = hi & 0x1FFFFFFFu;
+        const int64_t row[6] = {dt.tile_tab[4 * t] >> 16, dt.tile_tab[4 * t] & 0xFFFFu, p % 64, p / 64, kind, idx};
+        std::copy(row, row + 6, entries + 6 * cnt);
+      }
+      cnt++;
+    }
+  }
+  if (info) {
+    info[0] = dt.k; info[1] = dt.s; info[2] = (int64_t)dt.tile_tab.size() / 4; info[3] = cnt;
+    info[4] = an.bf.zero_len; info[5] = an.bf.storage; info[6] = (int64_t)an.bf.asm_src.size(); info[7] = an.nnzK();
+  }
+  if (perm) for (int k = 0; k < an.N; k++) perm[k] = an.perm[k];
+  return MI_OSQP_OK;
+}
+int mi_osqp_debug_host_tail_init(int64_t n, int64_t m, const int64_t *Pp, const int64_t *Pi, const int64_t *Ap, const int64_t *Ai,
+                                 int64_t *info, int64_t *perm, int64_t *entries, int64_t capacity) {
+  Analysis an;
+  int rc = analyze(n, m, Pp, Pi, Ap, Ai, tuning_from_env().analysis, an);
+  if (rc) return rc;
+  return export_tail_init(an, info, perm, entries, capacity);
+}
+int mi_osqp_batch_debug_tail_init(mi_osqp_batch *h, int64_t *info, int64_t *perm, int64_t *entries, int64_t capacity) {
+  if (!h) return MI_OSQP_ERR_NULL;
+  return export_tail_init(*h->anp, info, perm, entries, capacity);
 }
 
 int mi_osqp_debug_host_block_factor(int64_t n, int64_t m, const int64_t *Pp, const int64_t *Pi, const double *Pv,
```
